# VinAIResearch/GeoFormer

Measured on AMD Instinct MI355X. Metric: scenes/sec forward (ScanNetV2 ~150k pts), higher is better.
Workload: dtype f32

## Files before the change

geoformer_amd/_build.py:

```python
from __future__ import annotations

import os
import shutil
import subprocess
import sys
from concurrent.futures import ThreadPoolExecutor

PKG_DIR = os.path.dirname(os.path.abspath(__file__))
REPO_DIR = os.path.dirname(PKG_DIR)
CSRC_DIR = os.path.join(PKG_DIR, "csrc")
LIB_DIR = os.path.join(PKG_DIR, "lib")
OBJ_DIR = os.path.join(LIB_DIR, "obj")
LIB_PATH = os.path.join(LIB_DIR, "libgeoformer_hip.so")
INCLUDE_DIR = os.path.join(REPO_DIR, "include")

ARCH = "gfx950"


def _hipcc() -> str:
    for cand in (os.environ.get("HIPCC"), shutil.which("hipcc"), "/opt/rocm/bin/hipcc"):
        if cand and os.path.exists(cand):
            return cand
    raise RuntimeError("hipcc not found (need ROCm toolchain to build libgeoformer_hip.so)")


def _sources():
    return sorted(
        os.path.join(CSRC_DIR, f) for f in os.listdir(CSRC_DIR) if f.endswith(".hip")
    )


def _headers():
    hs = [os.path.join(CSRC_DIR, f) for f in os.listdir(CSRC_DIR) if f.endswith((".h", ".hpp"))]
    hs += [os.path.join(INCLUDE_DIR, f) for f in os.listdir(INCLUDE_DIR) if f.endswith(".h")]
    return hs


def _stale(target: str, deps) -> bool:
    if not os.path.exists(target):
        return True
    t = os.path.getmtime(target)
    return any(os.path.getmtime(d) > t for d in deps)


def build_hip(force: bool = False, verbose: bool = False) -> str:
    os.makedirs(OBJ_DIR, exist_ok=True)
    hipcc = _hipcc()
    hdrs = _headers()
    srcs = _sources()
    flags = [
        f"--offload-arch={ARCH}",
        "-O3",
        "-fPIC",
        "-std=c++17",
        "-ffp-contract=off",
        "-fno-gpu-rdc",
        "-Wno-unused-result",
        f"-I{INCLUDE_DIR}",
        f"-I{CSRC_DIR}",
    ]
    extra = {}
    jobs = []
    objs = []
    for s in srcs:
        o = os.path.join(OBJ_DIR, os.path.basename(s)[:-4] + ".o")
        objs.append(o)
        if force or _stale(o, [s] + hdrs):
            jobs.append((s, o))

    def _cc(job):
        s, o = job
        cmd = [hipcc, *flags, *extra.get(os.path.basename(s), []), "-c", s, "-o", o]
        if verbose:
            print(" ".join(cmd), file=sys.stderr)
        r = subprocess.run(cmd, capture_output=True, text=True)
        if r.returncode != 0:
            raise RuntimeError(f"hipcc failed for {s}:\n{r.stdout}\n{r.stderr}")
        return o

    if jobs:
        with ThreadPoolExecutor(max_workers=min(6, len(jobs))) as ex:
            list(ex.map(_cc, jobs))
    if force or jobs or _stale(LIB_PATH, objs):
        cmd = [hipcc, f"--offload-arch={ARCH}", "-shared", "-fPIC", "-o", LIB_PATH, *objs]
        r = subprocess.run(cmd, capture_output=True, text=True)
        if r.returncode != 0:
            raise RuntimeError(f"link failed:\n{r.stdout}\n{r.stderr}")
    return LIB_PATH


if __name__ == "__main__":
    print(build_hip(force="--force" in sys.argv, verbose=True))
```

geoformer_amd/_lib.py:

```python
from __future__ import annotations

import ctypes
import os
from ctypes import c_char_p, c_float, c_int, c_longlong, c_size_t, c_uint, c_void_p

from ._build import LIB_PATH

LIB_PATH = os.environ.get("GF_LIB_PATH", LIB_PATH)

_lib = None


class GeoFormerHipError(RuntimeError):
    pass


def _declare(lib):
    P, I, F = c_void_p, c_int, c_float
    sig = {
        "gf_abi_version": (I, []),
        "gf_last_error": (c_char_p, []),
        "gf_index_words": (c_size_t, [I, I, I, I]),
        "gf_index_scratch_bytes": (c_size_t, [c_size_t]),
        "gf_index_build": (I, [P, I, P, I, I, I, I, P, P, P, P, P]),
        "gf_rules_subm3": (I, [P, I, P, I, I, I, P, P, P, P, I, P, P, P]),
        "gf_rules_steps_words": (c_size_t, [I]),
        "gf_rules_down2": (I, [P, I, P, I, I, I, I, P, P, P, P, P, P, I, P, P, P, I, P, P, P]),
        "gf_rules_down2_chain_plan": (I, [I, I, I, I, I, I, P, P, P, P, P]),
        "gf_rules_down2_chain": (I, [P, I, I, I, I, I, I, P, P, P]),
        "gf_conv_packed_floats": (c_size_t, [I, I, I]),
        "gf_conv_pack_weights": (I, [P, I, I, I, P, P]),
        "gf_conv_pack_weights_t": (I, [P, I, I, I, I, P, P]),
        "gf_conv_fwd": (I, [P, P, P, P, P, I, I, I, I, I, I, P, P, P, P, P, P, P]),
        "gf_feeder_create": (P, [I]),
        "gf_feeder_submit": (I, [P, P]),
        "gf_feeder_wait_issued": (I, [P, I]),
        "gf_feeder_wait_copied": (I, [P, I]),
        "gf_feeder_wait_head": (I, [P, I]),
        "gf_feeder_destroy": (I, [P]),
        "gf_conv_dual_supported": (I, [I, I, I, I, I]),
        "gf_rules_flat_words": (c_size_t, [I, I]),
        "gf_rules_flat_steps": (I, [P, P, I, I, I, I, P, P]),
        "gf_conv_fwd_flat": (I, [P, P, P, P, P, P, I, I, I, I, I, I, P, P, P, P, P, P, P, P]),
        "gf_conv_fwd_dual": (I, [P, P, P, P, P, I, I, I, I, I, I, P, P, P, P, P, P, P, P]),
        "gf_dev_conv_fwd_timed": (I, [P, P, P, P, P, I, I, I, I, I, I, P, P, P, P, P, P, P, P, P]),
        "gf_dev_conv_knobs_g16": (I, [I, I, I, I]),
        "gf_dev_conv_chunks": (I, [I]),
        "gf_dev_conv_g16p_wpb": (I, [I]),
        "gf_dev_conv_knobs": (I, [I, I, I, I, I]),
        "gf_dev_conv_knob_flat": (I, [I, I]),
        "gf_dev_conv_knob_lw": (I, [I, I]),
        "gf_dev_conv_plan": (I, [P, P, P, P, P, P, I, I, I, I, I, I, P, P, P, P, P, P, P, P]),
        "gf_resblock_fwd": (I, [P, P, P, P, P, P, P, I, I, I, I, I, P, P, P, P, P, P, P, P]),
        "gf_conv_wgrad": (I, [P, P, P, I, I, I, I, I, P, P]),
        "gf_conv_wgrad_masked": (I, [P, P, P, P, I, I, I, I, I, P, P]),
        "gf_conv_wgrad_masked_acc": (I, [P, P, P, P, I, I, I, I, I, P, P]),
        "gf_lsap": (I, [P, I, I, P, P, P, P, P, P]),
        "gf_pair_losses_sums_floats": (c_size_t, [I]),
        "gf_pair_losses_fwd": (I, [P, P, P, I, I, I, P, P, P, P]),
        "gf_pair_losses_bwd": (I, [P, P, P, P, I, I, I, P, P, P, P]),
        "gf_unet_ws_bytes": (c_size_t, [P, I, I, I, I, I]),
        "gf_dev_unet_probe": (I, [I]),
        "gf_dev_host_wait_ns": (ctypes.c_ulonglong, [I]),
        "gf_dev_unet_probe_read": (I, [I, P, P]),
        "gf_dev_unet_probe_read2": (I, [I, P, P, P]),
        "gf_dev_conv_kernel_events": (I, [P, P]),
        "gf_dev_conv_kernel_events_taken": (I, []),
        "gf_dev_op_kernel_events": (I, [I, P, P]),
        "gf_dev_op_kernel_events_taken": (I, [I]),
        "gf_dev_event_create": (P, []),
        "gf_dev_event_destroy": (I, [P]),
        "gf_dev_event_elapsed_us": (I, [P, P, P]),
        "gf_unet_fwd": (I, [P, P, P, I, I, I, I, I, P, c_size_t, P, P, P, P]),
        "gf_unet_fwd_phased": (I, [P, P, P, I, I, I, I, I, P, c_size_t, P, P, P, P, P, I, P, P]),
        "gf_unet_fwd_ahead": (I, [P, P, P, I, I, I, I, I, P, c_size_t, P, P, P, P, P, I]),
        "gf_voxelize_fp": (I, [P, P, I, I, I, I, P, P]),
        "gf_voxelize_bp": (I, [P, P, I, I, I, I, P, P]),
        "gf_gather_points": (I, [P, P, I, I, I, I, P, P]),
        "gf_gather_points_grad": (I, [P, P, I, I, I, I, P, P]),
        "gf_group_points": (I, [P, P, I, I, I, I, I, P, P]),
        "gf_group_points_grad": (I, [P, P, I, I, I, I, I, P, P]),
        "gf_ball_query": (I, [P, P, I, I, I, F, I, P, P]),
        "gf_fps_scratch_bytes": (c_size_t, [I]),
        "gf_furthest_point_sampling": (I, [P, I, I, I, P, P, P]),
        "gf_furthest_point_sampling_resume": (I, [P, I, I, I, I, P, P, P]),
        "gf_knn_scratch_bytes": (c_size_t, [I]),
        "gf_knn_radius": (I, [P, I, I, F, I, P, P, P, P, P]),
        "gf_knn_error_flag": (P, [P, I]),
        "gf_geodesic_bfs": (I, [P, P, P, I, I, P, I, F, I, P, P, P, P]),
        "gf_geodesic_bfs_cfg": (I, [P, P, P, I, I, P, I, F, I, P, P, P, c_size_t, I, P]),
        "gf_geodesic_bfs_queue_words": (c_size_t, [I]),
        "gf_dev_cross_attn_bf3": (I, [I]),
        "gf_dev_bfs_qcap_max": (I, [I]),
        "gf_mask_head": (I, [P, P, P, P, P, P, P, P, P, I, I, I, P, P]),
        "gf_mask_head_packed": (I, [P, P, P, P, P, P, P, P, P, I, I, I, I, P, P]),
        "gf_mask_head_episodes": (I, [P, P, P, P, P, P, P, P, P, I, I, I, I, I, P, P, P]),
        "gf_mask_head_split_bytes": (c_size_t, [I]),
        "gf_mask_head_bwd": (I, [P, P, P, P, P, P, P, P, P, I, I, I, I, P, P, P, P]),
        "gf_mask_head_bwd_episodes": (I, [P, P, P, P, P, P, P, P, P, I, I, I, I, I, P, P, P, P]),
        "gf_mask_head_bwd_scratch_floats": (c_size_t, [I, I]),
        "gf_softmax_dim1_fwd": (I, [P, I, I, I, F, P, P]),
        "gf_softmax_dim1_bwd": (I, [P, P, I, I, I, F, P, P]),
        "gf_pointwise_mlp": (I, [P, I, I, P, P, P, P, P, P, P]),
        "gf_pointwise_mlp_rows": (I, [P, P, I, I, P, P, P, P, P, P, P]),
        "gf_group_mlp_max": (I, [P, I, I, I, I, P, P, P, P, P, P, P]),
        "gf_ball_query_centres": (I, [P, P, I, I, I, F, I, P, P, P]),
        "gf_sa_group_mlp_max": (I, [P, P, P, I, I, I, I, F, I, I, I, I, P, P, P, P, P, P, P, P, P, I, P]),
        "gf_ball_query_grid": (I, [P, I, P, P, I, F, I, P, I, P, P, P]),
        "gf_point_grid_build": (I, [P, I, F, P, P]),
        "gf_decoder_token_state_bytes": (c_size_t, [I, I]),
        "gf_decoder_token_stage": (I, [P, P, P, I, I, I, I, I, P, P, P, P, P, P]),
        "gf_mask_intersections_scratch_bytes": (c_size_t, [I, I]),
        "gf_mask_intersections": (I, [P, I, I, P, P, P]),
        "gf_proposal_stats_batched": (I, [P, I, I, P, P, c_longlong, I, F, F, I, I, P, P, P, P, P]),
        "gf_proposal_select_batched": (I, [P, P, P, I, I, P, P, P, P, P]),
        "gf_proposal_scatter_batched": (I, [P, I, I, P, P, I, I, P, F, P, P]),
        "gf_mask_intersections_batched": (I, [P, I, c_longlong, c_longlong, P, P, P]),
        "gf_matrix_nms_batched": (I, [P, I, P, I, F, F, P, P, P]),
        "gf_label_map_batched": (I, [P, I, c_longlong, I, F, P, P, P, P, P, P, P, P, P]),
        "gf_instance_overlaps_scratch_bytes": (c_size_t, [I, I]),
        "gf_instance_overlaps": (I, [P, I, I, P, I, P, P, I, I, P, P, P, P, P, P]),
        "gf_voxelize_idx_scratch_bytes": (c_size_t, [I]),
        "gf_voxelize_idx_count": (I, [P, I, I, I, P, P, P, P]),
        "gf_voxelize_idx_fill": (I, [P, I, I, I, P, P, I, I, P, P, P]),
        "gf_host_legacy_choice": (I, [P, P, c_longlong, c_longlong, P]),
        "gf_host_legacy_prefetch": (I, [P, I, c_longlong]),
        "gf_host_draw_sample": (I, [P, P, c_longlong, c_longlong, P, c_longlong, P, P, P, P, I, P, P, P]),
        "gf_fg_scratch_bytes": (c_size_t, [I]),
        "gf_fg_select": (I, [P, I, I, I, I, P, P, P, P, I, P, P, P, P, P, P, P, P, P]),
        "gf_host_wait_word": (I, [P, I, c_longlong]),
        "gf_proposal_stats": (I, [P, P, P, I, I, I, F, F, I, I, P, P, P, P, P]),
        "gf_proposal_stats_fs": (I, [P, P, I, I, F, F, I, F, P, P, P, P]),
        "gf_proposal_scatter": (I, [P, P, I, I, P, F, I, P, P]),
        "gf_relpos_prepare": (I, [P, P, I, I, I, P, P, P]),
        "gf_proposal_select": (I, [P, P, P, I, P, P, P, P, P]),
        "gf_backbone_transformer_scratch_bytes": (c_size_t, [I]),
        "gf_backbone_transformer_num_params": (I, [I]),
        "gf_backbone_transformer": (I, [P, P, P, I, I, I, I, P, P, P, P]),
        "gf_decoder_pre_train_save_bytes": (c_size_t, [I, I]),
        "gf_decoder_pre_train_work_bytes": (c_size_t, [I, I]),
        "gf_decoder_pre_grad_floats": (c_longlong, []),
        "gf_decoder_pre_train_fwd": (I, [P, P, I, I, P, F, c_uint, I, P, P, P, P]),
        "gf_decoder_pre_train_bwd": (I, [P, P, P, P, P, I, I, P, F, c_uint, I, P, P, P, P, P, P]),
        "gf_decoder_post_train_save_bytes": (c_size_t, [I, I, I]),
        "gf_decoder_post_train_work_bytes": (c_size_t, [I, I, I]),
        "gf_decoder_post_grad_floats": (c_longlong, [I]),
        "gf_decoder_post_train_fwd": (I, [P, P, I, I, I, P, F, c_uint, I, P, P, P, P]),
        "gf_decoder_post_train_bwd": (I, [P, P, P, P, I, I, I, P, F, c_uint, I, P, P, P, P, P, P]),
        "gf_backbone_transformer_train_save_bytes": (c_size_t, [I, I]),
        "gf_backbone_transformer_train_work_bytes": (c_size_t, [I, I, I]),
        "gf_backbone_transformer_grad_floats": (c_longlong, [I, I]),
        "gf_backbone_transformer_train_fwd": (I, [P, P, I, I, I, I, P, F, c_uint, P, P, P]),
        "gf_backbone_transformer_train_bwd": (I, [P, P, I, I, I, I, P, F, c_uint, P, P, P, P, P]),
        "gf_decoder_wpack_floats": (c_size_t, []),
        "gf_decoder_pack_weights": (I, [P, P, P, P, P]),
        "gf_decoder_cross_attn": (I, [P, P, P, P, P, P, P, P, P, P, P, P, I, I, I, I, P, P, P, P]),
        "gf_decoder_cross_attn_cfg": (I, [P, P, P, P, P, P, P, P, P, P, P, P, I, I, I, I, P, P, P, I, P]),
        "gf_decoder_cross_attn_bwd_scratch_floats": (c_size_t, [I, I, I]),
        "gf_decoder_cross_attn_bwd": (I, [P] * 16 + [I, I, I, I] + [P] * 6),
        "gf_bn_train_scratch_floats": (c_size_t, [I, I]),
        "gf_bn_relu_train_fwd": (I, [P, I, I, P, P, F, F, I, P, P, P, P, P, P, P]),
        "gf_bn_relu_train_bwd": (I, [P, P, P, I, I, P, P, P, I, P, P, P, P, P]),
        "gf_bn_relu_train_bwd_add": (I, [P, P, P, I, I, P, P, P, I, P, P, P, P, P, P]),
        "gf_unet_train_scratch_floats": (c_size_t, [P, I, P]),
        "gf_unet_train_fwd": (I, [P, I, I, P, P, P, P, P, P]),
        "gf_unet_train_bwd": (I, [P, I, I, P, P, P, P, P, P, P, P]),
        "gf_bn_train_cl_scratch_floats": (c_size_t, [I, I, c_longlong]),
        "gf_bn_relu_train_cl_fwd": (I, [P, I, I, c_longlong, P, P, F, F, I, P, P, P, P, P, P, P]),
        "gf_bn_relu_train_cl_bwd": (I, [P, P, P, I, I, c_longlong, P, P, P, I, P, P, P, P, P]),
        "gf_sec_op": (I, [I, P, P, I, I, P, P]),
        "gf_roipool_fp": (I, [P, P, I, I, P, P, P]),
        "gf_roipool_bp": (I, [P, P, I, I, P, P]),
        "gf_get_iou": (I, [P, P, P, P, I, I, P, P]),
        "gf_ballquery_batch_p_scratch_bytes": (c_size_t, [I]),
        "gf_ballquery_batch_p": (I, [P, P, P, I, I, F, P, P, P, P, P]),
        "gf_bfs_cluster_host": (I, [P, P, P, I, I, P, P, P, P]),
        "gf_three_nn": (I, [P, P, I, I, I, P, P, P]),
        "gf_three_interpolate": (I, [P, P, P, I, I, I, I, P, P]),
        "gf_three_interpolate_grad": (I, [P, P, P, I, I, I, I, P, P]),
        "gf_aug_scan_blocks": (I, [I]),
        "gf_aug_draw": (I, [P, ctypes.c_ulonglong, c_longlong, I, P]),
        "gf_aug_transform": (I, [P, I, I, ctypes.c_double, I, P]),
        "gf_aug_elastic": (I, [P, I, I, I, I, ctypes.c_double, I, ctypes.c_ulonglong, c_longlong, I, c_longlong, P]),
        "gf_aug_crop": (I, [P, I, I, I, I, c_longlong, I, P]),
        "gf_aug_collate": (I, [P, P, I, I, I, I, P]),
        "gf_aug_collate_fs": (I, [P, I, I, I, P]),
        "gf_aug_support": (I, [P, P, ctypes.c_double, I, I, P]),
        "gf_aug_test_query": (I, [P, ctypes.c_double, I, I, P]),
        "gf_aug_support_block": (I, [P, P, P, ctypes.c_double, I, I, P]),
    }
    for name, (res, args) in sig.items():
        fn = getattr(lib, name)
        fn.restype = res
        fn.argtypes = args
    return sig


EXPORTS = None


def _check_hw_queues(torch):
    import warnings

    from . import HW_QUEUES_MIN, HW_QUEUES_WANTED, hw_queues_setting

    have = hw_queues_setting()
    if have is not None and have >= HW_QUEUES_MIN:
        return
    up = torch.cuda.is_initialized()
    warnings.warn(
        f"geoformer_amd: GPU_MAX_HW_QUEUES is {'unset (runtime default 4)' if have is None else have}"
        + (" and the HIP runtime is already initialised" if up else "")
        + f": the runtime picks its own number of hardware queues.  Export GPU_MAX_HW_QUEUES="
        f"{HW_QUEUES_WANTED} or call geoformer_amd.configure_runtime() before the process's first HIP call"
        + (" (e.g. before torch.cuda.set_device in train.py / test.py)." if up else "."),
        RuntimeWarning, stacklevel=3)


def load():
    global _lib, EXPORTS
    if _lib is not None:
        return _lib
    if not os.path.exists(LIB_PATH):
        raise GeoFormerHipError(
            f"{LIB_PATH} is missing: build it with `python -m geoformer_amd._build` "
            "(or __graft_entry__.build()).  There is no CPU fallback for the HIP operators."
        )
    import torch

    _check_hw_queues(torch)
    lib = ctypes.CDLL(LIB_PATH)
    EXPORTS = _declare(lib)
    if lib.gf_abi_version() != 7:
        raise GeoFormerHipError("libgeoformer_hip.so ABI version mismatch")
    _lib = lib
    return lib


def check(status: int, what: str = ""):
    if status != 0:
        msg = load().gf_last_error()
        raise GeoFormerHipError(f"{what} failed ({status}): {msg.decode() if msg else ''}")


FEEDER_MAX_COPIES = 16

# ... 49 lines not shown
```

geoformer_amd/csrc/common.h:

```cpp
#pragma once
#include <hip/hip_runtime.h>
#include <hip/hip_ext.h>
#include <stdint.h>
#include <stdio.h>

#include <type_traits>

#include "geoformer_hip.h"

#define GF_WAVE 64

typedef float f32x4 __attribute__((ext_vector_type(4)));

#define GF_STEP_BLKS 7
#define GF_STEP_PHA 3
#define GF_CONV_CHUNKS 3072
#define GF_CONV_CHUNKS_MAX 4096
int gf_conv_chunks();

void gf_set_error(const char* fmt, ...);

#define GF_CHECK_ARG(cond, ...)          \
    do {                                 \
        if (!(cond)) {                   \
            gf_set_error(__VA_ARGS__);   \
            return GF_ERR_INVALID_ARG;   \
        }                                \
    } while (0)

#define GF_TRY(call)                                                             \
    do {                                                                         \
        hipError_t e__ = (call);                                                 \
        if (e__ != hipSuccess) {                                                 \
            gf_set_error("%s failed: %s", #call, hipGetErrorString(e__));        \
            return GF_ERR_LAUNCH;                                                \
        }                                                                        \
    } while (0)

#define GF_CHECK_LAUNCH(name)                                                        \
    do {                                                                             \
        hipError_t e__ = hipGetLastError();                                          \
        if (e__ != hipSuccess) {                                                     \
            gf_set_error("%s: launch failed: %s", name, hipGetErrorString(e__));     \
            return GF_ERR_LAUNCH;                                                    \
        }                                                                            \
    } while (0)

int gf_rules_down2_chain_range(const int32_t* coords, int M0, int B, int X, int Y, int Z, int nlevels, int l_begin,
                               int l_end, int32_t* ws, int32_t* counts, hipStream_t st);

int gf_iscan_blocks(int n);
void gf_iscan(const int32_t* v, int n, int32_t* start, int32_t* cursor, int32_t* block_sums, int32_t* block_off,
              hipStream_t st);

int gf_rules_down2_chain_all(const int32_t* coords, int M0, int B, int X, int Y, int Z, int nlevels, int32_t* ws,
                             int32_t* counts, hipStream_t st);
bool gf_rules_level_parallel();

static inline int gf_div_up(long long a, long long b) { return (int)((a + b - 1) / b); }

template <class T, T... Vs, class F>
static inline void gf_with(T v, F&& f) {
    (void)((v == Vs && (f(std::integral_constant<T, Vs>{}), true)) || ...);
}

void gf_allow_lds(const void* kernel, int bytes);

template <int D>
__device__ __forceinline__ float gf_shfl_xor(float v) {
    static_assert(D == 32 || D == 16 || D == 8 || D == 4 || D == 2 || D == 1, "gf_shfl_xor: D = 1, 2, 4, 8, 16, 32");
    const unsigned x = __float_as_uint(v);
    if constexpr (D == 32) {
        const auto r = __builtin_amdgcn_permlane32_swap(x, x, false, false);
        return __uint_as_float((__lane_id() & 32) ? r[0] : r[1]);
    } else if constexpr (D == 16) {
        const auto r = __builtin_amdgcn_permlane16_swap(x, x, false, false);
        return __uint_as_float((__lane_id() & 16) ? r[0] : r[1]);
    } else if constexpr (D == 8) {
        return __uint_as_float((unsigned)__builtin_amdgcn_update_dpp((int)x, (int)x, 0x128, 0xF, 0xF, false));
    } else if constexpr (D == 4) {
        const int t = __builtin_amdgcn_update_dpp((int)x, (int)x, 0x104, 0xF, 0x5, false);
        return __uint_as_float((unsigned)__builtin_amdgcn_update_dpp(t, (int)x, 0x114, 0xF, 0xA, false));
    } else if constexpr (D == 2) {
        return __uint_as_float((unsigned)__builtin_amdgcn_update_dpp((int)x, (int)x, 0x4E, 0xF, 0xF, false));
    } else {
        return __uint_as_float((unsigned)__builtin_amdgcn_update_dpp((int)x, (int)x, 0xB1, 0xF, 0xF, false));
    }
}
template <int D>
__device__ __forceinline__ int gf_shfl_xor_i(int v) {
    return __float_as_int(gf_shfl_xor<D>(__int_as_float(v)));
}
__device__ __forceinline__ int gf_wave_sum_i(int s) {
    s += gf_shfl_xor_i<32>(s);
    s += gf_shfl_xor_i<16>(s);
    s += gf_shfl_xor_i<8>(s);
    s += gf_shfl_xor_i<4>(s);
    s += gf_shfl_xor_i<2>(s);
    s += gf_shfl_xor_i<1>(s);
    return s;
}
__device__ __forceinline__ float gf_wave_max(float m) {
    m = fmaxf(m, gf_shfl_xor<32>(m));
    m = fmaxf(m, gf_shfl_xor<16>(m));
    m = fmaxf(m, gf_shfl_xor<8>(m));
    m = fmaxf(m, gf_shfl_xor<4>(m));
    m = fmaxf(m, gf_shfl_xor<2>(m));
    m = fmaxf(m, gf_shfl_xor<1>(m));
    return m;
}
__device__ __forceinline__ float gf_wave_sum(float s) {
    s += gf_shfl_xor<32>(s);
    s += gf_shfl_xor<16>(s);
    s += gf_shfl_xor<8>(s);
    s += gf_shfl_xor<4>(s);
    s += gf_shfl_xor<2>(s);
    s += gf_shfl_xor<1>(s);
    return s;
}

#define GF_FLAT_HIST 8
#define GF_FLAT_BSTART 40
#define GF_FLAT_BCUR 72
#define GF_FLAT_GOFF 128
#define GF_FLAT_BINS 1024
#define GF_FLAT_PAD 32
#define GF_LW_WPB 12
__host__ __device__ static inline size_t gf_flat_ppos_at(int ngroups) { return GF_FLAT_GOFF + (size_t)ngroups + 1; }
__host__ __device__ static inline size_t gf_flat_desc_at(int ngroups) { return (GF_FLAT_GOFF + 2 * (size_t)ngroups + 1 + 63) / 64 * 64; }
__host__ __device__ static inline size_t gf_flat_steps_at(int ngroups, int nbins) {
    return gf_flat_desc_at(ngroups) + (size_t)((ngroups + nbins - 1) / nbins + 1) * nbins * 4;
}
int gf_conv_lw_supported(int K, int M_in, int M_out, int Cin, int Cout, bool aligned, int* forced);
int gf_conv_lw(const float* in, const float* Wp, const uint32_t* gmask, const int32_t* flat, int K, int M_in, int M_out, int Cin,
               int Cout, const float* in_scale, const float* in_shift, const float* residual, const float* out_scale,
               const float* out_shift, float* out, float* out2, hipStream_t st);

enum { GF_OP_BFS = 0, GF_OP_CROSS_ATTN = 1, GF_OP_MASK_HEAD = 2, GF_OP_FPS = 3, GF_OP_CROSS_ATTN_BWD = 4,
       GF_OP_MASK_HEAD_BWD_FEAT = 5, GF_OP_MASK_HEAD_BWD_PARAM = 6, GF_OP_WGRAD = 7, GF_OP_COUNT = 8 };
struct GfOpEvents {
    hipEvent_t start, stop;
    int taken;
};
GfOpEvents* gf_op_events(int op);
#define GF_LAUNCH_OP(op, kernel, grid, block, lds, st, ...)                                              \
    do {                                                                                                 \
        GfOpEvents* oe__ = gf_op_events(op);                                                             \
        if (oe__->start) {                                                                               \
            hipExtLaunchKernelGGL(kernel, grid, block, (uint32_t)(lds), st, oe__->start, oe__->stop, 0u, __VA_ARGS__); \
            oe__->start = oe__->stop = nullptr;                                                          \
            oe__->taken = 1;                                                                             \
        } else {                                                                                         \
            hipLaunchKernelGGL(kernel, grid, block, lds, st, __VA_ARGS__);                               \
        }                                                                                                \
    } while (0)

struct GfIndex {
    const uint32_t* bitmap;
    const int32_t* prefix;
    const int32_t* perm;
    int X, Y, Z;
};

__device__ __forceinline__ int gf_index_lookup(const GfIndex& ix, int b, int x, int y, int z) {
    if ((unsigned)x >= (unsigned)ix.X || (unsigned)y >= (unsigned)ix.Y || (unsigned)z >= (unsigned)ix.Z) return -1;
    unsigned long long lin = (((unsigned long long)b * ix.X + x) * ix.Y + y) * ix.Z + z;
    unsigned long long w = lin >> 5;
    unsigned bit = (unsigned)(lin & 31);
    uint32_t word = ix.bitmap[w];
    if (!((word >> bit) & 1u)) return -1;
    int rank = ix.prefix[w] + __popc(word & ((1u << bit) - 1u));
    return ix.perm ? ix.perm[rank] : rank;
}

#define SCAN_THREADS 256
__device__ __forceinline__ int wave_incl_scan(int v) {
    const int lane = threadIdx.x & 63;
#pragma unroll
    for (int d = 1; d < 64; d <<= 1) {
        int t = __shfl_up(v, d, 64);
        if (lane >= d) v += t;
    }
    return v;
}

__device__ __forceinline__ int block_excl_scan(int v, int* total) {
    __shared__ int wsum[SCAN_THREADS / 64];
    const int lane = threadIdx.x & 63, wid = threadIdx.x >> 6;
    int inc = wave_incl_scan(v);
    if (lane == 63) wsum[wid] = inc;
    __syncthreads();
    int off = 0, tot = 0;
#pragma unroll
    for (int w = 0; w < SCAN_THREADS / 64; w++) {
        int s = wsum[w];
        if (w < wid) off += s;
        tot += s;
    }
    __syncthreads();
    *total = tot;
    return off + inc - v;
}

int gf_backbone_transformer_tables(const int* scene_offsets, int n_scenes, int M, void* scratch, void* stream);
int gf_backbone_transformer_prepared(const float* feats, const int* coords, const int* scene_offsets, int n_scenes, int M, int c,
                                     int n_layers, const float* const* params, void* scratch, float* out, void* stream);
```

geoformer_amd/csrc/geodesic.hip:

```cpp
#include <cstdlib>
#include "common.h"

#ifndef BFS_KEY_SCOPE
#define BFS_KEY_SCOPE __HIP_MEMORY_SCOPE_AGENT
#endif
#include <type_traits>

__device__ __forceinline__ int3 cell_of(float x, float y, float z, float inv_cell) {
    return make_int3((int)floorf(x * inv_cell), (int)floorf(y * inv_cell), (int)floorf(z * inv_cell));
}
__device__ __forceinline__ unsigned bucket_of(int cx, int cy, int cz, unsigned tmask) {
    return (((unsigned)cx * 73856093u) ^ ((unsigned)cy * 19349663u) ^ ((unsigned)cz * 83492791u)) & tmask;
}

__global__ void k_grid_count(const float* __restrict__ xyz, int n, float inv_cell, unsigned tmask,
                             int32_t* __restrict__ counts) {
    int i = blockIdx.x * blockDim.x + threadIdx.x;
    if (i >= n) return;
    int3 c = cell_of(xyz[i * 3 + 0], xyz[i * 3 + 1], xyz[i * 3 + 2], inv_cell);
    atomicAdd(&counts[bucket_of(c.x, c.y, c.z, tmask)], 1);
}

#define ISCAN_IPT 4
#define ISCAN_IPB (SCAN_THREADS * ISCAN_IPT)
__global__ void k_iscan_block_sums(const int32_t* __restrict__ v, int n, int32_t* __restrict__ block_sums) {
    int base = blockIdx.x * ISCAN_IPB + threadIdx.x * ISCAN_IPT;
    int s = 0;
#pragma unroll
    for (int j = 0; j < ISCAN_IPT; j++)
        if (base + j < n) s += v[base + j];
    int tot;
    block_excl_scan(s, &tot);
    if (threadIdx.x == 0) block_sums[blockIdx.x] = tot;
}
__global__ void k_iscan_top(const int32_t* __restrict__ block_sums, int nblocks, int32_t* __restrict__ block_off) {
    __shared__ int carry_s;
    if (threadIdx.x == 0) carry_s = 0;
    __syncthreads();
    for (int base = 0; base < nblocks; base += SCAN_THREADS) {
        int i = base + threadIdx.x;
        int val = i < nblocks ? block_sums[i] : 0;
        int tot;
        int ex = block_excl_scan(val, &tot);
        int carry = carry_s;
        if (i < nblocks) block_off[i] = carry + ex;
        __syncthreads();
        if (threadIdx.x == 0) carry_s = carry + tot;
        __syncthreads();
    }
}
__global__ void k_iscan_apply(const int32_t* __restrict__ v, int n, const int32_t* __restrict__ block_off,
                              int32_t* __restrict__ start, int32_t* __restrict__ cursor) {
    int base = blockIdx.x * ISCAN_IPB + threadIdx.x * ISCAN_IPT;
    int c[ISCAN_IPT];
    int s = 0;
#pragma unroll
    for (int j = 0; j < ISCAN_IPT; j++) {
        c[j] = (base + j < n) ? v[base + j] : 0;
        s += c[j];
    }
    int tot;
    int ex = block_excl_scan(s, &tot) + block_off[blockIdx.x];
#pragma unroll
    for (int j = 0; j < ISCAN_IPT; j++) {
        if (base + j < n) {
            start[base + j] = ex;
            cursor[base + j] = ex;
        }
        ex += c[j];
        if (base + j == n - 1) start[n] = ex;
    }
}

__global__ void k_grid_fill(const float* __restrict__ xyz, int n, float inv_cell, unsigned tmask,
                            int32_t* __restrict__ cursor, float4* __restrict__ sorted) {
    int i = blockIdx.x * blockDim.x + threadIdx.x;
    if (i >= n) return;
    const float x = xyz[i * 3 + 0], y = xyz[i * 3 + 1], z = xyz[i * 3 + 2];
    int3 c = cell_of(x, y, z, inv_cell);
    int pos = atomicAdd(&cursor[bucket_of(c.x, c.y, c.z, tmask)], 1);
    sorted[pos] = make_float4(x, y, z, __int_as_float(i));
}

int gf_iscan_blocks(int n) { return (n + ISCAN_IPB - 1) / ISCAN_IPB; }
void gf_iscan(const int32_t* v, int n, int32_t* start, int32_t* cursor, int32_t* block_sums, int32_t* block_off,
              hipStream_t st) {
    const int nb = gf_iscan_blocks(n);
    hipLaunchKernelGGL(k_iscan_block_sums, dim3(nb), dim3(SCAN_THREADS), 0, st, v, n, block_sums);
    hipLaunchKernelGGL(k_iscan_top, dim3(1), dim3(SCAN_THREADS), 0, st, block_sums, nb, block_off);
    hipLaunchKernelGGL(k_iscan_apply, dim3(nb), dim3(SCAN_THREADS), 0, st, v, n, block_off, start, cursor);
}

#define KNN_WAVES 4
#define KNN_CAP 1024
__global__ __launch_bounds__(KNN_WAVES * 64) void k_knn_radius(const float* __restrict__ xyz, int n, int k,
                                                               float radius, float inv_cell, unsigned tmask,
                                                               const int32_t* __restrict__ start,
                                                               const float4* __restrict__ sorted, int sqrt_out,
                                                               float* __restrict__ D, int32_t* __restrict__ I,
                                                               int32_t* __restrict__ deg, int* __restrict__ err) {
    __shared__ unsigned long long s_keys[KNN_WAVES][KNN_CAP];
    __shared__ int s_off[KNN_WAVES][28];
    __shared__ int s_beg[KNN_WAVES][27];
    const int lane = threadIdx.x & 63, wid = threadIdx.x >> 6;
    const int i = blockIdx.x * KNN_WAVES + wid;
    if (i >= n) return;
    const float qx = xyz[i * 3 + 0], qy = xyz[i * 3 + 1], qz = xyz[i * 3 + 2];
    const int3 qc = cell_of(qx, qy, qz, inv_cell);
    int beg = 0, cnt = 0;
    int ncx = 0, ncy = 0, ncz = 0;
    if (lane < 27) {
        ncx = qc.x + lane / 9 - 1;
        ncy = qc.y + (lane / 3) % 3 - 1;
        ncz = qc.z + lane % 3 - 1;
        const unsigned h = bucket_of(ncx, ncy, ncz, tmask);
        beg = start[h];
        cnt = start[h + 1] - beg;
    }
    int inc = cnt;
#pragma unroll
    for (int d = 1; d < 32; d <<= 1) {
        int t = __shfl_up(inc, d, 64);
        if (lane >= d) inc += t;
    }
    if (lane < 27) {
        s_off[wid][lane + 1] = inc;
        s_beg[wid][lane] = beg;
    }
    if (lane == 0) s_off[wid][0] = 0;
    const int total = __shfl(inc, 26, 64);
    __builtin_amdgcn_wave_barrier();
    int nin = 0;
    for (int t0 = 0; t0 < total; t0 += 64) {
        const int t = t0 + lane;
        bool hit = false;
        unsigned long long key = 0;
        if (t < total) {
            int c = 0;
#pragma unroll
            for (int s = 1; s < 27; s++) c += (s_off[wid][s] <= t) ? 1 : 0;
            const float4 p = sorted[s_beg[wid][c] + (t - s_off[wid][c])];
            const int3 pc = cell_of(p.x, p.y, p.z, inv_cell);
            const int ex = qc.x + c / 9 - 1, ey = qc.y + (c / 3) % 3 - 1, ez = qc.z + c % 3 - 1;
            if (pc.x == ex && pc.y == ey && pc.z == ez) {
                const float dx = qx - p.x, dy = qy - p.y, dz = qz - p.z;
                const float d2 = fmaf(dz, dz, fmaf(dy, dy, dx * dx));
                if (sqrtf(d2) <= radius) {
                    hit = true;
                    key = ((unsigned long long)__float_as_uint(d2) << 32) | (unsigned)__float_as_int(p.w);
                }
            }
        }
        const unsigned long long bal = __ballot(hit);
// ... 70 lines not shown

extern "C" int gf_point_grid_build(const float* xyz, int n, float radius, void* scratch, void* stream) {
    GF_CHECK_ARG(xyz && scratch && n >= 1 && radius > 0.f, "gf_point_grid_build: bad arguments");
    PointGrid G;
    if (int rc = build_point_grid(xyz, n, radius, scratch, (hipStream_t)stream, &G)) return rc;
    GF_CHECK_LAUNCH("gf_point_grid_build");
    return GF_OK;
}

extern "C" int gf_knn_radius(const float* xyz, int n, int k, float radius, int sqrt_out, float* D, int32_t* I,
                             int32_t* deg, void* scratch, void* stream) {
    GF_CHECK_ARG(n >= 0 && k >= 1 && k <= 64 && radius > 0.f, "gf_knn_radius: bad arguments n=%d k=%d r=%g", n, k,
                 radius);
    if (n == 0) return GF_OK;
    hipStream_t st = (hipStream_t)stream;
    PointGrid G;
    if (int rc = build_point_grid(xyz, n, radius, scratch, st, &G)) return rc;
    hipLaunchKernelGGL(k_knn_radius, dim3(gf_div_up(n, KNN_WAVES)), dim3(KNN_WAVES * 64), 0, st, xyz, n, k, radius,
                       G.inv_cell, G.tmask, G.start, G.sorted, sqrt_out, D, I, deg, G.err);
    GF_CHECK_LAUNCH("gf_knn_radius");
    return GF_OK;
}

#define BQG_WAVES 4
#define BQG_CAP 1024
__global__ __launch_bounds__(BQG_WAVES * 64) void k_ball_query_grid(const float* __restrict__ xyz, int n,
                                                                    const int32_t* __restrict__ centre_idx,
                                                                    const float* __restrict__ centres, int m,
                                                                    float radius2, int nsample, PointGrid G,
                                                                    float* __restrict__ new_xyz_out,
                                                                    int32_t* __restrict__ idx) {
    __shared__ __attribute__((aligned(16))) unsigned s_hit[BQG_WAVES][BQG_CAP + 16];
    __shared__ int s_off[BQG_WAVES][28];
    __shared__ int s_beg[BQG_WAVES][27];
    const int lane = threadIdx.x & 63, wid = threadIdx.x >> 6;
    const int j = blockIdx.x * BQG_WAVES + wid;
    if (j >= m) return;
    const float* c = centre_idx ? xyz + (size_t)centre_idx[j] * 3 : centres + (size_t)j * 3;
    const float qx = c[0], qy = c[1], qz = c[2];
    if (new_xyz_out && lane < 3) new_xyz_out[(size_t)j * 3 + lane] = lane == 0 ? qx : lane == 1 ? qy : qz;
    const int3 qc = cell_of(qx, qy, qz, G.inv_cell);
    int beg = 0, cnt = 0;
    if (lane < 27) {
        const unsigned h = bucket_of(qc.x + lane / 9 - 1, qc.y + (lane / 3) % 3 - 1, qc.z + lane % 3 - 1, G.tmask);
        beg = G.start[h];
        cnt = G.start[h + 1] - beg;
    }
    int inc = cnt;
#pragma unroll
    for (int d = 1; d < 32; d <<= 1) {
        int t = __shfl_up(inc, d, 64);
        if (lane >= d) inc += t;
    }
    if (lane < 27) {
        s_off[wid][lane + 1] = inc;
        s_beg[wid][lane] = beg;
    }
    if (lane == 0) s_off[wid][0] = 0;
    const int total = __shfl(inc, 26, 64);
    __builtin_amdgcn_wave_barrier();
    int nin = 0;
    for (int t0 = 0; t0 < total; t0 += 64) {
        const int t = t0 + lane;
        bool hit = false;
        unsigned pid = 0;
        if (t < total) {
            int cc = 0;
#pragma unroll
            for (int s = 1; s < 27; s++) cc += (s_off[wid][s] <= t) ? 1 : 0;
            const float4 p = G.sorted[s_beg[wid][cc] + (t - s_off[wid][cc])];
            const int3 pc = cell_of(p.x, p.y, p.z, G.inv_cell);
            if (pc.x == qc.x + cc / 9 - 1 && pc.y == qc.y + (cc / 3) % 3 - 1 && pc.z == qc.z + cc % 3 - 1) {
                const float dx = qx - p.x, dy = qy - p.y, dz = qz - p.z;
                hit = fmaf(dz, dz, fmaf(dy, dy, dx * dx)) < radius2;
                pid = (unsigned)__float_as_int(p.w);
            }
        }
        const unsigned long long bal = __ballot(hit);
        const int pos = nin + __popcll(bal & ((1ull << lane) - 1ull));
        if (hit && pos < BQG_CAP) s_hit[wid][pos] = pid;
        nin += __popcll(bal);
    }
    int32_t* row = idx + (size_t)j * nsample;
    if (nin > BQG_CAP) {
        int got = 0, first = -1;
        for (int s = 0; s < n && got < nsample; s += 64) {
            const int p = s + lane;
            bool hit = false;
            if (p < n) {
                const float dx = qx - xyz[(size_t)p * 3 + 0], dy = qy - xyz[(size_t)p * 3 + 1],
                            dz = qz - xyz[(size_t)p * 3 + 2];
                hit = fmaf(dz, dz, fmaf(dy, dy, dx * dx)) < radius2;
            }
            const unsigned long long bal = __ballot(hit);
            if (bal) {
                if (first < 0) first = s + __builtin_ctzll(bal);
                const int pos = got + __popcll(bal & ((1ull << lane) - 1ull));
                if (hit && pos < nsample) row[pos] = p;
                got += __popcll(bal);
            }
        }
        for (int l = min(got, nsample) + lane; l < nsample; l += 64) row[l] = first < 0 ? 0 : first;
        return;
    }
    {
        const int padded = (nin + 15) & ~15;
        if (nin + lane < padded) s_hit[wid][nin + lane] = 0xffffffffu;
    }
    __builtin_amdgcn_wave_barrier();
    unsigned lowest = 0xffffffffu;
    typedef unsigned u32x4 __attribute__((ext_vector_type(4)));
    const u32x4* list = reinterpret_cast<const u32x4*>(s_hit[wid]);
    const int n16 = (nin + 15) >> 4;
    for (int t = lane; t < nin; t += 64) {
        const unsigned key = s_hit[wid][t];
        int rank = 0;
        for (int u = 0; u < n16; u++) {
            const u32x4 a = list[4 * u + 0], b = list[4 * u + 1], c2 = list[4 * u + 2], d = list[4 * u + 3];
            rank += (a[0] < key) + (a[1] < key) + (a[2] < key) + (a[3] < key) + (b[0] < key) + (b[1] < key) +
                    (b[2] < key) + (b[3] < key) + (c2[0] < key) + (c2[1] < key) + (c2[2] < key) + (c2[3] < key) +
                    (d[0] < key) + (d[1] < key) + (d[2] < key) + (d[3] < key);
        }
        if (rank < nsample) row[rank] = (int)key;
        lowest = min(lowest, key);
    }
#pragma unroll
    for (int d = 32; d >= 1; d >>= 1) lowest = min(lowest, (unsigned)__shfl_xor((int)lowest, d, 64));
    const int pad = nin > 0 ? (int)lowest : 0;
    for (int l = min(nin, nsample) + lane; l < nsample; l += 64) row[l] = pad;
}

extern "C" int gf_ball_query_grid(const float* xyz, int n, const int32_t* centre_idx, const float* centres, int m,
                                  float radius, int nsample, void* scratch, int grid_ready, float* new_xyz,
                                  int32_t* idx, void* stream) {
    GF_CHECK_ARG(xyz && scratch && idx && (centre_idx || centres), "gf_ball_query_grid: null argument");
    GF_CHECK_ARG(n >= 1 && m >= 0 && nsample >= 1 && radius > 0.f, "gf_ball_query_grid: bad sizes");
    if (m == 0) return GF_OK;
    hipStream_t st = (hipStream_t)stream;
    PointGrid G;
    if (int rc = build_point_grid(xyz, n, radius, scratch, st, &G, grid_ready != 0)) return rc;
    hipLaunchKernelGGL(k_ball_query_grid, dim3(gf_div_up(m, BQG_WAVES)), dim3(BQG_WAVES * 64), 0, st, xyz, n, centre_idx,
                       centres, m, radius * radius, nsample, G, new_xyz, idx);
    GF_CHECK_LAUNCH("gf_ball_query_grid");
    return GF_OK;
}

extern "C" const int32_t* gf_knn_error_flag(void* scratch, int n) {
    const unsigned T = knn_table_size(n);
    const int nb = (int)((T + ISCAN_IPB - 1) / ISCAN_IPB);
    return (const int32_t*)scratch + 3 * (size_t)T + 1 + 2 * (size_t)nb;
}

#define BFS_THREADS 1024
__global__ __launch_bounds__(BFS_THREADS) void k_geodesic_bfs(const float* __restrict__ D, const int32_t* __restrict__ I,
                                                              const int32_t* __restrict__ deg, int n, int K,
                                                              const int32_t* __restrict__ src, float radius,
                                                              int max_step, float* __restrict__ geo,
                                                              unsigned* __restrict__ keys,
                                                              int32_t* __restrict__ queues) {
    __shared__ int s_cnt;
    const int q = blockIdx.x;
    float* g = geo + (size_t)q * n;
    unsigned* key = keys + (size_t)q * n;
    int2* cur = reinterpret_cast<int2*>(queues + (size_t)q * 4 * n);
    int2* nxt = cur + n;
    const int tid = threadIdx.x;
    for (int t = tid; t < n; t += BFS_THREADS) {
        g[t] = -1.0f;
        key[t] = 0xffffffffu;
    }
    const int s = src[q];
    __syncthreads();
    if (tid == 0) {
        g[s] = 0.0f;
        cur[0] = make_int2(s, deg ? deg[s] : K - 1);
        s_cnt = 0;
    }
    __syncthreads();
    int ncur = 1;
    const bool vec = (K & 3) == 0;
    for (int step = 0; step < max_step && ncur > 0; step++) {
        for (int f = tid; f < ncur; f += BFS_THREADS) {
            const int2 e = cur[f];
            const int u = e.x, du = e.y;
            const int32_t* Iu = I + (size_t)u * K;
            const float* Du = D + (size_t)u * K;
            for (int r0 = 0; r0 <= du; r0 += 16) {
                int v[16];
                float d[16];
#pragma unroll
                for (int c = 0; c < 4; c++) {
                    const int rb = r0 + 4 * c;
                    if (rb <= du && vec) {
                        const int4 vi = *reinterpret_cast<const int4*>(Iu + rb);
                        const float4 di = *reinterpret_cast<const float4*>(Du + rb);
                        v[4 * c + 0] = vi.x; v[4 * c + 1] = vi.y; v[4 * c + 2] = vi.z; v[4 * c + 3] = vi.w;
                        d[4 * c + 0] = di.x; d[4 * c + 1] = di.y; d[4 * c + 2] = di.z; d[4 * c + 3] = di.w;
                    } else {
#pragma unroll
                        for (int j = 0; j < 4; j++) {
                            const int rr = rb + j;
                            const bool ok = rr <= du && rr < K;
                            v[4 * c + j] = ok ? Iu[rr] : -1;
                            d[4 * c + j] = ok ? Du[rr] : 0.f;
                        }
                    }
                }
                float gv[16];
#pragma unroll
                for (int j = 0; j < 16; j++) {
                    const int rr = r0 + j;
                    const bool ok = rr >= 1 && rr <= du && v[j] >= 0 && d[j] <= radius;
                    gv[j] = ok ? g[v[j]] : 0.0f;
                }
#pragma unroll
                for (int j = 0; j < 16; j++) {
                    if (gv[j] < 0.0f) {
                        const unsigned cand = (((unsigned)u << 6) | (unsigned)(r0 + j)) + 1u;
                        const unsigned old = __hip_atomic_fetch_min(&key[v[j]], cand, __ATOMIC_RELAXED, BFS_KEY_SCOPE);
                        if (old == 0xffffffffu) {
                            const int pos = atomicAdd(&s_cnt, 1);
                            nxt[pos].x = v[j];
                        }
                    }
                }
            }
        }
        __syncthreads();
        const int nn = s_cnt;
        __syncthreads();
        if (tid == 0) s_cnt = 0;
        for (int t = tid; t < nn; t += BFS_THREADS) {
            const int v = nxt[t].x;
            const unsigned kk = __hip_atomic_load(&key[v], __ATOMIC_RELAXED, BFS_KEY_SCOPE) - 1u;
            const int u = (int)(kk >> 6), r = (int)(kk & 63u);
            const int dv = deg ? deg[v] : K - 1;
            g[v] = D[(size_t)u * K + r] + g[u];
            nxt[t].y = dv;
        }
        __syncthreads();
        int2* tmp = cur;
        cur = nxt;
        nxt = tmp;
        ncur = nn;
    }
}

#define BFS_LDS_MAX_N (1 << 19)
#ifndef BFS_LDS_BYTES
#define BFS_LDS_BYTES (150 * 1024)
#endif
__device__ __forceinline__ void bfs_lds_barrier() {
    __builtin_amdgcn_fence(__ATOMIC_RELEASE, "workgroup", "local");
    __builtin_amdgcn_s_barrier();
    __builtin_amdgcn_fence(__ATOMIC_ACQUIRE, "workgroup", "local");
}
template <int THREADS>
__global__ __launch_bounds__(THREADS) void k_geodesic_bfs_lds(const float* __restrict__ D,
                                                                  const int32_t* __restrict__ I, int n, int K,
                                                                  const int32_t* __restrict__ src, float radius,
                                                                  int max_step, float* __restrict__ geo,
                                                                  unsigned long long* __restrict__ keys,
                                                                  int2* __restrict__ queues, int qcap) {
    extern __shared__ __attribute__((aligned(16))) unsigned char smem[];
    __shared__ int s_cnt[2];
    const int nw = (n + 31) >> 5;
    unsigned* visited = reinterpret_cast<unsigned*>(smem);
    unsigned* touched = visited + nw;
    int2* q0 = reinterpret_cast<int2*>(touched + nw + ((2 * nw) & 1));
    int2* q1 = q0 + qcap;
    const int q = blockIdx.x;
    float* g = geo + (size_t)q * n;
    unsigned long long* key = keys + (size_t)q * n;
    int2* gq0 = queues + (size_t)q * 2 * n;
    int2* gq1 = gq0 + n;
    const int tid = threadIdx.x;
    for (int t = tid; t < n; t += THREADS) {
        g[t] = -1.0f;
        key[t] = ~0ull;
    }
    for (int t = tid; t < nw; t += THREADS) {
        visited[t] = 0u;
        touched[t] = 0u;
    }
    const int s = src[q];
    __syncthreads();
    if (tid == 0) {
        g[s] = 0.0f;
        visited[s >> 5] = 1u << (s & 31);
        touched[s >> 5] = 1u << (s & 31);
        q0[0] = make_int2(s, __float_as_int(0.0f));
        s_cnt[0] = 0;
        s_cnt[1] = 0;
    }
    __syncthreads();
    int ncur = 1;
    int2 *cl = q0, *cg = gq0, *nl = q1, *ng = gq1;
    constexpr int BFS_B = 4;
    const int l16 = tid & 15;
    const int gsh = (tid & 48) | 15;
    int pv[BFS_B];
    float pd[BFS_B];
    bool have_pf = false;
#ifdef BFS_TRACE
    unsigned long long tr[12] = {0, 0, 0, 0, 0, 0, 0, 0, 0, 0, 0, 0};
#define BT() __builtin_amdgcn_s_memtime()
#endif
    for (int step = 0; step < max_step && ncur > 0; step++) {
#ifdef BFS_TRACE
        const unsigned long long t0_ = BT();
        tr[5]++; tr[6] += ncur; tr[7] = tr[7] > (unsigned long long)ncur ? tr[7] : (unsigned long long)ncur;
#endif
        int* cnt = &s_cnt[step & 1];
        auto bid = [&](int u, float gu, int r, int v, float d) {
            const unsigned bit = 1u << (v & 31);
            if (!(visited[v >> 5] & bit)) {
#ifdef BFS_TRACE
                if ((tid >> 4) == 0) tr[9]++;
#endif
                const unsigned cand = (((unsigned)u << 6) | (unsigned)r) + 1u;
                __hip_atomic_fetch_min(&key[v], ((unsigned long long)cand << 32) | (unsigned)__float_as_int(d + gu),
                                       __ATOMIC_RELAXED, BFS_KEY_SCOPE);
                const unsigned old = atomicOr(&touched[v >> 5], bit);
                if (!(old & bit)) {
                    const int pos = atomicAdd(cnt, 1);
                    if (pos < qcap) nl[pos].x = v;
                    else ng[pos - qcap].x = v;
                }
            }
        };
        const int kc = l16 < K ? l16 : K - 1;
        auto batch = [&](int base, auto spill, auto pf) {
            unsigned cand[BFS_B];
            int v[BFS_B];
            float d[BFS_B];
            {
                float gu[BFS_B];
#pragma unroll
                for (int k = 0; k < BFS_B; k++) {
                    const int f = (base + k * THREADS + tid) >> 4;
                    const int fc = f < ncur ? f : ncur - 1;
                    int2 e = cl[fc < qcap ? fc : 0];
                    if constexpr (decltype(spill)::value)
                        if (fc >= qcap) e = cg[fc - qcap];
                    cand[k] = (((unsigned)e.x << 6) | (unsigned)l16) + 1u;
                    gu[k] = __int_as_float(e.y);
                    if constexpr (decltype(pf)::value) {
                        v[k] = pv[k];
                        d[k] = pd[k];
                    } else {
                        v[k] = I[(size_t)e.x * K + kc];
                        d[k] = D[(size_t)e.x * K + kc];
                    }
                }
#ifdef BFS_TRACE
                if (tid == 0) tr[8]++;
#endif
#pragma unroll
                for (int k = 0; k < BFS_B; k++) asm volatile("" : "+v"(v[k]), "+v"(d[k]));
#ifdef BFS_TRACE
                asm volatile("s_waitcnt vmcnt(0) lgkmcnt(0)" ::: "memory");
                if (base == 0) tr[10] += BT() - t0_;
#endif
#pragma unroll
                for (int k = 0; k < BFS_B; k++) {
                    const int f = (base + k * THREADS + tid) >> 4;
                    if (!(f < ncur && l16 < K && d[k] <= radius)) v[k] = -1;
                    d[k] += gu[k];
                }
            }
#ifdef BFS_TRACE
            const unsigned long long tb0_ = BT();
#endif
            unsigned long long mm = 0ull;
            unsigned w[BFS_B];
#pragma unroll
            for (int k = 0; k < BFS_B; k++) {
                mm |= ((__ballot(v[k] >= 0) >> gsh) & 1ull) << k;
                w[k] = visited[v[k] >= 0 ? (v[k] >> 5) : 0];
            }
#pragma unroll
            for (int k = 0; k < BFS_B; k++) {
                const unsigned bit = 1u << (v[k] & 31);
                const bool bids = v[k] >= 0 && l16 >= 1 && !(w[k] & bit);
#ifdef BFS_TRACE
                if ((tid >> 4) == 0) tr[9] += bids ? 1 : 0;
#endif
                w[k] = 1u;
                if (bids) {
                    __hip_atomic_fetch_min(&key[v[k]], ((unsigned long long)cand[k] << 32) | (unsigned)__float_as_int(d[k]),
                                           __ATOMIC_RELAXED, BFS_KEY_SCOPE);
                    w[k] = atomicOr(&touched[v[k] >> 5], bit) & bit;
                }
            }
            unsigned long long fm[BFS_B];
            int nfirst = 0;
#pragma unroll
            for (int k = 0; k < BFS_B; k++) {
                fm[k] = __ballot(w[k] == 0u);
                nfirst += __popcll(fm[k]);
            }
            if (nfirst) {
                int pos = 0;
                if ((tid & 63) == 0) pos = atomicAdd(cnt, nfirst);
                pos = __builtin_amdgcn_readfirstlane(pos);
#pragma unroll
                for (int k = 0; k < BFS_B; k++) {
                    if (w[k] == 0u) {
                        const int p = pos + (int)__builtin_amdgcn_mbcnt_hi((unsigned)(fm[k] >> 32),
                                                                             __builtin_amdgcn_mbcnt_lo((unsigned)fm[k], 0u));
                        if (p < qcap) nl[p].x = v[k];
                        else ng[p - qcap].x = v[k];
                    }
                    pos += __popcll(fm[k]);
                }
            }
#ifdef BFS_TRACE
            if (base == 0) tr[11] += BT() - tb0_;
#endif
            if (mm) {
#pragma unroll
                for (int k = 0; k < BFS_B; k++) {
                    if ((mm >> k) & 1ull) {
                        const int f = (base + k * THREADS + tid) >> 4;
                        int2 e = cl[f < qcap ? f : 0];
                        if constexpr (decltype(spill)::value)
                            if (f >= qcap) e = cg[f - qcap];
                        for (int r0 = 16; r0 < K; r0 += 16) {
                            const int r = r0 + l16;
                            int vv = -1;
                            float dd = 0.f;
                            if (r < K) {
                                vv = I[(size_t)e.x * K + r];
                                dd = D[(size_t)e.x * K + r];
                            }
                            const bool in2 = vv >= 0 && dd <= radius;
                            if (in2) bid(e.x, __int_as_float(e.y), r, vv, dd);
                            if (!((__ballot(in2) >> gsh) & 1ull)) break;
                        }
                    }
                }
            }
        };
        auto expand = [&](auto spill) {
            int base = 0;
            if (have_pf) {
                batch(0, spill, std::true_type{});
                base = BFS_B * THREADS;
            }
            for (; (base >> 4) < ncur; base += BFS_B * THREADS) batch(base, spill, std::false_type{});
        };
        if (ncur > qcap) expand(std::true_type{});
        else expand(std::false_type{});
#ifdef BFS_TRACE
        const unsigned long long t1_ = BT();
#endif
        asm volatile("s_waitcnt vmcnt(0)" ::: "memory");
#ifdef BFS_TRACE
        const unsigned long long t2_ = BT();
#endif
        __syncthreads();
#ifdef BFS_TRACE
        const unsigned long long t3_ = BT();
#endif
        const int nn = *cnt;
        if (tid == 0) s_cnt[(step + 1) & 1] = 0;
        const bool pf_now = step + 1 < max_step;
        auto commit_batch = [&](int base, auto spill, auto pf) {
            int v[BFS_B];
            unsigned kk[BFS_B];
#pragma unroll
            for (int k = 0; k < BFS_B; k++) {
                const int t = (base + k * THREADS + tid) >> 4;
                const int tc = t < nn ? t : nn - 1;
                v[k] = nl[tc < qcap ? tc : 0].x;
                if constexpr (decltype(spill)::value)
                    if (tc >= qcap) v[k] = ng[tc - qcap].x;
                kk[k] = __hip_atomic_load(reinterpret_cast<const unsigned*>(&key[v[k]]), __ATOMIC_RELAXED, BFS_KEY_SCOPE);
            }
            if constexpr (decltype(pf)::value) {
#pragma unroll
                for (int k = 0; k < BFS_B; k++) {
                    pv[k] = I[(size_t)v[k] * K + kc];
                    pd[k] = D[(size_t)v[k] * K + kc];
                }
            }
#pragma unroll
            for (int k = 0; k < BFS_B; k++) {
                const int t = (base + k * THREADS + tid) >> 4;
                if (t < nn && l16 == 0) {
                    const int di = (int)kk[k];
                    g[v[k]] = __int_as_float(di);
                    if (!decltype(spill)::value || t < qcap) nl[t].y = di;
                    else ng[t - qcap].y = di;
                    atomicOr(&visited[v[k] >> 5], 1u << (v[k] & 31));
                }
            }
        };
        auto commit = [&](auto spill) {
            int base = 0;
            if (pf_now && nn > 0) {
                commit_batch(0, spill, std::true_type{});
                base = BFS_B * THREADS;
            }
            for (; (base >> 4) < nn; base += BFS_B * THREADS) commit_batch(base, spill, std::false_type{});
        };
        if (nn > qcap) commit(std::true_type{});
        else commit(std::false_type{});
        have_pf = pf_now;
#ifdef BFS_TRACE
        const unsigned long long t4_ = BT();
#endif
        if (nn > qcap) __syncthreads();
        else bfs_lds_barrier();
#ifdef BFS_TRACE
        const unsigned long long t5_ = BT();
        tr[0] += t1_ - t0_; tr[1] += t2_ - t1_; tr[2] += t3_ - t2_; tr[3] += t4_ - t3_; tr[4] += t5_ - t4_;
#endif
        int2* t1 = cl; cl = nl; nl = t1;
        int2* t2 = cg; cg = ng; ng = t2;
        ncur = nn;
    }
#ifdef BFS_TRACE
    if (tid == 0 && n >= 12)
        for (int i = 0; i < 12; i++) reinterpret_cast<unsigned long long*>(gq0)[i] = tr[i];
#endif
}

template <int THREADS>
static void launch_bfs_lds(int nq, size_t lds, hipStream_t st, const float* D, const int32_t* I, int n, int K,
                           const int32_t* src, float radius, int max_step, float* geo, void* keys_ws, void* queue_ws,
                           int qcap) {
    gf_allow_lds((const void*)k_geodesic_bfs_lds<THREADS>, BFS_LDS_BYTES);
    GF_LAUNCH_OP(GF_OP_BFS, k_geodesic_bfs_lds<THREADS>, dim3(nq), dim3(THREADS), lds, st, D, I, n, K, src, radius, max_step,
                 geo, (unsigned long long*)keys_ws, (int2*)queue_ws, qcap);
}
static int g_bfs_qcap_max = 0;
extern "C" int gf_dev_bfs_qcap_max(int qcap) {
    g_bfs_qcap_max = qcap > 0 ? qcap : 0;
    return GF_OK;
}
extern "C" size_t gf_geodesic_bfs_queue_words(int n) { return (size_t)4 * (size_t)(n > 0 ? n : 0); }

extern "C" int gf_geodesic_bfs_cfg(const float* D, const int32_t* I, const int32_t* deg, int n, int K,
                                   const int32_t* src, int nq, float radius, int max_step, float* geo, void* keys_ws,
                                   void* queue_ws, size_t queue_words, int wg_threads, void* stream) {
    GF_CHECK_ARG(n >= 1 && K >= 2 && K <= 64 && nq >= 0 && max_step >= 0, "gf_geodesic_bfs: bad arguments");
    GF_CHECK_ARG(n < (1 << 26), "gf_geodesic_bfs: n=%d exceeds the 26-bit parent field", n);
    GF_CHECK_ARG(wg_threads == 1024 || wg_threads == 512 || wg_threads == 256, "gf_geodesic_bfs: wg_threads=%d (256, 512 or 1024)",
                 wg_threads);
    if (nq == 0) return GF_OK;
    GF_CHECK_ARG(queue_words >= (size_t)4 * (size_t)n, "gf_geodesic_bfs: queue workspace of %zu words per query, %zu needed",
                 queue_words, (size_t)4 * (size_t)n);
    const int nw = (n + 31) / 32;
    const size_t bm = ((size_t)2 * nw + ((2 * nw) & 1)) * sizeof(unsigned);
    while (wg_threads < 1024 && bm + 256 * 2 * sizeof(int2) > (size_t)BFS_LDS_BYTES * wg_threads / 1024) wg_threads *= 2;
    const size_t budget = (size_t)BFS_LDS_BYTES * wg_threads / 1024;
    if (n <= BFS_LDS_MAX_N && (K & 3) == 0 && bm + 64 * 2 * sizeof(int2) <= budget) {
        int qcap = (int)((budget - bm) / (2 * sizeof(int2)));
        if (qcap > n) qcap = n;
        if (g_bfs_qcap_max > 0 && qcap > g_bfs_qcap_max) qcap = g_bfs_qcap_max < 64 ? 64 : g_bfs_qcap_max;
        const size_t lds = bm + (size_t)qcap * 2 * sizeof(int2);
        hipStream_t st = (hipStream_t)stream;
        if (wg_threads == 256)
            launch_bfs_lds<256>(nq, lds, st, D, I, n, K, src, radius, max_step, geo, keys_ws, queue_ws, qcap);
        else if (wg_threads == 512)
            launch_bfs_lds<512>(nq, lds, st, D, I, n, K, src, radius, max_step, geo, keys_ws, queue_ws, qcap);
        else
            launch_bfs_lds<1024>(nq, lds, st, D, I, n, K, src, radius, max_step, geo, keys_ws, queue_ws, qcap);
        GF_CHECK_LAUNCH("gf_geodesic_bfs");
        return GF_OK;
    }
    hipLaunchKernelGGL(k_geodesic_bfs, dim3(nq), dim3(BFS_THREADS), 0, (hipStream_t)stream, D, I, deg, n, K, src,
                       radius, max_step, geo, (unsigned*)keys_ws, (int32_t*)queue_ws);
    GF_CHECK_LAUNCH("gf_geodesic_bfs");
    return GF_OK;
}

extern "C" int gf_geodesic_bfs(const float* D, const int32_t* I, const int32_t* deg, int n, int K, const int32_t* src,
                               int nq, float radius, int max_step, float* geo, void* keys_ws, void* queue_ws,
                               void* stream) {
    return gf_geodesic_bfs_cfg(D, I, deg, n, K, src, nq, radius, max_step, geo, keys_ws, queue_ws, (size_t)4 * (size_t)(n > 0 ? n : 0),
                               1024, stream);
}

__global__ void k_bqb_count(const float* __restrict__ xyz, const int32_t* __restrict__ batch_idxs,
                            const int32_t* __restrict__ batch_offsets, int n, float radius2, int32_t* __restrict__ cnt) {
    int i = blockIdx.x * blockDim.x + threadIdx.x;
    if (i >= n) return;
    const float ox = xyz[i * 3 + 0], oy = xyz[i * 3 + 1], oz = xyz[i * 3 + 2];
    const int b = batch_idxs[i];
    int c = 0;
    for (int k = batch_offsets[b]; k < batch_offsets[b + 1]; k++) {
        const float dx = ox - xyz[k * 3 + 0], dy = oy - xyz[k * 3 + 1], dz = oz - xyz[k * 3 + 2];
        if (fmaf(dz, dz, fmaf(dy, dy, dx * dx)) < radius2) {
            if (c >= 1000) break;
            c++;
        }
    }
    cnt[i] = c;
}
__global__ void k_bqb_fill(const float* __restrict__ xyz, const int32_t* __restrict__ batch_idxs,
                           const int32_t* __restrict__ batch_offsets, int n, float radius2,
                           const int32_t* __restrict__ start, const int32_t* __restrict__ cnt, long long thre,
                           int32_t* __restrict__ idx, int32_t* __restrict__ start_len) {
    int i = blockIdx.x * blockDim.x + threadIdx.x;
    if (i >= n) return;
    const int s = start[i];
    int c = cnt[i];
    start_len[i * 2 + 0] = s;
    start_len[i * 2 + 1] = c;
    if (s >= thre) return;
    if ((long long)s + c >= thre) c = (int)(thre - s);
    const float ox = xyz[i * 3 + 0], oy = xyz[i * 3 + 1], oz = xyz[i * 3 + 2];
    const int b = batch_idxs[i];
    int w = 0;
    for (int k = batch_offsets[b]; k < batch_offsets[b + 1] && w < c; k++) {
        const float dx = ox - xyz[k * 3 + 0], dy = oy - xyz[k * 3 + 1], dz = oz - xyz[k * 3 + 2];
        if (fmaf(dz, dz, fmaf(dy, dy, dx * dx)) < radius2) idx[s + w++] = k;
    }
}
extern "C" size_t gf_ballquery_batch_p_scratch_bytes(int n) {
    const size_t nb = ((size_t)n + ISCAN_IPB - 1) / ISCAN_IPB;
    return (2 * (size_t)n + 4 + 2 * nb + 16) * sizeof(int32_t);
}
extern "C" int gf_ballquery_batch_p(const float* xyz, const int32_t* batch_idxs, const int32_t* batch_offsets, int n,
                                    int meanActive, float radius, int32_t* idx, int32_t* start_len, int32_t* d_cumsum,
                                    void* scratch, void* stream) {
    GF_CHECK_ARG(n >= 0 && meanActive >= 1, "gf_ballquery_batch_p: bad arguments");
    hipStream_t st = (hipStream_t)stream;
    if (n == 0) {
        GF_TRY(hipMemsetAsync(d_cumsum, 0, sizeof(int32_t), st));
        return GF_OK;
    }
    const int nb = (n + ISCAN_IPB - 1) / ISCAN_IPB;
    int32_t* cnt = (int32_t*)scratch;
    int32_t* start = cnt + n;
    int32_t* block_sums = start + n + 2;
    int32_t* block_off = block_sums + nb;
    const float r2 = radius * radius;
    hipLaunchKernelGGL(k_bqb_count, dim3(gf_div_up(n, 256)), dim3(256), 0, st, xyz, batch_idxs, batch_offsets, n, r2, cnt);
    hipLaunchKernelGGL(k_iscan_block_sums, dim3(nb), dim3(SCAN_THREADS), 0, st, cnt, n, block_sums);
    hipLaunchKernelGGL(k_iscan_top, dim3(1), dim3(SCAN_THREADS), 0, st, block_sums, nb, block_off);
    hipLaunchKernelGGL(k_iscan_apply, dim3(nb), dim3(SCAN_THREADS), 0, st, cnt, n, block_off, start, start_len);
    GF_TRY(hipMemcpyAsync(d_cumsum, start + n, sizeof(int32_t), hipMemcpyDeviceToDevice, st));
    hipLaunchKernelGGL(k_bqb_fill, dim3(gf_div_up(n, 256)), dim3(256), 0, st, xyz, batch_idxs, batch_offsets, n, r2,
                       start, cnt, (long long)n * meanActive, idx, start_len);
    GF_CHECK_LAUNCH("gf_ballquery_batch_p");
    return GF_OK;
}
```

geoformer_amd/csrc/pointops.hip:

```cpp
#include <stdlib.h>

#include <type_traits>

#include "common.h"

__global__ void k_voxelize_fp(const float* __restrict__ feats, const int32_t* __restrict__ rules, int M, int maxActive,
                              int C, int average, float* __restrict__ out) {
    long long t = (long long)blockIdx.x * blockDim.x + threadIdx.x;
    if (t >= (long long)M * C) return;
    const int row = (int)(t / C), c = (int)(t - (long long)row * C);
    const int32_t* r = rules + (size_t)row * (maxActive + 1);
    const int n = r[0];
    const float mult = (average && n > 0) ? __fdiv_rn(1.0f, (float)n) : 1.0f;
    float acc = 0.f;
    for (int i = 1; i <= n; i++) acc = __fadd_rn(acc, __fmul_rn(mult, feats[(size_t)r[i] * C + c]));
    out[t] = acc;
}

__global__ void k_voxelize_bp(const float* __restrict__ d_out, const int32_t* __restrict__ rules, int M, int maxActive,
                              int C, int average, float* __restrict__ d_feats) {
    long long t = (long long)blockIdx.x * blockDim.x + threadIdx.x;
    if (t >= (long long)M * C) return;
    const int row = (int)(t / C), c = (int)(t - (long long)row * C);
    const int32_t* r = rules + (size_t)row * (maxActive + 1);
    const int n = r[0];
    const float mult = (average && n > 0) ? __fdiv_rn(1.0f, (float)n) : 1.0f;
    const float g = __fmul_rn(mult, d_out[t]);
    for (int i = 1; i <= n; i++) atomicAdd(&d_feats[(size_t)r[i] * C + c], g);
}

extern "C" int gf_voxelize_fp(const float* feats, const int32_t* rules, int M, int maxActive, int C, int average,
                              float* out, void* stream) {
    GF_CHECK_ARG(M >= 0 && maxActive >= 0 && C >= 1, "gf_voxelize_fp: bad sizes");
    if (M == 0) return GF_OK;
    hipLaunchKernelGGL(k_voxelize_fp, dim3(gf_div_up((long long)M * C, 256)), dim3(256), 0, (hipStream_t)stream, feats,
                       rules, M, maxActive, C, average, out);
    GF_CHECK_LAUNCH("gf_voxelize_fp");
    return GF_OK;
}
extern "C" int gf_voxelize_bp(const float* d_out, const int32_t* rules, int M, int maxActive, int C, int average,
                              float* d_feats, void* stream) {
    GF_CHECK_ARG(M >= 0 && maxActive >= 0 && C >= 1, "gf_voxelize_bp: bad sizes");
    if (M == 0) return GF_OK;
    hipLaunchKernelGGL(k_voxelize_bp, dim3(gf_div_up((long long)M * C, 256)), dim3(256), 0, (hipStream_t)stream, d_out,
                       rules, M, maxActive, C, average, d_feats);
    GF_CHECK_LAUNCH("gf_voxelize_bp");
    return GF_OK;
}

__global__ void k_gather_points(const float* __restrict__ points, const int32_t* __restrict__ idx, int b, int c, int n,
                                int m, float* __restrict__ out) {
    long long t = (long long)blockIdx.x * blockDim.x + threadIdx.x;
    if (t >= (long long)b * c * m) return;
    const int j = (int)(t % m);
    const long long bc = t / m;
    const int bi = (int)(bc / c);
    out[t] = points[bc * n + idx[(size_t)bi * m + j]];
}
__global__ void k_gather_points_grad(const float* __restrict__ grad_out, const int32_t* __restrict__ idx, int b, int c,
                                     int n, int m, float* __restrict__ grad_points) {
    long long t = (long long)blockIdx.x * blockDim.x + threadIdx.x;
    if (t >= (long long)b * c * m) return;
    const int j = (int)(t % m);
    const long long bc = t / m;
    const int bi = (int)(bc / c);
    atomicAdd(&grad_points[bc * n + idx[(size_t)bi * m + j]], grad_out[t]);
}
__global__ void k_group_points(const float* __restrict__ points, const int32_t* __restrict__ idx, int b, int c, int n,
                               int np, int ns, float* __restrict__ out) {
    long long t = (long long)blockIdx.x * blockDim.x + threadIdx.x;
    const long long per = (long long)np * ns;
    if (t >= (long long)b * c * per) return;
    const long long js = t % per;
    const long long bc = t / per;
    const int bi = (int)(bc / c);
    out[t] = points[bc * n + idx[(size_t)bi * per + js]];
}
__global__ void k_group_points_grad(const float* __restrict__ grad_out, const int32_t* __restrict__ idx, int b, int c,
                                    int n, int np, int ns, float* __restrict__ grad_points) {
    long long t = (long long)blockIdx.x * blockDim.x + threadIdx.x;
    const long long per = (long long)np * ns;
    if (t >= (long long)b * c * per) return;
    const long long js = t % per;
    const long long bc = t / per;
    const int bi = (int)(bc / c);
    atomicAdd(&grad_points[bc * n + idx[(size_t)bi * per + js]], grad_out[t]);
}

#define GF_ELEMENTWISE(fn, kern, total, ...)                                                                    \
    do {                                                                                                        \
        long long tot__ = (total);                                                                              \
        if (tot__ > 0) {                                                                                        \
            hipLaunchKernelGGL(kern, dim3(gf_div_up(tot__, 256)), dim3(256), 0, (hipStream_t)stream, __VA_ARGS__); \
            GF_CHECK_LAUNCH(fn);                                                                                \
        }                                                                                                       \
        return GF_OK;                                                                                           \
    } while (0)

extern "C" int gf_gather_points(const float* points, const int32_t* idx, int b, int c, int n, int m, float* out,
                                void* stream) {
    GF_ELEMENTWISE("gf_gather_points", k_gather_points, (long long)b * c * m, points, idx, b, c, n, m, out);
}
extern "C" int gf_gather_points_grad(const float* grad_out, const int32_t* idx, int b, int c, int n, int m,
                                     float* grad_points, void* stream) {
    GF_ELEMENTWISE("gf_gather_points_grad", k_gather_points_grad, (long long)b * c * m, grad_out, idx, b, c, n, m,
                   grad_points);
}
extern "C" int gf_group_points(const float* points, const int32_t* idx, int b, int c, int n, int np, int ns, float* out,
                               void* stream) {
    GF_ELEMENTWISE("gf_group_points", k_group_points, (long long)b * c * np * ns, points, idx, b, c, n, np, ns, out);
}
extern "C" int gf_group_points_grad(const float* grad_out, const int32_t* idx, int b, int c, int n, int np, int ns,
                                    float* grad_points, void* stream) {
    GF_ELEMENTWISE("gf_group_points_grad", k_group_points_grad, (long long)b * c * np * ns, grad_out, idx, b, c, n, np,
                   ns, grad_points);
}

#ifndef BQ_WAVES
#define BQ_WAVES 8
#endif
#ifndef BQ_TILE
#define BQ_TILE 2048
#endif
#define BQ_PLANE (BQ_TILE + 12)
#define BQ_LD ((BQ_TILE * 3 + BQ_WAVES * 64 - 1) / (BQ_WAVES * 64))
__global__ __launch_bounds__(BQ_WAVES * 64) void k_ball_query(const float* __restrict__ new_xyz,
                                                               const float* __restrict__ xyz, int n, int m,
                                                               float radius2, int nsample, int32_t* __restrict__ idx,
                                                               const int32_t* __restrict__ centre_idx,
                                                               float* __restrict__ new_xyz_out) {
    __shared__ __attribute__((aligned(16))) float tile[2][3 * BQ_PLANE];
    __shared__ int s_done[2][BQ_WAVES];
    const int bi = blockIdx.y;
    xyz += (size_t)bi * n * 3;
    idx += (size_t)bi * m * nsample;
    const int lane = threadIdx.x & 63, wid = threadIdx.x >> 6;
    const int j = blockIdx.x * BQ_WAVES + wid;
    const bool valid = j < m;
    float nx = 0.f, ny = 0.f, nz = 0.f;
    if (valid) {
        const float* c = centre_idx ? xyz + (size_t)centre_idx[(size_t)bi * m + j] * 3 : new_xyz + ((size_t)bi * m + j) * 3;
        nx = c[0];
        ny = c[1];
        nz = c[2];
        if (centre_idx && lane < 3) new_xyz_out[((size_t)bi * m + j) * 3 + lane] = lane == 0 ? nx : lane == 1 ? ny : nz;
    }
    int cnt = valid ? 0 : nsample;
    int first = -1;
    int slot[BQ_LD];
#pragma unroll
    for (int i = 0; i < BQ_LD; i++) {
        const unsigned f = threadIdx.x + BQ_WAVES * 64 * i;
        const unsigned p = __umulhi(f, 0xAAAAAAABu) >> 1;
        slot[i] = f < BQ_TILE * 3 ? (int)((f - 3u * p) * BQ_PLANE + p) : -1;
    }
// ... 46 lines not shown
                    if (first < 0) {
                        const int l0 = __builtin_ctzll(any);
                        const int u0 = ((bal[0] >> l0) & 1) ? 0 : ((bal[1] >> l0) & 1) ? 1 : ((bal[2] >> l0) & 1) ? 2 : 3;
                        first = base + s + 4 * l0 + u0;
                    }
                    const unsigned long long below = (1ull << lane) - 1ull;
                    int pos = cnt + __popcll(bal[0] & below) + __popcll(bal[1] & below) + __popcll(bal[2] & below) +
                              __popcll(bal[3] & below);
#pragma unroll
                    for (int u = 0; u < 4; u++) {
                        if (hit[u]) {
                            if (pos < nsample) idx[(size_t)j * nsample + pos] = base + s + 4 * lane + u;
                            pos++;
                        }
                    }
                    cnt += __popcll(bal[0]) + __popcll(bal[1]) + __popcll(bal[2]) + __popcll(bal[3]);
                }
            }
        }
        if (t + 1 < ntiles) stage(buf ^ 1);
        if (lane == 0) s_done[buf ^ 1][wid] = cnt >= nsample;
        __syncthreads();
    }
    if (valid) {
        const int filled = min(cnt, nsample);
        const int pad = first < 0 ? 0 : first;
        for (int l = filled + lane; l < nsample; l += 64) idx[(size_t)j * nsample + l] = pad;
    }
}

extern "C" int gf_ball_query(const float* new_xyz, const float* xyz, int b, int n, int m, float radius, int nsample,
                             int32_t* idx, void* stream) {
    GF_CHECK_ARG(b >= 0 && n >= 0 && m >= 0 && nsample >= 1, "gf_ball_query: bad sizes");
    if (b == 0 || m == 0) return GF_OK;
    const float radius2 = radius * radius;
    hipLaunchKernelGGL(k_ball_query, dim3(gf_div_up(m, BQ_WAVES), b), dim3(BQ_WAVES * 64), 0, (hipStream_t)stream,
                       new_xyz, xyz, n, m, radius2, nsample, idx, nullptr, nullptr);
    GF_CHECK_LAUNCH("gf_ball_query");
    return GF_OK;
}

extern "C" int gf_ball_query_centres(const float* xyz, const int32_t* centre_idx, int b, int n, int m, float radius,
                                     int nsample, float* new_xyz, int32_t* idx, void* stream) {
    GF_CHECK_ARG(b >= 0 && n >= 0 && m >= 0 && nsample >= 1, "gf_ball_query_centres: bad sizes");
    GF_CHECK_ARG(centre_idx && new_xyz, "gf_ball_query_centres: null argument");
    if (b == 0 || m == 0) return GF_OK;
    const float radius2 = radius * radius;
    hipLaunchKernelGGL(k_ball_query, dim3(gf_div_up(m, BQ_WAVES), b), dim3(BQ_WAVES * 64), 0, (hipStream_t)stream,
                       nullptr, xyz, n, m, radius2, nsample, idx, centre_idx, new_xyz);
    GF_CHECK_LAUNCH("gf_ball_query_centres");
    return GF_OK;
}

#define FPS_KEY_NONE 0x7fffffffu
#define FPS_SPIN_LIMIT (1 << 22)

__device__ __forceinline__ unsigned dpp_max_step(unsigned v, unsigned o) { return o > v ? o : v; }

__device__ __forceinline__ unsigned wave_max_u32(unsigned v) {
    v = dpp_max_step(v, (unsigned)__builtin_amdgcn_update_dpp(0, (int)v, 0xB1, 0xF, 0xF, true));
    v = dpp_max_step(v, (unsigned)__builtin_amdgcn_update_dpp(0, (int)v, 0x4E, 0xF, 0xF, true));
    v = dpp_max_step(v, (unsigned)__builtin_amdgcn_update_dpp(0, (int)v, 0x141, 0xF, 0xF, true));
    v = dpp_max_step(v, (unsigned)__builtin_amdgcn_update_dpp(0, (int)v, 0x140, 0xF, 0xF, true));
    const unsigned r0 = __builtin_amdgcn_readlane((int)v, 0), r1 = __builtin_amdgcn_readlane((int)v, 16);
    const unsigned r2 = __builtin_amdgcn_readlane((int)v, 32), r3 = __builtin_amdgcn_readlane((int)v, 48);
    const unsigned a = r0 > r1 ? r0 : r1, b = r2 > r3 ? r2 : r3;
    return a > b ? a : b;
}

__device__ __forceinline__ void wave_best(unsigned& dbits, unsigned& key) {
    const unsigned md = wave_max_u32(dbits);
    const unsigned long long owners = __ballot(dbits == md);
    if (__popcll(owners) == 1) {
        key = (unsigned)__builtin_amdgcn_readlane((int)key, __builtin_ctzll(owners));
    } else {
        const unsigned cand = dbits == md ? (FPS_KEY_NONE - key) : 0u;
        key = FPS_KEY_NONE - wave_max_u32(cand);
    }
    dbits = md;
}

template <int I, int N, typename F>
__device__ __forceinline__ void fps_static_for(F&& f) {
    if constexpr (I < N) {
        f(std::integral_constant<int, I>{});
        fps_static_for<I + 1, N>(f);
    }
}

#ifndef FPS_WAVES
#define FPS_WAVES 16
#endif
#ifndef FPS_MAXG
#define FPS_MAXG 16
#endif
#ifndef FPS_KPUB
#define FPS_KPUB 4
#endif
#ifndef FPS_K
#define FPS_K 16
#endif
#define FPS_PW (FPS_WAVES - FPS_WAVES / 4)
#ifndef FPS_POLL_SLEEP
#define FPS_POLL_SLEEP 4
#endif
#define FPS_NG (FPS_MAXG * FPS_KPUB / 64)
#define FPS_TAG (1ull << 63)

__device__ __forceinline__ unsigned long long fps_code(unsigned dbits, unsigned key) {
    return ((unsigned long long)dbits << 32) | ((unsigned long long)(FPS_KEY_NONE - key) << 1);
}
__device__ __forceinline__ unsigned long long wave_max_u64(unsigned long long c) {
    const unsigned hi = (unsigned)(c >> 32), md = wave_max_u32(hi);
    const unsigned long long owners = __ballot(hi == md);
    unsigned ml;
    if (__popcll(owners) == 1) {
        ml = (unsigned)__builtin_amdgcn_readlane((int)(unsigned)c, __builtin_ctzll(owners));
    } else {
        ml = wave_max_u32(hi == md ? (unsigned)c : 0u);
    }
    return ((unsigned long long)md << 32) | ml;
}
__device__ __forceinline__ int fps_code_index(unsigned long long c) {
    return c ? (int)((FPS_KEY_NONE - (unsigned)((c >> 1) & 0x7fffffffull)) & 0x3fffffu) : 0;
}

#ifdef FPS_TRACE
__device__ unsigned long long* g_fps_trace = nullptr;
extern "C" int gf_dev_fps_trace(void* p) {
    GF_TRY(hipMemcpyToSymbol(HIP_SYMBOL(g_fps_trace), &p, sizeof(p)));
    return GF_OK;
}
#define FT() __builtin_amdgcn_s_memtime()
#define FTA(i, a, b) do { ftr[i] += (b) - (a); } while (0)
#else
#define FT() 0ull
#define FTA(i, a, b) do { } while (0)
#endif

#define FPS_LDS_ST(p, v) __hip_atomic_store((p), (v), __ATOMIC_RELAXED, __HIP_MEMORY_SCOPE_WORKGROUP)
#define FPS_LDS_LD(p) __hip_atomic_load((p), __ATOMIC_RELAXED, __HIP_MEMORY_SCOPE_WORKGROUP)
#define FPS_ORDER() asm volatile("" ::: "memory")
template <int P>
__device__ __forceinline__ void fps_absorb(const float (&px)[P], const float (&py)[P], const float (&pz)[P], float (&tmp)[P],
                                           float ax, float ay, float az) {
#pragma unroll
    for (int i = 0; i < P; i++) {
        const float dx = px[i] - ax, dy = py[i] - ay, dz = pz[i] - az;
        tmp[i] = fminf(fmaf(dz, dz, fmaf(dy, dy, dx * dx)), tmp[i]);
    }
}

template <int P>
__global__ __launch_bounds__(FPS_WAVES * 64) void k_fps(const float* __restrict__ xyz, int n, int m, int m0, int G,
                                                        int bs_log2, int batch0,
                                                        unsigned long long* __restrict__ slots,
                                                        int32_t* __restrict__ idxs, int* __restrict__ err) {
    static_assert(FPS_NG >= 1 && FPS_NG * 64 == FPS_MAXG * FPS_KPUB && FPS_KPUB <= FPS_K && FPS_WAVES * 2 <= 64,
                  "lane mappings of the exchange");
    __shared__ unsigned long long s_part[2][FPS_WAVES * 2];
    __shared__ float s_xyz[2][FPS_K * 3];
    __shared__ unsigned s_prog[2];
    const int bi = batch0 + blockIdx.y, wg = blockIdx.x;
    xyz += (size_t)bi * n * 3;
    idxs += (size_t)bi * m;
    slots += (size_t)bi * 2 * FPS_MAXG * FPS_KPUB;
    const int lane = threadIdx.x & 63, wid = threadIdx.x >> 6;
    const bool holder = (wid & 3) != 0;
    const int hid = wid - 1 - (wid >> 2);
    const int gtid = (wg * FPS_PW + hid) * 64 + lane;
    const int stride = G * FPS_PW * 64;
    if (threadIdx.x < 2) s_prog[threadIdx.x] = 0u;
    if (!holder && lane < 4) s_part[lane >> 1][wid * 2 + (lane & 1)] = 0ull;

    float px[P], py[P], pz[P], tmp[P];
    unsigned key[P];
    unsigned elig = 0;
    const unsigned bs_mask = (1u << bs_log2) - 1u;
#pragma unroll
    for (int i = 0; i < P; i++) {
        const int k = gtid + i * stride;
        px[i] = py[i] = pz[i] = 0.f;
        tmp[i] = 1e10f;
        key[i] = FPS_KEY_NONE;
        if (holder && k < n) {
            px[i] = xyz[(size_t)k * 3 + 0];
            py[i] = xyz[(size_t)k * 3 + 1];
            pz[i] = xyz[(size_t)k * 3 + 2];
            const float mag = fmaf(pz[i], pz[i], fmaf(py[i], py[i], px[i] * px[i]));
            if (!((double)mag <= 1e-3)) elig |= 1u << i;
            const unsigned rev = bs_log2 ? (__brev((unsigned)k & bs_mask) >> (32 - bs_log2)) : 0u;
            key[i] = (rev << 22) | (unsigned)k;
        }
    }
    if (m0 <= 0 && wg == 0 && threadIdx.x == 0) idxs[0] = 0;
    int nnew = 1;
    float nx[FPS_K], ny[FPS_K], nz[FPS_K];
    nx[0] = xyz[0]; ny[0] = xyz[1]; nz[0] = xyz[2];
#pragma unroll
    for (int a = 1; a < FPS_K; a++) nx[a] = ny[a] = nz[a] = 0.f;
    int done = 1;
    if (m0 > 1) {
        for (int base = 0; base < m0 - 1; base += FPS_K) {
            const int cntk = min(FPS_K, m0 - 1 - base);
#pragma unroll
            for (int a = 0; a < FPS_K; a++) {
                const int pi = a < cntk ? idxs[base + a] : 0;
                nx[a] = xyz[(size_t)pi * 3 + 0];
                ny[a] = xyz[(size_t)pi * 3 + 1];
                nz[a] = xyz[(size_t)pi * 3 + 2];
            }
#pragma unroll
            for (int i = 0; i < P; i++) {
                if (elig & (1u << i)) {
                    float d2 = tmp[i];
#pragma unroll
                    for (int a = 0; a < FPS_K; a++) {
                        if (a < cntk) {
                            const float dx = px[i] - nx[a], dy = py[i] - ny[a], dz = pz[i] - nz[a];
                            d2 = fminf(fmaf(dz, dz, fmaf(dy, dy, dx * dx)), d2);
                        }
                    }
                    tmp[i] = d2;
                }
            }
        }
        const int pl = idxs[m0 - 1];
        nx[0] = xyz[(size_t)pl * 3 + 0];
        ny[0] = xyz[(size_t)pl * 3 + 1];
        nz[0] = xyz[(size_t)pl * 3 + 2];
        done = m0;
    }
#ifdef FPS_TRACE
    unsigned long long ftr[10] = {0, 0, 0, 0, 0, 0, 0, 0, 0, 0};
#endif
    if (holder) {
#pragma unroll
        for (int i = 0; i < P; i++) {
            if (elig & (1u << i)) {
                const float dx = px[i] - nx[0], dy = py[i] - ny[0], dz = pz[i] - nz[0];
                tmp[i] = fminf(fmaf(dz, dz, fmaf(dy, dy, dx * dx)), tmp[i]);
            }
        }
    } else {
        __builtin_amdgcn_s_setprio(3);
    }
    __syncthreads();
    for (int round = 1; done < m; round++) {
        const int par = round & 1;
        const unsigned long long ft0 = FT();
        unsigned bd = 0u, bk = FPS_KEY_NONE;
#pragma unroll
        for (int i = 0; i < P; i++) {
            if (elig & (1u << i)) {
                float d2 = tmp[i];
                const unsigned db = __float_as_uint(d2);
                if (db > bd || (db == bd && key[i] < bk)) {
                    bd = db;
                    bk = key[i];
                }
            }
        }
        const unsigned long long ft1 = FT();
        FTA(0, ft0, ft1);
        if (holder) {
        unsigned d1 = bd, k1 = bk;
        wave_best(d1, k1);
        unsigned cd = bd, ck = bk;
        if (bk == k1 && k1 != FPS_KEY_NONE) {
            cd = 0u;
            ck = FPS_KEY_NONE;
#pragma unroll
            for (int i = 0; i < P; i++) {
                if ((elig & (1u << i)) && key[i] != k1) {
                    const unsigned db = __float_as_uint(tmp[i]);
                    if (db > cd || (db == cd && key[i] < ck)) {
                        cd = db;
                        ck = key[i];
                    }
                }
            }
        }
        unsigned d2w = cd, k2w = ck;
        wave_best(d2w, k2w);
        if (lane == 0) {
            unsigned long long c1 = fps_code(d1, k1), c2 = fps_code(d2w, k2w);
            if (c2 != 0ull) c2 |= 1ull;
            else if (c1 != 0ull) c1 |= 1ull;
            s_part[par][wid * 2 + 0] = c1;
            s_part[par][wid * 2 + 1] = c2;
        }
        }
        const unsigned long long ft2 = FT();
        FTA(1, ft1, ft2);
        __syncthreads();
        const unsigned long long ft3 = FT();
        FTA(2, ft2, ft3);
        if (wid == 0) {
            unsigned long long mine = lane < FPS_WAVES * 2 ? s_part[par][lane] : 0ull;
            unsigned long long wgc[FPS_KPUB];
            bool stop = false;
            int cnt = 0;
            fps_static_for<0, FPS_KPUB>([&](auto tc) {
                constexpr int t = decltype(tc)::value;
                const unsigned long long best = stop ? 0ull : wave_max_u64(mine);
                wgc[t] = best & ~1ull;
                if (best != 0ull) {
                    if (mine == best) mine = 0ull;
                    if (best & 1ull) stop = true;
                    cnt = t + 1;
// ... 33 lines not shown
#pragma unroll
                    for (int j = 0; j < FPS_NG; j++) {
                        if (!ok[j]) {
                            v[j] = __hip_atomic_load(rs + lane + 64 * j, __ATOMIC_RELAXED, __HIP_MEMORY_SCOPE_AGENT);
                            ok[j] = (v[j] & FPS_TAG) == tag;
                            all = all && ok[j];
                        }
                    }
                    if (++spins > FPS_SPIN_LIMIT) {
                        *err = 1;
                        break;
                    }
                }
#pragma unroll
                for (int j = 0; j < FPS_NG; j++) v[j] = (lane + 64 * j < G * FPS_KPUB) ? (v[j] & ~FPS_TAG) : 0ull;
            }
            const unsigned long long ft5 = FT();
            FTA(4, ft4, ft5);
            float vx[FPS_NG], vy[FPS_NG], vz[FPS_NG];
#pragma unroll
            for (int j = 0; j < FPS_NG; j++) {
                const int ci = fps_code_index(v[j]);
                vx[j] = xyz[(size_t)ci * 3 + 0];
                vy[j] = xyz[(size_t)ci * 3 + 1];
                vz[j] = xyz[(size_t)ci * 3 + 2];
            }
            static_assert(FPS_NG == 1, "one gathered candidate per lane");
#ifdef FPS_TRACE
            {
                float probe = vx[0];
                asm volatile("v_mov_b32 %0, %0" : "+v"(probe));
                vx[0] = probe;
            }
#endif
            const unsigned long long ft6 = FT();
            FTA(5, ft5, ft6);
            const unsigned long long mine0 = v[0];
            const unsigned long long Bcode = wave_max_u64((mine0 & 1ull) ? (mine0 & ~1ull) : 0ull);
            unsigned ckey = (unsigned)((mine0 >> 1) & 0x7fffffffull);
            float cdist = __uint_as_float((unsigned)(mine0 >> 32));
            bool alive = mine0 != 0ull;
            int nacc = 0;
            float kx = 0.f, ky = 0.f, kz = 0.f;
            int kidx = 0;
            bool direct = false;
            const unsigned clo = ckey << 1;
            const unsigned Bhi = (unsigned)(Bcode >> 32), Blo = (unsigned)Bcode;
            auto take = [&](int ol, unsigned best_lo, int t) {
                const float bx = __int_as_float(__builtin_amdgcn_readlane(__float_as_int(vx[0]), ol));
                const float by = __int_as_float(__builtin_amdgcn_readlane(__float_as_int(vy[0]), ol));
                const float bz = __int_as_float(__builtin_amdgcn_readlane(__float_as_int(vz[0]), ol));
                const bool keeper = lane == t;
                kx = keeper ? bx : kx;
                ky = keeper ? by : ky;
                kz = keeper ? bz : kz;
                kidx = keeper ? (int)((FPS_KEY_NONE - ((best_lo >> 1) & 0x7fffffffu)) & 0x3fffffu) : kidx;
                if (lane == ol) alive = false;
                if (lane == 0) {
                    FPS_LDS_ST(&s_xyz[par][t * 3 + 0], bx);
                    FPS_LDS_ST(&s_xyz[par][t * 3 + 1], by);
                    FPS_LDS_ST(&s_xyz[par][t * 3 + 2], bz);
                    FPS_ORDER();
                    FPS_LDS_ST(&s_prog[par], ((unsigned)round << 8) | (unsigned)(t + 1));
                }
                const float dx = vx[0] - bx, dy = vy[0] - by, dz = vz[0] - bz;
                cdist = fminf(cdist, fmaf(dz, dz, fmaf(dy, dy, dx * dx)));
            };
            {
                const unsigned long long my = alive ? (((unsigned long long)__float_as_uint(cdist) << 32) | clo) : 0ull;
                const unsigned long long best = wave_max_u64(my);
                if (best == 0ull) {
                    if (lane == 0) {
                        FPS_LDS_ST(&s_xyz[par][0], xyz[0]);
                        FPS_LDS_ST(&s_xyz[par][1], xyz[1]);
                        FPS_LDS_ST(&s_xyz[par][2], xyz[2]);
                        if (wg == 0) idxs[done] = 0;
                    }
                    direct = true;
                } else {
                    take(__builtin_ctzll(__ballot(alive && my == best)), (unsigned)best, 0);
                }
                nacc = 1;
            }
            if (!direct) {
#pragma unroll 1
                for (int t = 1; t < FPS_K && done + t < m; t++) {
                    const unsigned hi = alive ? __float_as_uint(cdist) : 0u;
                    const unsigned md = wave_max_u32(hi);
                    if (md == 0u) break;
                    const unsigned long long owners = __ballot(hi == md);
                    int ol;
                    unsigned blo;
                    if (__popcll(owners) == 1) {
                        ol = __builtin_ctzll(owners);
                        blo = (unsigned)__builtin_amdgcn_readlane((int)clo, ol);
                    } else {
                        blo = wave_max_u32(hi == md ? clo : 0u);
                        ol = __builtin_ctzll(__ballot(hi == md && clo == blo));
                    }
                    if (md < Bhi || (md == Bhi && blo < Blo)) break;
                    take(ol, blo, t);
                    nacc = t + 1;
                }
            }
            if (!direct && lane < nacc && wg == 0) idxs[done + lane] = kidx;
            FPS_ORDER();
            if (lane == 0) FPS_LDS_ST(&s_prog[par], ((unsigned)round << 8) | 0x80u | (unsigned)nacc);
            nnew = nacc;
            (void)kx; (void)ky; (void)kz;
            const unsigned long long ft7 = FT();
            FTA(6, ft6, ft7);
        }
        else if (holder) {
            const unsigned tag = (unsigned)round << 8;
            int seen = 0;
            for (;;) {
                const unsigned c = FPS_LDS_LD(&s_prog[par]);
                FPS_ORDER();
                const bool cur = (c & 0xffffff00u) == tag;
                const int cnt = cur ? (int)(c & 0x7fu) : 0;
                for (int a = seen; a < cnt; a++) {
                    const float ax = FPS_LDS_LD(&s_xyz[par][a * 3 + 0]), ay = FPS_LDS_LD(&s_xyz[par][a * 3 + 1]),
                                az = FPS_LDS_LD(&s_xyz[par][a * 3 + 2]);
                    fps_absorb<P>(px, py, pz, tmp, ax, ay, az);
                }
                seen = cnt;
                if (cur && (c & 0x80u)) break;
                __builtin_amdgcn_s_sleep(FPS_POLL_SLEEP);
            }
            nnew = seen;
        } else {
            const unsigned tag = (unsigned)round << 8;
            unsigned c;
            for (;;) {
                c = FPS_LDS_LD(&s_prog[par]);
                if ((c & 0xffffff80u) == (tag | 0x80u)) break;
                __builtin_amdgcn_s_sleep(32);
            }
            nnew = (int)(c & 0x7fu);
        }
        done += nnew;
#ifdef FPS_TRACE
        ftr[8] += 1;
        ftr[9] += nnew;
#endif
    }
#ifdef FPS_TRACE
    if (g_fps_trace && wg == 0 && threadIdx.x == 0)
        for (int i = 0; i < 10; i++) g_fps_trace[i] = ftr[i];
#endif
}

template <int P>
static void launch_fps(int G, int nb, hipStream_t st, const float* xyz, int n, int m, int m0, int bs_log2, int batch0,
                       unsigned long long* slots, int32_t* idxs, int* err) {
    GF_LAUNCH_OP(GF_OP_FPS, (k_fps<P>), dim3(G, nb), dim3(FPS_WAVES * 64), 0, st, xyz, n, m, m0, G, bs_log2, batch0, slots,
                 idxs, err);
}

extern "C" size_t gf_fps_scratch_bytes(int b) {
    return ((size_t)b * 2 * FPS_MAXG * FPS_KPUB + 8) * sizeof(unsigned long long);
}

extern "C" int gf_furthest_point_sampling_resume(const float* xyz, int b, int n, int m, int m_known, int32_t* idxs,
                                                 void* scratch, void* stream);

extern "C" int gf_furthest_point_sampling(const float* xyz, int b, int n, int m, int32_t* idxs, void* scratch,
                                          void* stream) {
    return gf_furthest_point_sampling_resume(xyz, b, n, m, 0, idxs, scratch, stream);
}

extern "C" int gf_furthest_point_sampling_resume(const float* xyz, int b, int n, int m, int m_known, int32_t* idxs,
                                                 void* scratch, void* stream) {
    GF_CHECK_ARG(b >= 0 && n >= 1 && m >= 0, "gf_furthest_point_sampling: bad sizes b=%d n=%d m=%d", b, n, m);
    GF_CHECK_ARG(m_known >= 0 && m_known <= m, "gf_furthest_point_sampling_resume: m_known=%d not in [0, m=%d]", m_known,
                 m);
    if (m_known == m && m > 0) return GF_OK;
    GF_CHECK_ARG(n < (1 << 22), "gf_furthest_point_sampling: n=%d exceeds the 22-bit index of the tie-break key", n);
    if (b == 0 || m == 0) return GF_OK;
    hipStream_t st = (hipStream_t)stream;
    int bs_log2 = 0;
    while ((2 << bs_log2) <= n && bs_log2 < 9) bs_log2++;
    const int per_wg = FPS_PW * 64;
    int G = (2 * n + per_wg * 5 - 1) / (per_wg * 5);
    if (G < 1) G = 1;
    if (G > FPS_MAXG) G = FPS_MAXG;
    const int P = (n + G * per_wg - 1) / (G * per_wg);
    GF_CHECK_ARG(P <= 22, "gf_furthest_point_sampling: n=%d too large (max %d)", n, FPS_MAXG * per_wg * 22);
    unsigned long long* slots = (unsigned long long*)scratch;
    int* err = (int*)(slots + (size_t)b * 2 * FPS_MAXG * FPS_KPUB);
    GF_TRY(hipMemsetAsync(scratch, 0, gf_fps_scratch_bytes(b), st));
    const int per_launch = 1024 / (G * FPS_WAVES) > 0 ? 1024 / (G * FPS_WAVES) : 1;
    for (int b0 = 0; b0 < b; b0 += per_launch) {
        const int nb = (b - b0) < per_launch ? (b - b0) : per_launch;
        if (P <= 1) launch_fps<1>(G, nb, st, xyz, n, m, m_known, bs_log2, b0, slots, idxs, err);
        else if (P <= 2) launch_fps<2>(G, nb, st, xyz, n, m, m_known, bs_log2, b0, slots, idxs, err);
        else if (P <= 3) launch_fps<3>(G, nb, st, xyz, n, m, m_known, bs_log2, b0, slots, idxs, err);
        else if (P <= 4) launch_fps<4>(G, nb, st, xyz, n, m, m_known, bs_log2, b0, slots, idxs, err);
        else if (P <= 5) launch_fps<5>(G, nb, st, xyz, n, m, m_known, bs_log2, b0, slots, idxs, err);
        else if (P <= 6) launch_fps<6>(G, nb, st, xyz, n, m, m_known, bs_log2, b0, slots, idxs, err);
        else if (P <= 8) launch_fps<8>(G, nb, st, xyz, n, m, m_known, bs_log2, b0, slots, idxs, err);
        else if (P <= 12) launch_fps<12>(G, nb, st, xyz, n, m, m_known, bs_log2, b0, slots, idxs, err);
        else if (P <= 16) launch_fps<16>(G, nb, st, xyz, n, m, m_known, bs_log2, b0, slots, idxs, err);
        else if (P <= 20) launch_fps<20>(G, nb, st, xyz, n, m, m_known, bs_log2, b0, slots, idxs, err);
        else launch_fps<22>(G, nb, st, xyz, n, m, m_known, bs_log2, b0, slots, idxs, err);
    }
    GF_CHECK_LAUNCH("gf_furthest_point_sampling");
    return GF_OK;
}
```

geoformer_amd/model/geoformer.py:

```python
from __future__ import annotations

import functools
import os

import numpy as np
import torch
import torch.nn as nn
from torch.nn import functional as F

from .. import _lib, pointops, spconv, unet_exec, unet_train
from . import config as _config
from .backbone import ResidualBlock, UBlock, conv1d_bn_relu, random_downsample
from .layers import (BatchNorm1d, BigLinear, GenericMLP, LazyRelPos, PointwiseConv1d, PositionEmbeddingCoordsSine, RelPosSpec,
                     TransformerDecoder,
                     TransformerDecoderLayer, scene_counts)
from .set_abstraction import PointnetSAModuleVotesSeparate


class _Voxelization(torch.autograd.Function):

    @staticmethod
    def forward(ctx, feats, map_rule, mode=4):
        ctx.rule, ctx.mode, ctx.N = map_rule, mode, feats.shape[0]
        return pointops.voxelize_fp(feats.contiguous(), map_rule, mode)

    @staticmethod
    def backward(ctx, d_out):
        d_feats = torch.zeros((ctx.N, d_out.shape[1]), dtype=torch.float32, device=d_out.device)
        pointops.voxelize_bp(d_out.contiguous(), ctx.rule, ctx.mode, d_feats)
        return d_feats, None, None


voxelization = _Voxelization.apply


import threading
import weakref


def _bfs_wg(nq, scenes=1):
    return 1024 if nq * scenes <= 224 else 512
_SIDE_STREAMS = {}
_OFFS_CACHE = threading.local()


def get_batch_offsets(batch_idxs, bs, host_only=False):
    if bs == 1:
        n = int(batch_idxs.shape[0])
        t = torch.tensor([0, n], dtype=torch.int32, device="cpu" if host_only else batch_idxs.device)
        _OFFS_CACHE.key, _OFFS_CACHE.val = t, [0, n]
        return t
    counts = scene_counts(batch_idxs, bs)
    return torch.cat([counts.new_zeros(1), counts.cumsum(0)]).int()



def _offsets_list(t):
    if getattr(_OFFS_CACHE, "key", None) is t:
        return _OFFS_CACHE.val
    lru = getattr(_OFFS_CACHE, "lru", None)
    if lru is None:
        lru = _OFFS_CACHE.lru = {}
    hit = lru.get(id(t))
    if hit is not None and hit[0]() is t and hit[1] == t._version:
        return hit[2]
    val = t.tolist()
    if len(lru) > 64:
        lru.clear()
    lru[id(t)] = (weakref.ref(t), t._version, val)
    return val


def _tensors_of(obj):
    if torch.is_tensor(obj):
        yield obj
    elif isinstance(obj, (tuple, list)):
        for o in obj:
            yield from _tensors_of(o)


@torch.no_grad()
def knn_graphs(locs_float_, batch_offsets_, batch_size, neighbor=64, radius=0.05):
    offs = _offsets_list(batch_offsets_)
    return [pointops.knn_radius(locs_float_[offs[b]:offs[b + 1]].contiguous(), neighbor, radius, sqrt_out=True,
                                return_flag=True)
            for b in range(batch_size)]


def knn_truncated(graphs):
    fl = [g[3] for g in (graphs or ()) if len(g) > 3]
    return torch.stack([f.reshape(()) for f in fl]).amax().reshape(1) if fl else None


@torch.no_grad()
def cal_geodesic(pre_enc_inds, locs_float_, batch_offsets_, max_step=128, neighbor=64, radius=0.05, n_queries=128,
                 graphs=None):
    if graphs is None:
        graphs = knn_graphs(locs_float_, batch_offsets_, pre_enc_inds.shape[0], neighbor, radius)
    out = []
    for b in range(pre_enc_inds.shape[0]):
        D, I, deg = graphs[b][:3]
        src = pre_enc_inds[b][:n_queries].int().contiguous()
        out.append(pointops.geodesic_bfs(D, I, deg, src, radius, max_step))
    return out


def _stream_key_of(device, stream):
    idx = torch.device(device).index
    return (torch.cuda.current_device() if idx is None else idx, stream.cuda_stream)


def _stream_key(device=None):
    raw = getattr(torch._C, "_cuda_getCurrentRawStream", None)
    if raw is not None:
        idx = torch.cuda.current_device() if device is None else torch.device(device).index
        if idx is None:
            idx = torch.cuda.current_device()
        return (idx, raw(idx))
    st = torch.cuda.current_stream(device)
    return (st.device.index, st.cuda_stream)


class PendingProposals:

    _pinned = []
    _lock = threading.Lock()

    def __init__(self, final, cls_pred, scores, logits, fg_idxs, logit_thresh, num_points, knn_flags=()):
        self.stream = torch.cuda.current_stream(logits.device)
        sel, cls, sc, cnt = pointops.proposal_select(final.contiguous(), cls_pred.contiguous(), scores.contiguous())
        self.args = (sel, cls, sc, logits, fg_idxs, logit_thresh, num_points)
        with PendingProposals._lock:
            buf = PendingProposals._pinned.pop() if PendingProposals._pinned else None
        if buf is None:
            buf = torch.zeros(2, dtype=torch.int32).pin_memory()
        buf[1] = 0
        buf[0:1].copy_(cnt, non_blocking=True)
        for f in knn_flags:
            buf[1:2].copy_(f, non_blocking=True)
        self.host = buf
        self.done = torch.cuda.Event()
        self.done.record(self.stream)
        self.value = None
        self.home = None

    def get(self):
        if self.value is None:
            sel, cls, sc, logits, fg_idxs, logit_thresh, num_points = self.args
            _lib.timed_wait(self.done)
            n, overflow = int(self.host[0]), int(self.host[1])
            with PendingProposals._lock:
                PendingProposals._pinned.append(self.host)
            self.host = None
            if overflow:
                from .._lib import GeoFormerHipError

                raise GeoFormerHipError("kNN graph: a point has more in-radius neighbours than the kernel's candidate list "
                                        "holds (1024); its row is not the 64 nearest and the geodesic distances "
                                        "would be wrong -- deduplicate the scene's points")
            if n == 0:
                self.value = ([], [], [])
            else:
                with torch.cuda.stream(self.stream):
                    proposals = pointops.proposal_scatter(logits, sel[:n], fg_idxs, logit_thresh, num_points)
                self.value = (cls[:n], sc[:n], proposals)
                if self.home is not None:
                    cur = torch.cuda.current_stream(logits.device)
                    if cur.cuda_stream != self.stream.cuda_stream:
                        ev = torch.cuda.Event()
                        ev.record(self.stream)
                        cur.wait_event(ev)
                        for t in self.value:
                            t.record_stream(cur)
            self.args = None
        return self.value


class PendingBatchProposals:

    def __init__(self, n_scenes, scene_ids=(), table=None, sel=None, cls=None, scores=None, counts=None, fg_idxs=None,
                 logit_thresh=0.5, num_points=(), max_N=0, knn_flags=(), value=None):
        self.value = value
        if value is not None:
            return
        self.n_scenes, self.scene_ids, self.num_points, self.max_N = n_scenes, list(scene_ids), list(num_points), max_N
        self.args = (table, sel, cls, scores, counts, fg_idxs, logit_thresh)
        S = len(self.scene_ids)
        self.stream = torch.cuda.current_stream(sel.device)
        self.host = torch.zeros(S + 1, dtype=torch.int32).pin_memory()
        self.host[:S].copy_(counts, non_blocking=True)
        for f in knn_flags:
            self.host[S:S + 1].copy_(f, non_blocking=True)
        self.done = torch.cuda.Event()
        self.done.record(self.stream)
# ... 209 lines not shown
        return self._preprocess(batch_input, batch_size)

    def _preprocess(self, batch_input, batch_size):
        feats = batch_input["feats"]
        if self.cfg.use_coords:
            feats = torch.cat((feats, batch_input["locs_float"]), 1).float()
        voxel_feats = voxelization(feats, batch_input["v2p_map"], self.cfg.mode)
        return spconv.SparseConvTensor(voxel_feats, batch_input["voxel_locs"].int().contiguous(), batch_input["spatial_shape"],
                                       batch_size)

    def _inputs_ahead(self, batch_input):
        evs = batch_input.get("inputs_event") if isinstance(batch_input, dict) else None
        locs = batch_input["voxel_locs"]
        if evs is None or not locs.is_cuda or torch.is_grad_enabled() or os.environ.get("GF_UNET_EXEC", "1") == "0":
            return None
        if unet_exec.phase_pending():
            return None
        main = torch.cuda.current_stream(locs.device)
        if main.query():
            return None
        return main, unet_exec.side_stream_for(locs.device, main), list(evs)

    def unet_features(self, x, batch_size):
        if os.environ.get("GF_UNET_EXEC", "1") != "0" and unet_exec.supported(self, x.features, x.spatial_shape):
            x.features = unet_exec.unet_forward(self, x.features.contiguous(), x._coords(), batch_size, x.spatial_shape)
            return x
        if unet_exec.take_coords_ready() is not None:
            torch.cuda.current_stream().wait_stream(unet_exec.side_stream_for(x.features.device))
        sig = unet_train.supported(self, x)
        if sig:
            feats = unet_train.unet_forward(self, x, batch_size, sig)
            if feats is not None:
                x.features = feats
                return x
        x.indice_dict["_prebuild"] = self.prebuild_rulebooks
        return self.output_layer(self.unet(self.input_conv(x)))

    def forward_backbone(self, batch_input, batch_size, want_preds=True):
        ctx = self._grad_ctx("unet")
        with ctx():
            x = self.unet_features(self.preprocess_input(batch_input, batch_size), batch_size)
            return self._semantic_head(x, batch_input, want_preds)

    def _semantic_head(self, x, batch_input, want_preds):
        p2v = batch_input["p2v_map"]
        if not want_preds and p2v.dtype == torch.int32 and p2v.is_contiguous():
            vox = x.features.contiguous()
            chain = self._pointwise_chain("semantic", [self.semantic, self.semantic_linear], vox)
            if chain is not None:
                return (vox, p2v), pointops.pointwise_mlp(vox, chain, rows=p2v), None
        output_feats = pointops.points_from_voxels(x.features, p2v, batch_input.get("v2p_map")).contiguous()
        chain = self._pointwise_chain("semantic", [self.semantic, self.semantic_linear], output_feats)
        if chain is not None:
            semantic_scores = pointops.pointwise_mlp(output_feats, chain)
        else:
            semantic_scores = self.semantic_linear(self.semantic(output_feats))
        semantic_preds = semantic_scores.max(1)[1] if want_preds else None
        return output_feats, semantic_scores, semantic_preds

    @staticmethod
    def prebuild_rulebooks(x, nlevels=6):
        from .. import sparse

        if not x.features.is_cuda or x.indices.shape[0] == 0:
            return
        coords = x._coords()
        chain = sparse.down_rules_chain(coords, x.batch_size, x.spatial_shape, nlevels)
        cur = coords
        for l, r in enumerate(chain):
            r.prebuilt_for = cur.data_ptr()
            x.indice_dict[f"spconv{l + 1}"] = r
            cur = r.out_coords

    def _mask_tower_rows(self, feats):
        if not (feats.is_cuda and torch.is_grad_enabled() and feats.dim() == 2 and feats.dtype == torch.float32
                and os.environ.get("GF_FUSED_BN", "1") != "0"):
            return None
        from .layers import _SplitKLinearFn

        mods = list(self.mask_tower)
        x = feats.contiguous()
        last = mods[-1]
        if not (isinstance(last, nn.Conv1d) and last.kernel_size == (1,)):
            return None
        for mod in mods[:-1]:
            if not (isinstance(mod, nn.Sequential) and len(mod) == 3 and isinstance(mod[0], nn.Conv1d)
                    and mod[0].kernel_size == (1,) and mod[0].bias is None and isinstance(mod[2], nn.ReLU)
                    and isinstance(mod[1], nn.BatchNorm1d) and mod[1].num_features == mod[0].out_channels
                    and pointops.bn_relu_train_supported(
                        mod[1], x if mod[0].out_channels == x.shape[1] else x.new_empty((x.shape[0], mod[0].out_channels)))):
                return None
        for mod in mods[:-1]:
            x = pointops.bn_relu_train(mod[1], _SplitKLinearFn.apply(x, mod[0].weight[:, :, 0], None))
        return _SplitKLinearFn.apply(x, last.weight[:, :, 0], last.bias).unsqueeze(2)

    def forward_aggregator(self, locs_float_, output_feats_, batch_offsets_, batch_size):
        ctx = self._grad_ctx("set_aggregator")
        offs = _offsets_list(batch_offsets_)
        with ctx():
            locs, gfeat, gxyz, inds = [], [], [], []
            for b in range(batch_size):
                n_b = offs[b + 1] - offs[b]
                if n_b == 0:
                    return None
                npoint = min(n_b, self.cfg.n_downsampling)
                draw = pointops.legacy_choice(n_b, npoint) if locs_float_.is_cuda else \
                    np.random.choice(n_b, npoint, replace=False)
                sampling_indices = torch.tensor(draw, dtype=torch.long, device=locs_float_.device)
                self.last_sampling_indices = sampling_indices
                xyz_b = locs_float_[offs[b]:offs[b + 1]][sampling_indices].unsqueeze(0)
                feat_b = output_feats_[offs[b]:offs[b + 1]][sampling_indices].unsqueeze(0)
                l, gf, gx, idx = self.set_aggregator.group_points(xyz_b.contiguous(),
                                                                  feat_b.transpose(1, 2).contiguous())
                locs.append(l); gfeat.append(gf); gxyz.append(gx); inds.append(idx)
            context_locs, pre_enc_inds = torch.cat(locs), torch.cat(inds)
            context_feats = self.set_aggregator.mlp(torch.cat(gfeat), torch.cat(gxyz)).transpose(1, 2)
            return context_locs, context_feats, pre_enc_inds

    def _sampling_split(self):
        nq = self.cfg.n_query_points
        npoint_sa = self.set_aggregator.npoint
        return nq, npoint_sa, os.environ.get("GF_OVERLAP", "1") != "2" and npoint_sa > nq

    def _first_picks(self, xyz_b, sb, first=None, xyz_ready=None):
        nq, npoint_sa, split = self._sampling_split()
        if xyz_ready is None:
            xyz_ready = torch.cuda.Event()
            xyz_ready.record(sb)
        if first is None:
            first = pointops.furthest_point_sampling(xyz_b, nq if split else npoint_sa)
        src = first[0, :nq].contiguous()
        first_ready = torch.cuda.Event()
        first_ready.record(sb)
        idx = pointops.furthest_point_sampling(xyz_b, npoint_sa, known=first) if split else first
        fps_done = torch.cuda.Event()
        fps_done.record(sb)
        return xyz_ready, first, src, first_ready, idx, fps_done

    def _sample_from_count(self, n, locs_rows, bufs):
        npoint = min(n, self.cfg.n_downsampling)
        drawn = pointops.draw_sample(n, npoint, locs_rows, bufs)
        if drawn is None:
            return None
        sampling_indices, xyz_b = drawn[:2]
        sb = torch.cuda.current_stream()
        if len(drawn) == 3:
            first_ready = torch.cuda.Event()
            first_ready.record(sb)
            return (sampling_indices, xyz_b) + self._first_picks(xyz_b, sb, first=drawn[2], xyz_ready=first_ready)
        return (sampling_indices, xyz_b) + self._first_picks(xyz_b, sb)

    def _aggregate_geodesic_overlapped(self, locs_float_, output_feats_, batch_offsets_, batch_size, graphs, max_step,
                                       pc_dims=None, sample=True, epilogue=True, early=None, presampled=None,
                                       presampled_before=None):
        offs = _offsets_list(batch_offsets_)
        grad_ctx = self._grad_ctx("set_aggregator")
        nq, npoint_sa, split = self._sampling_split()
        main = torch.cuda.current_stream()
        sides = _SIDE_STREAMS
        side = sides.get((locs_float_.device, main.cuda_stream))
        if side is None:
            side = torch.cuda.Stream(device=locs_float_.device)
            sides[(locs_float_.device, main.cuda_stream)] = side
        aux = sides.get((locs_float_.device, main.cuda_stream, "aux"))
        if aux is None:
            aux = sides[(locs_float_.device, main.cuda_stream, "aux")] = torch.cuda.Stream(device=locs_float_.device)
        geo_ready = [None] * batch_size
        staged, geo = [None] * batch_size, [None] * batch_size
        fps_done_evs = []
        multi = batch_size > 1 and early is None and not epilogue
        scene_streams = []
        def host_draw(b, n_b):
            npoint = min(n_b, self.cfg.n_downsampling)
            pins = getattr(_OFFS_CACHE, "draw_pins", None)
            if pins is None:
                pins = _OFFS_CACHE.draw_pins = {}
            pin = pins.get((main.cuda_stream, b))
            if pin is None or pin.numel() < npoint:
                pin = pins[(main.cuda_stream, b)] = torch.empty(max(npoint, 65536), dtype=torch.int64).pin_memory()
            drawn = pointops.legacy_choice(n_b, npoint, out=pin.numpy())
            if drawn.ctypes.data != pin.data_ptr():
                pin.numpy()[:npoint] = drawn
            return pin, npoint

        order = list(range(batch_size))
        draws = {}
        if multi:
            for b in order:
                if offs[b + 1] - offs[b] == 0:
                    return None, None
                if sample:
                    draws[b] = host_draw(b, offs[b + 1] - offs[b])
            order.sort(key=lambda b: -(offs[b + 1] - offs[b]))
        for b in order:
            n_b = offs[b + 1] - offs[b]
            if n_b == 0:
                return None, None
            if multi:
                sb = sides.get((locs_float_.device, main.cuda_stream, "scene", b))
                if sb is None:
                    sb = sides[(locs_float_.device, main.cuda_stream, "scene", b)] = torch.cuda.Stream(device=locs_float_.device)
                side_b = sides.get((locs_float_.device, main.cuda_stream, "bfs", b))
                if side_b is None:
                    side_b = sides[(locs_float_.device, main.cuda_stream, "bfs", b)] = torch.cuda.Stream(device=locs_float_.device)
                sb.wait_stream(main)
                scene_streams.append(sb)
            else:
                sb, side_b = main, side
            with torch.cuda.stream(sb):
                if presampled is not None and b == 0 and not multi and sample:
                    sampling_indices, xyz_b, xyz_ready, first, src, first_ready, idx, fps_done = presampled
                    self.last_sampling_indices = sampling_indices
                else:
                    if sample:
                        pin, npoint = draws[b] if b in draws else host_draw(b, n_b)
                        sampling_indices = pin[:npoint].to(locs_float_.device, non_blocking=True)
                        self.last_sampling_indices = sampling_indices
                        xyz_b = locs_float_[offs[b]:offs[b + 1]][sampling_indices].unsqueeze(0).contiguous()
                    else:
                        sampling_indices = None
                        xyz_b = locs_float_[offs[b]:offs[b + 1]].unsqueeze(0).contiguous()
                    xyz_ready, first, src, first_ready, idx, fps_done = self._first_picks(xyz_b, sb)
                fps_done_evs.append(fps_done)
                picks_ready = first_ready
            if early is not None and b == 0:
                aux.wait_event(presampled_before if presampled_before is not None else xyz_ready)
                with torch.cuda.stream(aux):
                    graphs = early(True)
                    for t in _tensors_of(graphs):
                        t.record_stream(main)
                        t.record_stream(side)
                    graphs_done = torch.cuda.Event()
                    graphs_done.record(aux)
                side.wait_event(graphs_done)
            side_b.wait_event(first_ready)
            with torch.cuda.stream(side_b):
                D, I, deg = graphs[b][:3]
                g = pointops.geodesic_bfs(D, I, deg, src, 0.05, max_step,
                                          wg_threads=_bfs_wg(int(src.shape[0]), batch_size) if split else 1024)
                g.record_stream(main)
                src.record_stream(side_b)
                geo[b] = g
                ev = torch.cuda.Event()
                ev.record(side_b)
                geo_ready[b] = ev
            if early is not None and b == 0:
                with torch.cuda.stream(aux):
                    early_out = tuple(early(False)) + (graphs,)
                    for t in _tensors_of(early_out[:2]):
                        t.record_stream(main)
                        t.record_stream(side)
                    early_done = torch.cuda.Event()
                    early_done.record(aux)
            grid = None
            if xyz_b.shape[1] >= 4096 and not torch.is_grad_enabled():
                aux.wait_event(xyz_ready)
                with torch.cuda.stream(aux):
                    xyz_b.record_stream(aux)
                    grid = pointops.point_grid_build(xyz_b, self.set_aggregator.radius)
                    grid.record_stream(main)
                    grid_done = torch.cuda.Event()
                    grid_done.record(aux)
                grid = (grid, grid_done)
            if multi:
                for t in (xyz_b, idx, first, sampling_indices):
                    if t is not None:
                        t.record_stream(main)
            if early is not None and b == 0:
                main.wait_event(early_done)
            staged[b] = [xyz_b, None, idx, grid, sampling_indices]
            if not epilogue:
                continue
            self._side_epilogue(b, batch_size, g, xyz_b, src, pc_dims, main, side, aux, picks_ready)
        for sb in scene_streams:
            main.wait_stream(sb)
        with grad_ctx():
            for b, st in enumerate(staged):
                feat_b = output_feats_[offs[b]:offs[b + 1]]
                if st[4] is not None:
                    feat_b = pointops.take_rows_unique(feat_b, st[4])
                st[1] = feat_b.unsqueeze(0).transpose(1, 2).contiguous()
        staged = [tuple(st[:4]) for st in staged]
        self.__dict__.setdefault("_gf_pending_side", {})[_stream_key(locs_float_.device)] = geo_ready
        self.__dict__.setdefault("_gf_stretch_events", {})[_stream_key(locs_float_.device)] = fps_done_evs + [
            ev for ev in geo_ready if ev is not None]
        cat = lambda ts: ts[0] if len(ts) == 1 else torch.cat(ts)
        with grad_ctx():
            fused = []
            for xyz_b, feat_b, idx, grid in staged:
                if grid is not None:
                    main.wait_event(grid[1])
                fused.append(self.set_aggregator.fused_forward(xyz_b, feat_b, idx, grid=None if grid is None else grid[0]))
            if all(f is not None for f in fused):
                context_locs, pre_enc_inds = cat([f[0] for f in fused]), cat([st[2] for st in staged])
                context_feats = cat([f[1] for f in fused]).transpose(1, 2)
                res = ((context_locs, context_feats, pre_enc_inds), geo)
                return res + (early_out,) if early is not None else res
            locs, gfeat, gxyz, inds = [], [], [], []
            for xyz_b, feat_b, idx, _ in staged:
                l, gf, gx, idx = self.set_aggregator.group_points(xyz_b, feat_b, inds=idx)
                locs.append(l); gfeat.append(gf); gxyz.append(gx); inds.append(idx)
            context_locs, pre_enc_inds = cat(locs), cat(inds)
            context_feats = self.set_aggregator.mlp(cat(gfeat), cat(gxyz)).transpose(1, 2)
        res = ((context_locs, context_feats, pre_enc_inds), geo)
        return res + (early_out,) if early is not None else res

    def _side_epilogue(self, b, batch_size, g, xyz_b, src, pc_dims, main, side, aux, first_ready):
        early = self._early()
        if b == 0:
            early.clear()
        with torch.cuda.stream(side):
            mx = torch.max(g, dim=1)[0]
            mx = torch.sqrt(torch.where(mx < 0, torch.max(mx), mx)).contiguous()
            mx.record_stream(main)
            ev = torch.cuda.Event()
            ev.record(side)
            early[("mx", b)] = (g, mx, ev)
        if batch_size == 1 and pc_dims is not None and self.cfg.dec_dim == 64:
            aux.wait_event(first_ready)
            with torch.cuda.stream(aux):
                qpr = self._pointwise_chain("qproj", [self.query_projection], xyz_b)
                if qpr is not None:
                    xyz_b.record_stream(aux)
                    q_locs = xyz_b[:, src.long()]
                    qpe = self.pos_embedding(q_locs, input_range=pc_dims).float()
                    qpos = pointops.pointwise_mlp(qpe[0].t().contiguous(), qpr)
                    qpos.record_stream(main)
                    src.record_stream(aux)
                    ev = torch.cuda.Event()
                    ev.record(aux)
                    early["qpos"] = (q_locs, qpos, ev)

    def _early(self):
        if not torch.cuda.is_available():
            return {}
        return self.__dict__.setdefault("_gf_early", {}).setdefault(_stream_key(), {})

    def _join_side_stream(self):
        pend = self.__dict__.get("_gf_pending_side")
        if pend and torch.cuda.is_available():
            for ev in pend.pop(_stream_key(), None) or ():
                torch.cuda.current_stream().wait_event(ev)

    def relative_position_embedding(self, context_locs, query_locs, pc_dims, geo_dists, pre_enc_inds):
        B = context_locs.shape[0]
        self._join_side_stream()
        if context_locs.is_cuda and self.cfg.dec_dim == 64 and (not torch.is_grad_enabled()
                                                                 or os.environ.get("GF_FUSED_BWD", "1") != "0"):
            if B == 1 and pre_enc_inds.dtype == torch.int32:
                g1, m1 = pointops.relpos_prepare(geo_dists[0].contiguous(), pre_enc_inds[0].contiguous())
                geo, max_geo = g1.unsqueeze(0), m1.unsqueeze(0)
            elif B > 1 and pre_enc_inds.stride(0) == 0 and all(g is geo_dists[0] for g in geo_dists):
                g1 = geo_dists[0][:, pre_enc_inds[0].long()]
                m1 = torch.max(g1, dim=1)[0]
                m1 = torch.where(m1 < 0, torch.max(m1), m1)
                geo, max_geo = g1.unsqueeze(0).expand(B, -1, -1).contiguous(), m1.unsqueeze(0).expand(B, -1).contiguous()
            else:
                geo = torch.stack([geo_dists[b][:, pre_enc_inds[b].long()] for b in range(B)], dim=0).contiguous()
                max_geo = torch.max(geo, dim=2)[0]
                max_geo = torch.where(max_geo < 0, torch.max(max_geo), max_geo).contiguous()
            return RelPosSpec(geo, max_geo, query_locs.contiguous(), context_locs.contiguous(),
                              pc_dims[0].float().contiguous(), pc_dims[1].float().contiguous(),
                              self.pos_embedding.gauss_B.contiguous())
        rel = torch.abs(query_locs[:, :, None, :] - context_locs[:, None, :, :])
        nq, nc = rel.shape[1], rel.shape[2]
        geo = torch.stack([geo_dists[b][:, pre_enc_inds[b].long()] for b in range(B)], dim=0)
        max_geo = torch.max(geo, dim=2)[0]
        max_all = torch.max(max_geo)
        max_geo = torch.where(max_geo < 0, max_all, max_geo)
        geo3 = geo[:, :, :, None].repeat(1, 1, 1, 3)
        geo3 = torch.where(geo3 < 0, max_geo[:, :, None, None] + rel, geo3)
        emb = self.pos_embedding(geo3.reshape(B, nq * nc, -1), input_range=pc_dims).reshape(B, -1, nq, nc)
        return emb.permute(2, 3, 0, 1)

    def forward_decoder(self, context_locs, context_feats, query_locs, pc_dims, geo_dists, pre_enc_inds):
        nq = self.cfg.n_query_points
        if context_locs.shape[0] == 1 and context_locs.is_cuda and not torch.is_grad_enabled():
            e2d = self._pointwise_chain("e2d", [self.encoder_to_decoder_projection], context_feats)
            qpr = self._pointwise_chain("qproj", [self.query_projection], context_feats)
            if e2d is not None and qpr is not None:
                ctx = pointops.pointwise_mlp(context_feats[0].contiguous(), e2d)
                rel = LazyRelPos(lambda: self.relative_position_embedding(context_locs, query_locs, pc_dims, geo_dists,
                                                                          pre_enc_inds))
                hit = self._early().pop("qpos", None)
                if hit is not None and hit[0].shape == query_locs.shape:
                    torch.cuda.current_stream().wait_event(hit[2])
                    qpos = hit[1]
                else:
                    qpe = self.pos_embedding(query_locs, input_range=pc_dims).float()
                    qpos = pointops.pointwise_mlp(qpe[0].t().contiguous(), qpr)
                memory = ctx.unsqueeze(1)
                return self.decoder(tgt=memory[:nq], memory=memory, pos=None, query_pos=qpos.unsqueeze(1),
                                    relative_pos=rel)
        context_embedding_pos = self.pos_embedding(context_locs, input_range=pc_dims)
        context_feats = self.encoder_to_decoder_projection(context_feats.permute(0, 2, 1))
        query_embedding_pos = self.query_projection(self.pos_embedding(query_locs, input_range=pc_dims).float())
        dec_inputs = context_feats[:, :, :nq].permute(2, 0, 1)
        relative_embedding_pos = self.relative_position_embedding(context_locs, query_locs, pc_dims, geo_dists,
                                                                  pre_enc_inds)
        return self.decoder(tgt=dec_inputs, memory=context_feats.permute(2, 0, 1),
                            pos=context_embedding_pos.permute(2, 0, 1), query_pos=query_embedding_pos.permute(2, 0, 1),
                            relative_pos=relative_embedding_pos)

    def parse_dynamic_params(self, params, out_channels):
        n = params.size(0)
        w1, w2, b1, b2 = torch.split_with_sizes(params, self.weight_nums + self.bias_nums, dim=1)
        return ([w1.reshape(n * out_channels, -1, 1), w2.reshape(n, -1, 1)],
                [b1.reshape(n * out_channels), b2.reshape(n)])

    def mask_heads_forward(self, geo_dist, mask_features, weights, biases, num_insts, coords_, fps_sampling_coords,
                           use_geo=True):
        n_mask = mask_features.size(0)
        if (mask_features.is_cuda and self.output_dim == 16 and not torch.is_grad_enabled()):
            mx = None
            if use_geo:
                early = self._early()
                hit = next((early.pop(k) for k in list(early) if k[0] == "mx" and early[k][0] is geo_dist), None)
                if hit is not None:
                    torch.cuda.current_stream().wait_event(hit[2])
                    mx = hit[1]
                else:
                    mx = torch.max(geo_dist, dim=1)[0]
                    mx = torch.sqrt(torch.where(mx < 0, torch.max(mx), mx)).contiguous()
            od = self.output_dim
            logits = pointops.mask_head(
                mask_features.reshape(n_mask, od).contiguous(), coords_.contiguous(),
                geo_dist.contiguous() if use_geo else None, fps_sampling_coords.reshape(-1, 3).contiguous(), mx,
                weights[0].reshape(num_insts, od, od + 3).contiguous(), biases[0].reshape(num_insts, od).contiguous(),
                weights[1].reshape(num_insts, od).contiguous(), biases[1].reshape(num_insts).contiguous())
            return logits.reshape(1, num_insts, n_mask)
        rel = fps_sampling_coords.reshape(-1, 1, 3) - coords_.reshape(1, -1, 3)
        if use_geo:
            mx = torch.max(geo_dist, dim=1)[0]
            mx = torch.sqrt(torch.where(mx < 0, torch.max(mx), mx))
            rel = torch.where((geo_dist < 0).unsqueeze(-1), rel + mx[:, None, None] * torch.sign(rel), rel)
        w1, w2 = weights[0].reshape(num_insts, self.output_dim, -1), weights[1].reshape(num_insts, 1, -1)
        b1, b2 = biases[0].reshape(num_insts, self.output_dim, 1), biases[1].reshape(num_insts, 1, 1)
        feat = mask_features.reshape(n_mask, -1)
        h = torch.matmul(w1[:, :, :3], rel.permute(0, 2, 1)) + torch.matmul(w1[:, :, 3:], feat.t().unsqueeze(0)) + b1
        x = torch.matmul(w2, F.relu(h)) + b2
        return x.reshape(1, num_insts, n_mask)

    def _mask_head_packed(self, geo_dist, mask_features, params, num_insts, coords_, fps_sampling_coords):
        n_mask = mask_features.size(0)
        early = self._early()
        hit = next((early.pop(k) for k in list(early) if k[0] == "mx" and early[k][0] is geo_dist), None)
        if hit is not None:
            torch.cuda.current_stream().wait_event(hit[2])
            mx = hit[1]
        else:
            mx = torch.max(geo_dist, dim=1)[0]
            mx = torch.sqrt(torch.where(mx < 0, torch.max(mx), mx)).contiguous()
        logits = pointops.mask_head_packed(mask_features.reshape(n_mask, self.output_dim).contiguous(),
                                           coords_.contiguous(), geo_dist.contiguous(),
                                           fps_sampling_coords.reshape(-1, 3).contiguous(), mx, params.contiguous())
        return logits.reshape(1, num_insts, n_mask)

    def get_mask_prediction(self, geo_dists, param_kernels, mask_features, locs_float_, fps_sampling_locs,
                            batch_offsets_):
        num_layers, n_queries, batch = param_kernels.shape[:3]
        offs = _offsets_list(batch_offsets_)
        outputs = []
        fused_train = (mask_features.is_cuda and torch.is_grad_enabled() and self.output_dim == 16 and self.use_coords
                       and os.environ.get("GF_FUSED_BWD", "1") != "0")
        per_scene, train_ctrl = {}, {}
        if fused_train:
# ... 112 lines not shown
        cls_scores = torch.gather(cls_prob, 1, cls_pred.unsqueeze(-1)).squeeze(-1)
        sem_scores = torch.matmul(mask_bool.float(), sem_b) / (npts[:, None] + 1e-6)
        sem_scores = torch.gather(sem_scores, 1, cls_pred.unsqueeze(-1)).squeeze(-1)
        scores = mask_scores * torch.pow(cls_scores, 0.5) * sem_scores
        final = (cls_pred >= 4) & (npts >= npoint_thresh) & (mask_scores >= score_thresh)
        if torch.count_nonzero(final) == 0:
            return [], [], []
        masks_final = mask_bool[final]
        proposals = torch.zeros((masks_final.shape[0], num_points), dtype=torch.int, device=mask_prob.device)
        inst, pts = torch.nonzero(masks_final, as_tuple=True)
        proposals[inst, fg_idxs[pts]] = 1
        return cls_pred[final], scores[final], proposals

    def generate_proposals_batched(self, mask_logits, cls_logits, fg_idxs, batch_offsets, fg_offsets, scene_ids,
                                   n_scenes, sem_prob, logit_thresh=0.5, score_thresh=0.5, npoint_thresh=100,
                                   defer=False, knn_flags=()):
        from .. import postprocess

        offs = _offsets_list(batch_offsets)
        logits = [ml.contiguous() for ml in mask_logits]
        nq = logits[0].shape[0]
        starts = [offs[b] for b in scene_ids]
        npts = [offs[b + 1] - offs[b] for b in scene_ids]
        sem_t = sem_prob[1] if isinstance(sem_prob, tuple) else sem_prob.t().contiguous()
        table = postprocess.proposal_scene_table([t.data_ptr() for t in logits], fg_offsets, starts, npts)
        table_d = pointops._table_dev(table, fg_idxs.device)
        cls_pred, _, scores, final = pointops.proposal_stats_batched(table_d, nq, cls_logits.contiguous(), sem_t,
                                                                     logit_thresh, score_thresh, npoint_thresh,
                                                                     min_class=4)
        sel, cls, sc, counts = pointops.proposal_select_batched(final, cls_pred, scores)
        pending = PendingBatchProposals(n_scenes, scene_ids, table_d, sel, cls, sc, counts, fg_idxs.contiguous(),
                                        logit_thresh, npts, int(table[:, 1].max()), knn_flags)
        pending.keep = logits
        return pending if defer else pending.get()

    def forward(self, batch_input, epoch, training=True, defer_proposals=False, all_scenes=False):
        if all_scenes and (training or not batch_input["locs_float"].is_cuda):
            raise ValueError("forward(all_scenes=True) is the batched eval forward on the GPU (training=False)")
        steps = self._forward_steps(batch_input, epoch, training, defer_proposals, False, all_scenes)
        try:
            while True:
                next(steps)
        except StopIteration as done:
            return done.value

    def forward_split(self, batch_input, epoch, training=True, defer_proposals=False):
        return SplitForward(self._forward_steps(batch_input, epoch, training, defer_proposals, True))

    def _forward_steps(self, batch_input, epoch, training, defer_proposals, split, all_scenes=False):
        cfg = self.cfg
        outputs = {}
        batch_idxs = batch_input["locs"][:, 0].int()
        locs_float = batch_input["locs_float"]
        batch_offsets = batch_input["offsets"]
        batch_size = len(batch_offsets) - 1
        assert batch_size > 0
        pc_dims = [batch_input["pc_maxs"], batch_input["pc_mins"]]

        fused_fg = (locs_float.is_cuda and not torch.is_grad_enabled() and epoch > self.prepare_epochs
                    and locs_float.dtype == torch.float32)
        output_feats, semantic_scores, semantic_preds = self.forward_backbone(batch_input, batch_size,
                                                                              want_preds=not fused_fg)
        outputs["semantic_scores"] = semantic_scores
        if epoch <= self.prepare_epochs:
            return outputs
        same_fold = cfg.train_fold == cfg.cvfold
        fg_pending = None
        if fused_fg:
            feats_src, feat_rows = output_feats if isinstance(output_feats, tuple) else (output_feats.contiguous(), None)
            fg_pending = pointops.select_foreground(
                semantic_scores.contiguous(), 4 if same_fold else 3, not same_fold, locs_float.contiguous(),
                batch_idxs.contiguous(), feats_src, feat_rows, deferred=True)
        if split:
            backbone_done = torch.cuda.Event() if locs_float.is_cuda else None
            if backbone_done is not None:
                backbone_done.record()
            yield backbone_done
        if fused_fg:
            presampled = None
            from_count = (batch_size == 1 and not training and cfg.n_downsampling
                          and os.environ.get("GF_OVERLAP", "1") != "0")
            if batch_size == 1 and locs_float.is_cuda and cfg.n_downsampling and epoch > self.prepare_epochs:
                pointops.legacy_prefetch(int(1.4 * locs_float.shape[0]) + 4096)
                if from_count:
                    nq_, npoint_sa_, split_ = self._sampling_split()
                    draw_bufs = pointops.draw_sample_buffers(int(cfg.n_downsampling), int(locs_float.shape[0]),
                                                             locs_float.device, fps_m=nq_ if split_ else npoint_sa_)
                    draw_bufs["before"] = fg_pending.done
            n_fg = fg_pending.wait()
            if from_count and n_fg > 0:
                presampled = self._sample_from_count(n_fg, fg_pending.bufs[1], draw_bufs)
            fg_idxs, locs_float_, batch_idxs_, output_feats_, semantic_scores_ = fg_pending.views()
        else:
            fg = semantic_preds >= 4 if same_fold else semantic_preds == 3
            fg_idxs = torch.nonzero(fg).view(-1)
        agree = self.rank_agreement if (training and torch.is_grad_enabled()) else None
        if len(fg_idxs) == 0:
            if agree is not None:
                agree(False, locs_float.device)
            outputs["mask_predictions"] = None
            if all_scenes:
                empty = [([], [], []) for _ in range(batch_size)]
                outputs["proposal_scores_per_scene"] = PendingBatchProposals(batch_size, value=empty) \
                    if defer_proposals else empty
            return outputs
        if not fused_fg:
            batch_idxs_ = batch_idxs[fg_idxs]
            locs_float_ = locs_float[fg_idxs]
            output_feats_ = pointops.take_rows_unique(output_feats, fg_idxs)
            semantic_scores_ = semantic_scores[fg_idxs]
        batch_offsets_ = get_batch_offsets(batch_idxs_, batch_size, host_only=fused_fg and not training)
        offs_ = _offsets_list(batch_offsets_)
        nonempty = min(offs_[b + 1] - offs_[b] for b in range(batch_size)) > 0
        n_scenes, scene_ids = batch_size, list(range(batch_size))
        if all_scenes and not nonempty:
            scene_ids = [b for b in range(batch_size) if offs_[b + 1] > offs_[b]]
            offs_ = [offs_[b] for b in scene_ids] + [offs_[-1]]
            batch_offsets_ = torch.tensor(offs_, dtype=torch.int32, device=batch_offsets_.device)
            pc_dims = [pc_dims[0][scene_ids], pc_dims[1][scene_ids]]
            batch_size, nonempty = len(scene_ids), True
        if agree is not None and not agree(nonempty, locs_float.device):
            outputs["mask_predictions"] = None
            return outputs

        def sampling_independent(graphs_only=None):
            if graphs_only is True:
                return knn_graphs(locs_float_, batch_offsets_, batch_size, neighbor=64, radius=0.05)
            chain = self._pointwise_chain("mask_tower", [self.mask_tower], output_feats_)
            if chain is not None:
                mf = pointops.pointwise_mlp(output_feats_.contiguous(), chain).unsqueeze(2)
            else:
                mf = self._mask_tower_rows(output_feats_)
                if mf is None:
                    mf = self.mask_tower(output_feats_.unsqueeze(2).permute(2, 1, 0)).permute(2, 1, 0)
            sp = None
            if not training:
                sp = F.softmax(semantic_scores_, dim=1)
                if sp.is_cuda:
                    sp = (sp, sp.t().contiguous())
            if graphs_only is False:
                return mf, sp
            gr = None
            if locs_float_.is_cuda and nonempty:
                gr = knn_graphs(locs_float_, batch_offsets_, batch_size, neighbor=64, radius=0.05)
            return mf, sp, gr

        max_step = 128 if self.training else 256
        geo_dists = None
        overlap = locs_float_.is_cuda and nonempty and os.environ.get("GF_OVERLAP", "1") != "0"
        if overlap and fused_fg and not training:
            contexts, geo_dists, (mask_features_, sem_prob, graphs) = self._aggregate_geodesic_overlapped(
                locs_float_, output_feats_, batch_offsets_, batch_size, None, max_step, pc_dims, epilogue=True,
                early=sampling_independent, presampled=presampled if fused_fg else None,
                presampled_before=draw_bufs["before"] if (fused_fg and presampled is not None) else None)
        else:
            mask_features_, sem_prob, graphs = sampling_independent()
            if graphs is not None and overlap:
                contexts, geo_dists = self._aggregate_geodesic_overlapped(locs_float_, output_feats_, batch_offsets_,
                                                                          batch_size, graphs, max_step, pc_dims,
                                                                          epilogue=not torch.is_grad_enabled())
            else:
                contexts = self.forward_aggregator(locs_float_, output_feats_, batch_offsets_, batch_size)
        if contexts is None:
            outputs["mask_predictions"] = None
            return outputs
        context_locs, context_feats, pre_enc_inds = contexts
        query_locs = context_locs[:, :cfg.n_query_points, :]

        if geo_dists is None:
            geo_dists = cal_geodesic(pre_enc_inds, locs_float_, batch_offsets_, max_step=max_step, neighbor=64,
                                     radius=0.05, n_queries=cfg.n_query_points, graphs=graphs)
        if split:
            stretch = []
            if locs_float.is_cuda:
                stretch = list(self.__dict__.get("_gf_stretch_events", {}).pop(_stream_key(locs_float.device), ()))
                if not stretch:
                    ev = torch.cuda.Event()
                    ev.record()
                    stretch = [ev]
            yield stretch
        dec_outputs = self.forward_decoder(context_locs, context_feats, query_locs, pc_dims, geo_dists, pre_enc_inds)
        self._join_side_stream()

        if training:
            idxs_sub, idxs_sub_raw = random_downsample(batch_offsets_, batch_size, n_subsample=30000,
                                                         host_offsets=_offsets_list(batch_offsets_))
            geo_sub = [geo_dists[b][:, idxs_sub_raw[b]] for b in range(batch_size)]
            del geo_dists
            batch_idxs_sub = batch_idxs_[idxs_sub]
            offsets_sub = get_batch_offsets(batch_idxs_sub, batch_size)
            outputs["fg_idxs"] = fg_idxs[idxs_sub]
            outputs["num_insts"] = cfg.n_query_points * batch_size
            outputs["batch_idxs"] = batch_idxs_sub
            outputs["n_fg_total"] = int(offs_[-1])
            trunc = knn_truncated(graphs)
            if trunc is not None:
                outputs["knn_truncated"] = trunc
            outputs["mask_predictions"] = self.get_mask_prediction(geo_sub, dec_outputs,
                                                                   pointops.take_rows_unique(mask_features_, idxs_sub),
                                                                   locs_float_[idxs_sub], query_locs, offsets_sub)
        else:
            dec_outputs = dec_outputs[-1:, ...]
            outputs["fg_idxs"] = fg_idxs
            outputs["num_insts"] = cfg.n_query_points * batch_size
            outputs["batch_idxs"] = batch_idxs_
            preds = self.get_mask_prediction(geo_dists, dec_outputs, mask_features_, locs_float_, query_locs,
                                             batch_offsets_)
            outputs["mask_predictions"] = preds
            if all_scenes:
                outputs["proposal_scores_per_scene"] = self.generate_proposals_batched(
                    preds[-1]["mask_logits"], preds[-1]["cls_logits"], fg_idxs, batch_offsets, offs_, scene_ids,
                    n_scenes, sem_prob, logit_thresh=0.5, score_thresh=cfg.TEST_SCORE_THRESH,
                    npoint_thresh=cfg.TEST_NPOINT_THRESH, defer=defer_proposals,
                    knn_flags=[f for f in (knn_truncated(graphs),) if f is not None])
            else:
                outputs["proposal_scores"] = self.generate_proposal(
                    preds[-1]["mask_logits"], preds[-1]["cls_logits"], fg_idxs, batch_offsets, batch_offsets_,
                    semantic_scores_=semantic_scores_, logit_thresh=0.5, score_thresh=cfg.TEST_SCORE_THRESH,
                    npoint_thresh=cfg.TEST_NPOINT_THRESH, sem_prob=sem_prob, defer=defer_proposals,
                    knn_flags=[f for f in (knn_truncated(graphs),) if f is not None])
        if locs_float.is_cuda:
            self._early().clear()
        return outputs
```

geoformer_amd/pointops.py:

```python
from __future__ import annotations

import contextlib
import os
import threading

import numpy as np
import torch

from . import _lib
from ._lib import check, ptr, stream_ptr


def _f32c(t, name):
    if not (t.is_cuda and t.dtype == torch.float32 and t.is_contiguous()):
        raise RuntimeError(f"{name}: expected a contiguous float32 tensor on the GPU")
    return t


def _i32c(t, name):
    if not (t.is_cuda and t.dtype == torch.int32 and t.is_contiguous()):
        raise RuntimeError(f"{name}: expected a contiguous int32 tensor on the GPU")
    return t


# ... 194 lines not shown

    bg = np.random.mtrand._rand._bit_generator
    hit = _LEGACY_STATE.get(id(bg))
    if hit is None or hit[0] is not bg:
        addr = None
        if type(bg).__name__ == "MT19937":
            try:
                a = int(bg.ctypes.state_address)
                st = np.random.get_state()
                key = np.ctypeslib.as_array((ctypes.c_uint32 * 624).from_address(a))
                if st[0] == "MT19937" and int(ctypes.c_int.from_address(a + 2496).value) == int(st[2]) and \
                        bool((key == np.asarray(st[1], dtype=np.uint32)).all()):
                    addr = a
            except Exception:
                addr = None
        _LEGACY_STATE.clear()
        hit = _LEGACY_STATE[id(bg)] = (bg, addr)
    return None if hit[1] is None else (hit[1], bg.lock)


def legacy_prefetch(nwords):
    import ctypes

    import numpy as np

    direct = _legacy_state()
    if direct is not None:
        addr, lock = direct
        with lock:
            check(_lib.load().gf_host_legacy_prefetch(addr, int(ctypes.c_int.from_address(addr + 2496).value), int(nwords)),
                  "gf_host_legacy_prefetch")
        return
    st = np.random.get_state()
    if st[0] != "MT19937":
        return
    key = np.ascontiguousarray(st[1], dtype=np.uint32)
    check(_lib.load().gf_host_legacy_prefetch(key.ctypes.data, int(st[2]), int(nwords)), "gf_host_legacy_prefetch")


_DRAW_PINS = {}


def draw_sample_buffers(kmax, n_cap, device, fps_m=0):
    key = (device.index, stream_ptr())
    pin = _DRAW_PINS.get(key)
    if pin is None or pin.numel() < max(n_cap, kmax):
        pin = _DRAW_PINS[key] = torch.empty(max(n_cap + n_cap // 4, kmax, 65536), dtype=torch.int32).pin_memory()
    bufs = {"pin": pin, "idx32": torch.empty(kmax, dtype=torch.int32, device=device),
            "idx64": torch.empty(kmax, dtype=torch.int64, device=device),
            "xyz": torch.empty((1, kmax, 3), dtype=torch.float32, device=device), "kmax": kmax, "fps_m": 0}
    if fps_m > 0:
        bufs["fps_m"] = int(fps_m)
        bufs["fps_idx"] = torch.empty((1, int(fps_m)), dtype=torch.int32, device=device)
        bufs["fps_scratch"] = torch.empty(_lib.load().gf_fps_scratch_bytes(1) // 8 + 1, dtype=torch.int64, device=device)
    return bufs


def draw_sample(n, k, xyz_src, bufs):
    n, k = int(n), int(k)
    direct = _legacy_state() if 1 <= k <= n <= 0x7fffffff and k <= bufs["kmax"] else None
    if direct is None:
        return None
    _f32c(xyz_src, "xyz_src")
    addr, lock = direct
    pin = bufs["pin"]
    fps_m = bufs["fps_m"] if 0 < bufs["fps_m"] <= k else 0
    with lock:
        check(_lib.load().gf_host_draw_sample(addr, addr + 2496, n, k, pin.data_ptr(), pin.numel(), ptr(bufs["idx32"]),
                                              ptr(bufs["idx64"]), ptr(xyz_src), ptr(bufs["xyz"]), fps_m,
                                              ptr(bufs["fps_idx"]) if fps_m else None,
                                              ptr(bufs["fps_scratch"]) if fps_m else None, stream_ptr()),
              "gf_host_draw_sample")
    if fps_m:
        return bufs["idx64"][:k], bufs["xyz"][:, :k], bufs["fps_idx"]
    return bufs["idx64"][:k], bufs["xyz"][:, :k]


def legacy_choice(n, k, out=None):
    import ctypes

    import numpy as np

    n, k = int(n), int(k)
    direct = _legacy_state() if 1 <= k <= n <= 0x7fffffff else None
    if direct is not None:
        addr, lock = direct
        if out is None or out.dtype != np.int64 or out.size < k or not out.flags.c_contiguous:
            out = np.empty(k, dtype=np.int64)
        with lock:
            check(_lib.load().gf_host_legacy_choice(addr, addr + 2496, n, k, out.ctypes.data), "gf_host_legacy_choice")
        return out[:k]
    st = np.random.get_state()
    if st[0] != "MT19937" or not (1 <= k <= n <= 0x7fffffff):
        return np.random.choice(n, k, replace=False)
    key = np.ascontiguousarray(st[1], dtype=np.uint32).copy()
    pos = ctypes.c_int32(int(st[2]))
    if out is None or out.dtype != np.int64 or out.size < k or not out.flags.c_contiguous:
        out = np.empty(k, dtype=np.int64)
    check(_lib.load().gf_host_legacy_choice(key.ctypes.data, ctypes.addressof(pos), n, k, out.ctypes.data),
          "gf_host_legacy_choice")
    np.random.set_state((st[0], key, int(pos.value), st[3], st[4]))
    return out[:k]


def knn_radius(xyz, k, radius, sqrt_out=True, check_overflow=False, return_flag=False):
    _f32c(xyz, "xyz")
    n = xyz.shape[0]
    lib = _lib.load()
    dev = xyz.device
    D = torch.empty((n, k), dtype=torch.float32, device=dev)
    I = torch.empty((n, k), dtype=torch.int32, device=dev)
    deg = torch.empty(n, dtype=torch.int32, device=dev)
    scratch = torch.empty(lib.gf_knn_scratch_bytes(n) // 4 + 16, dtype=torch.int32, device=dev)
    check(lib.gf_knn_radius(ptr(xyz), n, k, float(radius), int(sqrt_out), ptr(D), ptr(I), ptr(deg), ptr(scratch),
                            stream_ptr()), "gf_knn_radius")
    if check_overflow:
        off = (lib.gf_knn_error_flag(ptr(scratch), n) - scratch.data_ptr()) // 4
        if int(scratch[off].item()) != 0:
            raise _lib.GeoFormerHipError("gf_knn_radius: a point has more in-radius neighbours than the kernel's "
                                         "candidate list holds (rows truncated)")
    if return_flag:
        off = (lib.gf_knn_error_flag(ptr(scratch), n) - scratch.data_ptr()) // 4
        return D, I, deg, scratch[off:off + 1]
    return D, I, deg


_SCRATCH = {}


def scratch(name, numel, dtype, device):
    dev = torch.device(device)
    key = (dev.index if dev.index is not None else torch.cuda.current_device(), torch.cuda.current_stream(dev).cuda_stream,
           name, dtype)
    t = _SCRATCH.get(key)
    if t is None or t.numel() < numel:
        _SCRATCH[key] = None
        t = _SCRATCH[key] = torch.empty(int(numel * 1.25) + 64, dtype=dtype, device=dev)
    return t[:numel]


def release_scratch(device=None):
    if device is not None:
        dev = torch.device(device)
        idx = dev.index if dev.index is not None else torch.cuda.current_device()
    for key in list(_SCRATCH):
        if device is None or key[0] == idx:
            del _SCRATCH[key]


def scratch_bytes():
    return sum(t.numel() * t.element_size() for t in _SCRATCH.values() if t is not None)


def geodesic_bfs(D, I, deg, src, radius, max_step, wg_threads=1024):
    _f32c(D, "D"); _i32c(I, "I"); _i32c(src, "src")
    n, K = D.shape
    nq = src.shape[0]
    dev = D.device
    geo = torch.empty((nq, n), dtype=torch.float32, device=dev)
    lib = _lib.load()
    keys = scratch("bfs_keys", nq * n, torch.int64, dev)
    qwords = int(lib.gf_geodesic_bfs_queue_words(n))
    queues = scratch("bfs_queues", nq * qwords, torch.int32, dev)
    check(lib.gf_geodesic_bfs_cfg(ptr(D), ptr(I), ptr(deg), n, K, ptr(src), nq, float(radius), int(max_step),
                                          ptr(geo), ptr(keys), ptr(queues), qwords, int(wg_threads), stream_ptr()),
          "gf_geodesic_bfs")
    return geo


def _mask_head_split_ws(N, device, split):
    if not split:
        return None
    return scratch("mask_head_split", _lib.load().gf_mask_head_split_bytes(N) // 8 + 1, torch.int64, device)


def mask_head(feat, coords, geo, qxyz, sqrt_max_geo, w1, b1, w2, b2, split=True):
    for t, name in ((feat, "feat"), (coords, "coords"), (qxyz, "qxyz"), (w1, "w1"), (b1, "b1"), (w2, "w2"), (b2, "b2")):
        _f32c(t, name)
    N, C = feat.shape
    nq = qxyz.shape[0]
    out = torch.empty((nq, N), dtype=torch.float32, device=feat.device)
    check(_lib.load().gf_mask_head_episodes(ptr(feat), ptr(coords), ptr(geo), ptr(qxyz), ptr(sqrt_max_geo), ptr(w1), ptr(b1),
                                            ptr(w2), ptr(b2), 0, N, nq, 1, C, ptr(_mask_head_split_ws(N, feat.device, split)),
                                            ptr(out), stream_ptr()), "gf_mask_head")
    return out


def mask_head_packed(feat, coords, geo, qxyz, sqrt_max_geo, params, split=True):
    return mask_head_episodes(feat, coords, geo, qxyz, sqrt_max_geo, params.unsqueeze(0), split=split)[0]


def mask_head_episodes(feat, coords, geo, qxyz, sqrt_max_geo, params, split=True):
    for t, name in ((feat, "feat"), (coords, "coords"), (qxyz, "qxyz"), (params, "params")):
        _f32c(t, name)
    N, C = feat.shape
    E, nq, ld = params.shape
    if ld != C * (C + 3) + C + C + 1 or qxyz.shape[0] != nq:
        raise RuntimeError(f"mask_head_episodes: params {tuple(params.shape)} for {qxyz.shape[0]} queries, C={C}")
    base = params.data_ptr()
    o_w2, o_b1, o_b2 = C * (C + 3), C * (C + 3) + C, C * (C + 3) + 2 * C
    out = torch.empty((E, nq, N), dtype=torch.float32, device=feat.device)
    check(_lib.load().gf_mask_head_episodes(ptr(feat), ptr(coords), ptr(geo), ptr(qxyz), ptr(sqrt_max_geo), base,
                                            base + 4 * o_b1, base + 4 * o_w2, base + 4 * o_b2, ld, N, nq, E, C,
                                            ptr(_mask_head_split_ws(N, feat.device, split)), ptr(out), stream_ptr()),
          "gf_mask_head_episodes")
    return out


class _MaskHeadFn(torch.autograd.Function):

    @staticmethod
    def forward(ctx, feat, params, coords, geo, qxyz, sqrt_max_geo):
        ctx.save_for_backward(feat, params, coords, geo, qxyz, sqrt_max_geo)
        return mask_head_packed(feat, coords, geo, qxyz, sqrt_max_geo, params)

    @staticmethod
    def backward(ctx, gout):
        feat, params, coords, geo, qxyz, mx = ctx.saved_tensors
        N, C = feat.shape
        nq, ld = params.shape
        lib = _lib.load()
        dparams = torch.empty_like(params)
        dfeat = torch.zeros_like(feat)
        scratch = torch.empty(lib.gf_mask_head_bwd_scratch_floats(N, nq), dtype=torch.float32, device=feat.device)
        base = params.data_ptr()
        o_w2, o_b1 = C * (C + 3), C * (C + 3) + C
        check(lib.gf_mask_head_bwd(ptr(feat), ptr(coords), ptr(geo), ptr(qxyz), ptr(mx), base, base + 4 * o_b1,
                                   base + 4 * o_w2, ptr(gout.contiguous()), ld, N, nq, C, ptr(dparams), ptr(dfeat),
                                   ptr(scratch), stream_ptr()), "gf_mask_head_bwd")
        return dfeat, dparams, None, None, None, None


class _MaskHeadEpisodesFn(torch.autograd.Function):

    @staticmethod
    def forward(ctx, feat, params, coords, geo, qxyz, sqrt_max_geo):
        ctx.save_for_backward(feat, params, coords, geo, qxyz, sqrt_max_geo)
        return mask_head_episodes(feat, coords, geo, qxyz, sqrt_max_geo, params)

    @staticmethod
    def backward(ctx, gout):
        feat, params, coords, geo, qxyz, mx = ctx.saved_tensors
        N, C = feat.shape
        E, nq, ld = params.shape
        lib = _lib.load()
        dparams = torch.empty_like(params)
        dfeat = torch.zeros_like(feat)
        scratch = torch.empty(lib.gf_mask_head_bwd_scratch_floats(N, E * nq), dtype=torch.float32, device=feat.device)
        base = params.data_ptr()
        o_w2, o_b1 = C * (C + 3), C * (C + 3) + C
        check(lib.gf_mask_head_bwd_episodes(ptr(feat), ptr(coords), ptr(geo), ptr(qxyz), ptr(mx), base, base + 4 * o_b1,
                                            base + 4 * o_w2, ptr(gout.contiguous()), ld, N, nq, E, C, ptr(dparams),
                                            ptr(dfeat), ptr(scratch), stream_ptr()), "gf_mask_head_bwd_episodes")
        return dfeat, dparams, None, None, None, None


def mask_head_train_episodes(feat, params, coords, geo, qxyz, sqrt_max_geo):
    for t, name in ((feat, "feat"), (coords, "coords"), (qxyz, "qxyz"), (params, "params")):
        _f32c(t, name)
    return _MaskHeadEpisodesFn.apply(feat, params, coords, geo, qxyz, sqrt_max_geo)


def mask_head_train(feat, params, coords, geo, qxyz, sqrt_max_geo):
    for t, name in ((feat, "feat"), (coords, "coords"), (qxyz, "qxyz"), (params, "params")):
        _f32c(t, name)
    return _MaskHeadFn.apply(feat, params, coords, geo, qxyz, sqrt_max_geo)


class PointwiseChain:

    def __init__(self, modules):
        import ctypes

        layers = []
        for m in modules:
            name = type(m).__name__
            if isinstance(m, (torch.nn.Linear, torch.nn.Conv1d, torch.nn.Conv2d)):
                W = m.weight.detach()
                W = W.reshape(W.shape[0], W.shape[1]).float().contiguous()
                bias = m.bias.detach().float() if m.bias is not None else torch.zeros(W.shape[0], device=W.device)
                layers.append([W, torch.ones_like(bias), bias.clone(), 0])
            elif isinstance(m, torch.nn.modules.batchnorm._BatchNorm):
                if m.training:
                    raise RuntimeError("PointwiseChain folds eval-mode BatchNorm only")
                s = (m.weight / torch.sqrt(m.running_var + m.eps)).detach().float()
                layers[-1][2] = (layers[-1][2] - m.running_mean.detach()) * s + m.bias.detach()
                layers[-1][1] = layers[-1][1] * s
            elif isinstance(m, torch.nn.ReLU):
                layers[-1][3] = 1
            elif isinstance(m, (torch.nn.Identity, torch.nn.Dropout)):
                continue
            else:
                raise RuntimeError(f"PointwiseChain: unsupported module {name}")
        self.tensors = [[l[0], l[1].contiguous(), l[2].contiguous()] for l in layers]
        n = len(layers)
        self.n = n
        self.channels = [layers[0][0].shape[1]] + [l[0].shape[0] for l in layers]
        mk = lambda k: (ctypes.c_void_p * n)(*[t[k].data_ptr() for t in self.tensors])
        self.W, self.scale, self.shift = mk(0), mk(1), mk(2)
        self.ch = (ctypes.c_int * (n + 1))(*self.channels)
        self.relu = (ctypes.c_int * n)(*[l[3] for l in layers])

    @staticmethod
    def supported(modules):
        ch = []
        for m in modules:
            if isinstance(m, (torch.nn.Linear, torch.nn.Conv1d)):
                if isinstance(m, torch.nn.Conv1d) and (m.kernel_size != (1,) or m.groups != 1 or m.stride != (1,)):
                    return False
                ch.append((m.weight.shape[1], m.weight.shape[0]))
        if not 1 <= len(ch) <= 4:
            return False
        ok = all(ci % 16 == 0 and 16 <= ci <= 64 for ci, _ in ch) and all(co % 16 == 0 and co <= 64 for _, co in ch[:-1])
        return ok and 1 <= ch[-1][1] <= 64


def pointwise_mlp(x, chain, rows=None):
    _f32c(x, "x")
    N = x.shape[0]
    if rows is not None:
# ... 767 lines not shown
```

include/geoformer_hip.h:

```cpp
#ifndef GEOFORMER_HIP_H
#define GEOFORMER_HIP_H

#include <stddef.h>
#include <stdint.h>

#ifdef __cplusplus
extern "C" {
#endif

#define GF_ABI_VERSION 7

typedef enum {
    GF_OK = 0,
    GF_ERR_INVALID_ARG = -1,
    GF_ERR_LAUNCH = -2,
    GF_ERR_UNSUPPORTED = -3,
    GF_ERR_CALLBACK = -4,
} gf_status;

int gf_abi_version(void);
const char* gf_last_error(void);

size_t gf_fg_scratch_bytes(int N);
int gf_fg_select(const float* scores, int N, int C, int cls, int mode, const float* locs, const int32_t* batch_idxs,
// ... 60 lines not shown
                  float* dW, void* stream);
int gf_conv_wgrad_masked(const float* in, const float* dout, const int32_t* nbr, const uint32_t* gmask, int K, int M_out,
                         int ld, int Cin, int Cout, float* dW, void* stream);
int gf_conv_wgrad_masked_acc(const float* in, const float* dout, const int32_t* nbr, const uint32_t* gmask, int K,
                             int M_out, int ld, int Cin, int Cout, float* dW, void* stream);

typedef struct GfTrainOp {
    int kind, level, table, src, dst, aux, Cin, Cout, no_dgrad, pad_;
    const float* w;
    const float *gamma, *beta;
    float *running_mean, *running_var;
    float eps, momentum;
    long long wp_off;
    long long pgrad_off;
    long long stats_off;
} GfTrainOp;
typedef struct GfTrainLevel {
    int M, ld;
    const int32_t* nbr; const uint32_t* gmask; const int32_t* steps;
    int M_coarse, ld_down;
    const int32_t* child; const uint32_t* gmask_down;
    int ld_up, pad_; const int32_t* up; const uint32_t* gmask_up;
    const int32_t* flat;
} GfTrainLevel;
size_t gf_unet_train_scratch_floats(const GfTrainOp* ops, int nops, const GfTrainLevel* levels);
int gf_unet_train_fwd(const GfTrainOp* ops, int op_begin, int op_end, const GfTrainLevel* levels, float* const* act,
                      float* wp, float* stats, float* scratch, void* stream);
int gf_unet_train_bwd(const GfTrainOp* ops, int op_begin, int op_end, const GfTrainLevel* levels, float* const* act,
                      float** grad, unsigned char* ghas, const float* stats, float* pgrad, float* scratch, void* stream);

#define GF_UNET_MAX_LEVELS 8
typedef struct GfResBlockParams {
    const float *wp0, *wp1, *wpi;
    const float *s0, *t0, *s1, *t1;
} GfResBlockParams;
typedef struct GfUnetLevelParams {
    int C;
    int tr_layers;
    GfResBlockParams blocks[2];
    GfResBlockParams tail[2];
    const float *down_wp, *down_s, *down_t;
    const float *up_wp, *up_s, *up_t;
    const float* const* tr_params;
} GfUnetLevelParams;
typedef struct GfUnetParams {
    int nlevels;
    int cin;
    const float* input_wp;
    const float *out_s, *out_t;
    GfUnetLevelParams level[GF_UNET_MAX_LEVELS];
} GfUnetParams;
size_t gf_unet_ws_bytes(const GfUnetParams* P, int M0, int B, int X, int Y, int Z);
int gf_unet_fwd(const GfUnetParams* P, const float* feats, const int32_t* coords, int M0, int B, int X, int Y, int Z,
                void* ws, size_t ws_bytes, int32_t* host_counts, float* out, void* stream, void* side_stream);
typedef int (*GfUnetBetween)(void* user, void** events_out, int max_events);
int gf_unet_fwd_phased(const GfUnetParams* P, const float* feats, const int32_t* coords, int M0, int B, int X, int Y, int Z,
                       void* ws, size_t ws_bytes, int32_t* host_counts, float* out, void* stream, void* side_stream,
                       void* const* gate_events, int n_gate, GfUnetBetween between, void* user);

int gf_unet_fwd_ahead(const GfUnetParams* P, const float* feats, const int32_t* coords, int M0, int B, int X, int Y, int Z,
                      void* ws, size_t ws_bytes, int32_t* host_counts, float* out, void* stream, void* side_stream,
                      void* const* input_events, int n_input);


int gf_lsap(const float* cost, int nq, int K, const int32_t* present, int32_t* match_q, int32_t* match_of_q,
            int32_t* n_match, int32_t* status, void* stream);

size_t gf_pair_losses_sums_floats(int K);
int gf_pair_losses_fwd(const float* mask_logits, const float* inst_masks, const int32_t* match_q, int nq, int K, int n,
                       const int32_t* n_match, float* sums, float* out, void* stream);
int gf_pair_losses_bwd(const float* mask_logits, const float* inst_masks, const int32_t* match_of_q, const float* sums,
                       int nq, int K, int n, const int32_t* n_match, const float* grad_out, float* d_logits, void* stream);

size_t gf_bn_train_scratch_floats(int M, int C);
int gf_bn_relu_train_fwd(const float* x, int M, int C, const float* gamma, const float* beta, float eps, float momentum,
                         int relu, float* running_mean, float* running_var, float* y, float* save_mean,
                         float* save_invstd, float* scratch, void* stream);
int gf_bn_relu_train_bwd(const float* x, const float* y, const float* dy, int M, int C, const float* gamma,
                         const float* save_mean, const float* save_invstd, int relu, float* dx, float* dgamma,
                         float* dbeta, float* scratch, void* stream);
int gf_bn_relu_train_bwd_add(const float* x, const float* y, const float* dy, int M, int C, const float* gamma,
                             const float* save_mean, const float* save_invstd, int relu, const float* addend, float* dx,
                             float* dgamma, float* dbeta, float* scratch, void* stream);

size_t gf_bn_train_cl_scratch_floats(int B, int C, long long L);
int gf_bn_relu_train_cl_fwd(const float* x, int B, int C, long long L, const float* gamma, const float* beta, float eps,
                            float momentum, int relu, float* running_mean, float* running_var, float* y,
                            float* save_mean, float* save_invstd, float* scratch, void* stream);
int gf_bn_relu_train_cl_bwd(const float* x, const float* y, const float* dy, int B, int C, long long L,
                            const float* gamma, const float* save_mean, const float* save_invstd, int relu, float* dx,
                            float* dgamma, float* dbeta, float* scratch, void* stream);


size_t gf_voxelize_idx_scratch_bytes(int N);
int gf_voxelize_idx_count(const long long* coords, int N, int ncol, int mode, void* scratch, int32_t* input_map,
                          int32_t* d_M_maxActive, void* stream);
int gf_voxelize_idx_fill(const long long* coords, int N, int ncol, int mode, void* scratch, const int32_t* input_map,
                         int M, int maxActive, long long* out_coords, int32_t* out_map, void* stream);

#define GF_FEEDER_MAX_COPIES 16
typedef struct {
    int slot, n_copies;
    const void* src[GF_FEEDER_MAX_COPIES];
    void* pinned[GF_FEEDER_MAX_COPIES];
    void* dev[GF_FEEDER_MAX_COPIES];
    size_t bytes[GF_FEEDER_MAX_COPIES];
    const long long* coords_dev;
    int N, ncol, mode, pad_;
    void* scratch;
    int32_t* input_map;
    int32_t* head_dev;
    int32_t* head_host;
    void* stream;
} GfFeederJob;
void* gf_feeder_create(int device);
int gf_feeder_submit(void* feeder, const GfFeederJob* job);
int gf_feeder_wait_issued(void* feeder, int slot);
int gf_feeder_wait_copied(void* feeder, int slot);
int gf_feeder_wait_head(void* feeder, int slot);
int gf_feeder_destroy(void* feeder);

int gf_voxelize_fp(const float* feats, const int32_t* rules, int M, int maxActive, int C, int average, float* out,
                   void* stream);
int gf_voxelize_bp(const float* d_out, const int32_t* rules, int M, int maxActive, int C, int average, float* d_feats,
                   void* stream);


int gf_gather_points(const float* points, const int32_t* idx, int b, int c, int n, int m, float* out, void* stream);
int gf_gather_points_grad(const float* grad_out, const int32_t* idx, int b, int c, int n, int m, float* grad_points,
                          void* stream);
int gf_group_points(const float* points, const int32_t* idx, int b, int c, int n, int npoints, int nsample, float* out,
                    void* stream);
int gf_group_points_grad(const float* grad_out, const int32_t* idx, int b, int c, int n, int npoints, int nsample,
                         float* grad_points, void* stream);
int gf_ball_query(const float* new_xyz, const float* xyz, int b, int n, int m, float radius, int nsample, int32_t* idx,
                  void* stream);
size_t gf_fps_scratch_bytes(int b);
int gf_furthest_point_sampling(const float* xyz, int b, int n, int m, int32_t* idxs, void* scratch, void* stream);
int gf_furthest_point_sampling_resume(const float* xyz, int b, int n, int m, int m_known, int32_t* idxs,
                                      void* scratch, void* stream);


size_t gf_knn_scratch_bytes(int n);
int gf_knn_radius(const float* xyz, int n, int k, float radius, int sqrt_out, float* D, int32_t* I, int32_t* deg,
                  void* scratch, void* stream);
const int32_t* gf_knn_error_flag(void* scratch, int n);

size_t gf_geodesic_bfs_queue_words(int n);
int gf_geodesic_bfs(const float* D, const int32_t* I, const int32_t* deg, int n, int K, const int32_t* src, int nq,
                    float radius, int max_step, float* geo, void* keys_ws, void* queue_ws, void* stream);
int gf_geodesic_bfs_cfg(const float* D, const int32_t* I, const int32_t* deg, int n, int K, const int32_t* src, int nq,
                        float radius, int max_step, float* geo, void* keys_ws, void* queue_ws, size_t queue_words,
                        int wg_threads, void* stream);

int gf_mask_head(const float* feat, const float* coords, const float* geo, const float* qxyz,
                 const float* sqrt_max_geo, const float* w1, const float* b1, const float* w2, const float* b2, int N,
                 int nq, int C, float* out, void* stream);
int gf_mask_head_packed(const float* feat, const float* coords, const float* geo, const float* qxyz,
                        const float* sqrt_max_geo, const float* w1, const float* b1, const float* w2, const float* b2,
                        int ldp, int N, int nq, int C, float* out, void* stream);
size_t gf_mask_head_split_bytes(int N);
int gf_mask_head_episodes(const float* feat, const float* coords, const float* geo, const float* qxyz,
                          const float* sqrt_max_geo, const float* w1, const float* b1, const float* w2, const float* b2,
                          int ldp, int N, int nq, int E, int C, void* split_ws, float* out, void* stream);

size_t gf_mask_head_bwd_scratch_floats(int N, int nq);
int gf_mask_head_bwd(const float* feat, const float* coords, const float* geo, const float* qxyz,
                     const float* sqrt_max_geo, const float* w1, const float* b1, const float* w2, const float* gout,
                     int ldp, int N, int nq, int C, float* dparams, float* dfeat, float* scratch, void* stream);
int gf_mask_head_bwd_episodes(const float* feat, const float* coords, const float* geo, const float* qxyz,
                              const float* sqrt_max_geo, const float* w1, const float* b1, const float* w2,
                              const float* gout, int ldp, int N, int nq, int E, int C, float* dparams, float* dfeat,
                              float* scratch, void* stream);


int gf_pointwise_mlp(const float* x, int N, int n_layers, const float* const* W, const float* const* scale,
                     const float* const* shift, const int* channels, const int* relu, float* out, void* stream);
int gf_pointwise_mlp_rows(const float* x, const int32_t* rows, int N, int n_layers, const float* const* W,
                          const float* const* scale, const float* const* shift, const int* channels, const int* relu,
                          float* out, void* stream);

int gf_group_mlp_max(const float* grouped, int B, int npoint, int nsample, int n_layers, const float* const* W,
                     const float* const* scale, const float* const* shift, const int* channels, const int* relu,
                     float* out, void* stream);

int gf_ball_query_centres(const float* xyz, const int32_t* centre_idx, int b, int n, int m, float radius, int nsample,
                          float* new_xyz, int32_t* idx, void* stream);
int gf_point_grid_build(const float* xyz, int n, float radius, void* scratch, void* stream);
int gf_ball_query_grid(const float* xyz, int n, const int32_t* centre_idx, const float* centres, int m, float radius,
                       int nsample, void* scratch, int grid_ready, float* new_xyz, int32_t* idx, void* stream);
int gf_sa_group_mlp_max(const float* xyz, const float* feats, const int32_t* inds, int B, int n, int C, int npoint,
                        float radius, int nsample, int use_xyz, int normalize_xyz, int n_layers,
                        const float* const* W, const float* const* scale, const float* const* shift,
                        const int* channels, const int* relu, float* new_xyz, int32_t* idx, float* out, void* scratch,
                        int grid_ready, void* stream);

int gf_softmax_dim1_fwd(const float* x, int n0, int n1, int inner, float scale, float* y, void* stream);
int gf_softmax_dim1_bwd(const float* y, const float* gy, int n0, int n1, int inner, float scale, float* gx,
                        void* stream);


size_t gf_decoder_token_state_bytes(int nq, int B);
int gf_decoder_token_stage(const float* attn_out, const float* tgt_in, const float* query_pos, int nq, int B, int d,
                           int nhead, int ff, const float* const* post_params, const float* const* pre_params,
                           void* state, float* inter_out, float* q1_out, void* stream);

size_t gf_decoder_pre_train_save_bytes(int T, int B);
size_t gf_decoder_pre_train_work_bytes(int T, int B);
long long gf_decoder_pre_grad_floats(void);
int gf_decoder_pre_train_fwd(const float* x, const float* qpos, int T, int B, const float* const* params, float p,
                             unsigned seed, int layer, void* save, float* t2n, float* q1, void* stream);
int gf_decoder_pre_train_bwd(const float* x, const float* qpos, const float* t2n, const float* d_t2n, const float* d_q1,
                             int T, int B, const float* const* params, float p, unsigned seed, int layer, void* save,
                             void* work, float* dx, float* dqpos, float* grads, void* stream);
size_t gf_decoder_post_train_save_bytes(int T, int B, int ff);
size_t gf_decoder_post_train_work_bytes(int T, int B, int ff);
long long gf_decoder_post_grad_floats(int ff);
int gf_decoder_post_train_fwd(const float* ca, const float* t2n, int T, int B, int ff, const float* const* params,
                              float p, unsigned seed, int layer, void* save, float* x3, float* inter, void* stream);
int gf_decoder_post_train_bwd(const float* ca, const float* x3, const float* d_x3, const float* d_inter, int T, int B,
                              int ff, const float* const* params, float p, unsigned seed, int layer, void* save,
                              void* work, float* d_ca, float* d_t2n, float* grads, void* stream);


int gf_proposal_stats(const float* mask_logits, const float* cls_logits, const float* sem_prob, int nq, int N,
                      int ncls, float logit_thresh, float score_thresh, int npoint_thresh, int min_class,
                      int* cls_pred, int* npoints, float* scores, int* final_mask, void* stream);

int gf_proposal_stats_fs(const float* mask_logits, const float* sim, int nq, int N, float logit_thresh,
                         float score_thresh, int npoint_thresh, float sim_thresh, int* npoints, float* scores,
                         int* final_mask, void* stream);

int gf_proposal_scatter(const float* mask_logits, const int* sel, int n_sel, int N, const long long* fg_idxs,
                        float logit_thresh, int num_points, int* proposals, void* stream);

int gf_relpos_prepare(const float* geo, const int32_t* inds, int nq, int n, int nc, float* geo_ctx, float* max_geo,
                      void* stream);

int gf_proposal_select(const int32_t* final_, const int32_t* cls_pred, const float* scores, int nq, int32_t* sel,
                       long long* cls_out, float* scores_out, int32_t* d_count, void* stream);

size_t gf_mask_intersections_scratch_bytes(int n, int N);
int gf_mask_intersections(const int32_t* masks, int n, int N, void* scratch, int32_t* inter, void* stream);

#define GF_PROP_SCENE_FIELDS 6
int gf_proposal_stats_batched(const long long* table, int S, int nq, const float* cls_logits, const float* sem_prob,
                              long long sem_stride, int ncls, float logit_thresh, float score_thresh, int npoint_thresh,
                              int min_class, int* cls_pred, int* npoints, float* scores, int* final_mask, void* stream);
int gf_proposal_select_batched(const int32_t* final_, const int32_t* cls_pred, const float* scores, int S, int nq,
                               int32_t* sel, long long* cls_out, float* scores_out, int32_t* counts, void* stream);
int gf_proposal_scatter_batched(const long long* table, int S, int nq, const int32_t* sel, const int32_t* counts,
                                int total_rows, int max_N, const long long* fg_idxs, float logit_thresh, int* packed,
                                void* stream);

#define GF_NMS_SCENE_FIELDS 8
#define GF_NMS_MAX_N 1024
int gf_mask_intersections_batched(const long long* table, int S, long long max_waves, long long max_pairs, void* bits,
                                  int32_t* inter, void* stream);
int gf_matrix_nms_batched(const long long* table, int S, const int32_t* inter, int kernel, float sigma,
                          float final_score_thresh, int32_t* picks, int32_t* pick_counts, void* stream);

#define GF_LBL_SCENE_FIELDS 12
#define GF_LBL_CHUNK 4096
#define GF_LBL_OWN_SPLIT 4
#define GF_LBL_TABLE_INTS 5
#define GF_LBL_TABLE_FLOATS 10
int gf_label_map_batched(const long long* table, int S, long long max_points, int max_picks, float min_score,
                         void* bits, float* part_f, int32_t* part_cnt, int32_t* own_part, int32_t* owner, int32_t* ids,
                         int32_t* tab_i, float* tab_f, void* stream);

size_t gf_instance_overlaps_scratch_bytes(int N, int C);
int gf_instance_overlaps(const int32_t* masks, int n_rows, int N, const int32_t* rows, int n, const long long* gt_ids,
                         const int32_t* class_ids, int C, int max_gt, void* scratch, int32_t* d_G, long long* gt_id,
                         int32_t* gt_count, int32_t* inter, void* stream);


size_t gf_backbone_transformer_scratch_bytes(int M);
int gf_backbone_transformer_num_params(int n_layers);
int gf_backbone_transformer(const float* feats, const int* coords, const int* scene_offsets, int n_scenes, int M,
                            int c, int n_layers, const float* const* params, void* scratch, float* out,
                            void* stream);

size_t gf_backbone_transformer_train_save_bytes(int M, int n_layers);
size_t gf_backbone_transformer_train_work_bytes(int M, int n_layers, int n_scenes);
long long gf_backbone_transformer_grad_floats(int c, int n_layers);
int gf_backbone_transformer_train_fwd(const float* feats, const int* coords, int n_scenes, int M, int c, int n_layers,
                                      const float* const* params, float p, unsigned seed, void* save, float* out,
                                      void* stream);
int gf_backbone_transformer_train_bwd(const float* feats, const float* dout, int n_scenes, int M, int c, int n_layers,
                                      const float* const* params, float p, unsigned seed, void* save, void* work,
                                      float* dfeats, float* grads, void* stream);


size_t gf_decoder_wpack_floats(void);
int gf_decoder_pack_weights(const float* W1, const float* W2, const float* Wv, float* Wpack, void* stream);

int gf_decoder_cross_attn(const float* geo_ctx, const float* max_geo, const float* qloc, const float* cloc,
                          const float* lo, const float* hi, const float* gaussB, const float* Q1, const float* K1,
                          const float* Kv, const float* Wpack, const float* b2, int B, int nq, int nc, int d, float* out,
                          float* stat_m, float* stat_l, void* stream);
int gf_decoder_cross_attn_cfg(const float* geo_ctx, const float* max_geo, const float* qloc, const float* cloc,
                              const float* lo, const float* hi, const float* gaussB, const float* Q1, const float* K1,
                              const float* Kv, const float* Wpack, const float* b2, int B, int nq, int nc, int d,
                              float* out, float* stat_m, float* stat_l, int wg_waves, void* stream);

size_t gf_decoder_cross_attn_bwd_scratch_floats(int B, int nq, int nc);
// ... 98 lines not shown
```

include/geoformer_hip_dev.h:

```cpp
#ifndef GEOFORMER_HIP_DEV_H
#define GEOFORMER_HIP_DEV_H

#include "geoformer_hip.h"

#ifdef __cplusplus
extern "C" {
#endif

int gf_dev_conv_fwd_timed(const float* in, const float* Wp, const int32_t* nbr, const uint32_t* gmask,
                          const int32_t* steps, int K, int M_in, int M_out, int ld, int Cin, int Cout, const float* in_scale, const float* in_shift,
                          const float* residual, const float* out_scale, const float* out_shift, float* out, void* ev_start,
                          void* ev_stop, void* stream);

int gf_dev_conv_knobs(int split, int wide, int pair, int ldsw, int block);

int gf_dev_conv_knobs_g16(int use, int ldsw, int gpw, int pipe);

int gf_dev_conv_knob_flat(int use, int max_items);

int gf_dev_conv_knob_lw(int use, int min_groups);

int gf_dev_conv_plan(const float* in, const float* Wp, const int32_t* nbr, const uint32_t* gmask, const int32_t* steps,
                     const int32_t* flat, int K, int M_in, int M_out, int ld, int Cin, int Cout, const float* in_scale,
                     const float* in_shift, const float* residual, const float* out_scale, const float* out_shift, float* out,
                     float* out_act, int* desc);

int gf_dev_conv_chunks(int n);
int gf_dev_conv_g16p_wpb(int wpb);

int gf_dev_unet_probe(int mode);
unsigned long long gf_dev_host_wait_ns(int reset);
int gf_dev_unet_probe_read(int max_records, int* meta, float* us);
int gf_dev_unet_probe_read2(int max_records, int* meta, float* us, float* us_kernel);
int gf_dev_conv_kernel_events(void* start, void* stop);
int gf_dev_conv_kernel_events_taken(void);

int gf_dev_op_kernel_events(int op, void* start, void* stop);
int gf_dev_op_kernel_events_taken(int op);
void* gf_dev_event_create(void);
int gf_dev_event_destroy(void* event);
int gf_dev_event_elapsed_us(void* start, void* stop, float* us);

int gf_dev_cross_attn_bf3(int on);

int gf_dev_bfs_qcap_max(int qcap);

#ifdef __cplusplus
}
#endif
#endif
```

Measured before the change: 225.6.

## Fuse per-query geodesic max into BFS kernel and add co-residency launch planner

The geodesic BFS kernels now track the per-query maximum distance and write it out in a wave-shuffle plus atomicMax epilogue. The side epilogue uses that value, so it no longer runs a separate torch.max/where reduction over the full geo matrix. A planner can cap BFS LDS and pick the block size so BFS blocks fit on a CU beside the FPS kernel, but this is gated behind a dev flag that is off by default. The LDS kernel also gains a waves_per_eu(7) attribute, which may raise register pressure, and the build now emits kernel resource usage remarks.

```diff
diff --git a/geoformer_amd/_build.py b/geoformer_amd/_build.py
--- a/geoformer_amd/_build.py
+++ b/geoformer_amd/_build.py
@@ -15,6 +15,11 @@
 INCLUDE_DIR = os.path.join(REPO_DIR, "include")
 
 ARCH = "gfx950"
+USAGE_FLAG = "-Rpass-analysis=kernel-resource-usage"
+
+
+def _usage_path(obj: str) -> str:
+    return obj[:-2] + ".usage.txt"
 
 
 def _hipcc() -> str:
@@ -56,6 +61,7 @@
         "-ffp-contract=off",
         "-fno-gpu-rdc",
         "-Wno-unused-result",
+        USAGE_FLAG,
         f"-I{INCLUDE_DIR}",
         f"-I{CSRC_DIR}",
     ]
@@ -65,7 +71,7 @@
     for s in srcs:
         o = os.path.join(OBJ_DIR, os.path.basename(s)[:-4] + ".o")
         objs.append(o)
-        if force or _stale(o, [s] + hdrs):
+        if force or _stale(o, [s] + hdrs) or not os.path.exists(_usage_path(o)):
             jobs.append((s, o))
 
     def _cc(job):
@@ -76,6 +82,8 @@
         r = subprocess.run(cmd, capture_output=True, text=True)
         if r.returncode != 0:
             raise RuntimeError(f"hipcc failed for {s}:\n{r.stdout}\n{r.stderr}")
+        with open(_usage_path(o), "w") as f:
+            f.write(r.stderr)
         return o
 
     if jobs:
@@ -89,5 +97,28 @@
     return LIB_PATH
 
 
+_USAGE_FIELDS = {"VGPRs": "vgprs", "AGPRs": "agprs", "ScratchSize [bytes/lane]": "scratch", "LDS Size [bytes/block]": "lds",
+                 "Occupancy [waves/SIMD]": "occupancy"}
+
+
+def kernel_resource_usage(source: str) -> dict:
+    path = _usage_path(os.path.join(OBJ_DIR, source + ".o"))
+    if not os.path.exists(path):
+        build_hip()
+    out, cur = {}, None
+    with open(path) as f:
+        for line in f:
+            if "remark:" not in line:
+                continue
+            text = line.split("remark:", 1)[1].replace("[-Rpass-analysis=kernel-resource-usage]", "").strip()
+            key, _, val = text.rpartition(":")
+            key, val = key.strip(), val.strip()
+            if key == "Function Name":
+                cur = out.setdefault(val, {})
+            elif cur is not None and key in _USAGE_FIELDS:
+                cur[_USAGE_FIELDS[key]] = int(val)
+    return out
+
+
 if __name__ == "__main__":
     print(build_hip(force="--force" in sys.argv, verbose=True))
diff --git a/geoformer_amd/_lib.py b/geoformer_amd/_lib.py
--- a/geoformer_amd/_lib.py
+++ b/geoformer_amd/_lib.py
@@ -90,8 +90,11 @@
         "gf_geodesic_bfs": (I, [P, P, P, I, I, P, I, F, I, P, P, P, P]),
         "gf_geodesic_bfs_cfg": (I, [P, P, P, I, I, P, I, F, I, P, P, P, c_size_t, I, P]),
         "gf_geodesic_bfs_queue_words": (c_size_t, [I]),
+        "gf_geodesic_bfs_plan": (I, [I, I, I, P, P, P]),
+        "gf_geodesic_bfs_ex": (I, [P, P, P, I, I, P, I, F, I, P, P, P, P, c_size_t, I, I, I, I, P, P]),
         "gf_dev_cross_attn_bf3": (I, [I]),
         "gf_dev_bfs_qcap_max": (I, [I]),
+        "gf_dev_bfs_plan_coresident": (I, [I]),
         "gf_mask_head": (I, [P, P, P, P, P, P, P, P, P, I, I, I, P, P]),
         "gf_mask_head_packed": (I, [P, P, P, P, P, P, P, P, P, I, I, I, I, P, P]),
         "gf_mask_head_episodes": (I, [P, P, P, P, P, P, P, P, P, I, I, I, I, I, P, P, P]),
diff --git a/geoformer_amd/csrc/common.h b/geoformer_amd/csrc/common.h
--- a/geoformer_amd/csrc/common.h
+++ b/geoformer_amd/csrc/common.h
@@ -65,6 +65,8 @@
 }
 
 void gf_allow_lds(const void* kernel, int bytes);
+
+int gf_fps_footprint(int n, int* G, int* P, int* vgprs, int* static_lds, int* threads);
 
 template <int D>
 __device__ __forceinline__ float gf_shfl_xor(float v) {
diff --git a/geoformer_amd/csrc/geodesic.hip b/geoformer_amd/csrc/geodesic.hip
--- a/geoformer_amd/csrc/geodesic.hip
+++ b/geoformer_amd/csrc/geodesic.hip
@@ -1,4 +1,6 @@
 #include <cstdlib>
+#include <map>
+#include <mutex>
 #include "common.h"
 
 #ifndef BFS_KEY_SCOPE
@@ -375,13 +377,22 @@
 }
 
 #define BFS_THREADS 1024
+__device__ __forceinline__ void bfs_store_max(int lmax, int* s_max, float* out) {
+#pragma unroll
+    for (int d = 32; d >= 1; d >>= 1) lmax = max(lmax, __shfl_xor(lmax, d, 64));
+    if ((threadIdx.x & 63) == 0) atomicMax(s_max, lmax);
+    __syncthreads();
+    if (threadIdx.x == 0) *out = __int_as_float(*s_max);
+}
 __global__ __launch_bounds__(BFS_THREADS) void k_geodesic_bfs(const float* __restrict__ D, const int32_t* __restrict__ I,
                                                               const int32_t* __restrict__ deg, int n, int K,
                                                               const int32_t* __restrict__ src, float radius,
                                                               int max_step, float* __restrict__ geo,
+                                                              float* __restrict__ geo_max,
                                                               unsigned* __restrict__ keys,
                                                               int32_t* __restrict__ queues) {
     __shared__ int s_cnt;
+    __shared__ int s_max;
     const int q = blockIdx.x;
     float* g = geo + (size_t)q * n;
     unsigned* key = keys + (size_t)q * n;
@@ -398,9 +409,11 @@
         g[s] = 0.0f;
         cur[0] = make_int2(s, deg ? deg[s] : K - 1);
         s_cnt = 0;
+        s_max = 0;
     }
     __syncthreads();
     int ncur = 1;
+    int lmax = 0;
     const bool vec = (K & 3) == 0;
     for (int step = 0; step < max_step && ncur > 0; step++) {
         for (int f = tid; f < ncur; f += BFS_THREADS) {
@@ -458,7 +471,9 @@
             const unsigned kk = __hip_atomic_load(&key[v], __ATOMIC_RELAXED, BFS_KEY_SCOPE) - 1u;
             const int u = (int)(kk >> 6), r = (int)(kk & 63u);
             const int dv = deg ? deg[v] : K - 1;
-            g[v] = D[(size_t)u * K + r] + g[u];
+            const float gvn = D[(size_t)u * K + r] + g[u];
+            g[v] = gvn;
+            lmax = max(lmax, __float_as_int(gvn));
             nxt[t].y = dv;
         }
         __syncthreads();
@@ -467,6 +482,7 @@
         nxt = tmp;
         ncur = nn;
     }
+    if (geo_max) bfs_store_max(lmax, &s_max, geo_max + q);
 }
 
 #define BFS_LDS_MAX_N (1 << 19)
@@ -479,14 +495,16 @@
     __builtin_amdgcn_fence(__ATOMIC_ACQUIRE, "workgroup", "local");
 }
 template <int THREADS>
-__global__ __launch_bounds__(THREADS) void k_geodesic_bfs_lds(const float* __restrict__ D,
+__global__ __launch_bounds__(THREADS) __attribute__((amdgpu_waves_per_eu(7))) void k_geodesic_bfs_lds(const float* __restrict__ D,
                                                                   const int32_t* __restrict__ I, int n, int K,
                                                                   const int32_t* __restrict__ src, float radius,
                                                                   int max_step, float* __restrict__ geo,
+                                                                  float* __restrict__ geo_max,
                                                                   unsigned long long* __restrict__ keys,
                                                                   int2* __restrict__ queues, int qcap) {
     extern __shared__ __attribute__((aligned(16))) unsigned char smem[];
     __shared__ int s_cnt[2];
+    __shared__ int s_max;
     const int nw = (n + 31) >> 5;
     unsigned* visited = reinterpret_cast<unsigned*>(smem);
     unsigned* touched = visited + nw;
@@ -515,9 +533,11 @@
         q0[0] = make_int2(s, __float_as_int(0.0f));
         s_cnt[0] = 0;
         s_cnt[1] = 0;
+        s_max = 0;
     }
     __syncthreads();
     int ncur = 1;
+    int lmax = 0;
     int2 *cl = q0, *cg = gq0, *nl = q1, *ng = gq1;
     constexpr int BFS_B = 4;
     const int l16 = tid & 15;
@@ -714,6 +734,7 @@
                 if (t < nn && l16 == 0) {
                     const int di = (int)kk[k];
                     g[v[k]] = __int_as_float(di);
+                    lmax = max(lmax, di);
                     if (!decltype(spill)::value || t < qcap) nl[t].y = di;
                     else ng[t - qcap].y = di;
                     atomicOr(&visited[v[k] >> 5], 1u << (v[k] & 31));
@@ -748,15 +769,16 @@
     if (tid == 0 && n >= 12)
         for (int i = 0; i < 12; i++) reinterpret_cast<unsigned long long*>(gq0)[i] = tr[i];
 #endif
+    if (geo_max) bfs_store_max(lmax, &s_max, geo_max + q);
 }
 
 template <int THREADS>
 static void launch_bfs_lds(int nq, size_t lds, hipStream_t st, const float* D, const int32_t* I, int n, int K,
-                           const int32_t* src, float radius, int max_step, float* geo, void* keys_ws, void* queue_ws,
-                           int qcap) {
+                           const int32_t* src, float radius, int max_step, float* geo, float* geo_max, void* keys_ws,
+                           void* queue_ws, int qcap) {
     gf_allow_lds((const void*)k_geodesic_bfs_lds<THREADS>, BFS_LDS_BYTES);
     GF_LAUNCH_OP(GF_OP_BFS, k_geodesic_bfs_lds<THREADS>, dim3(nq), dim3(THREADS), lds, st, D, I, n, K, src, radius, max_step,
-                 geo, (unsigned long long*)keys_ws, (int2*)queue_ws, qcap);
+                 geo, geo_max, (unsigned long long*)keys_ws, (int2*)queue_ws, qcap);
 }
 static int g_bfs_qcap_max = 0;
 extern "C" int gf_dev_bfs_qcap_max(int qcap) {
@@ -765,20 +787,84 @@
 }
 extern "C" size_t gf_geodesic_bfs_queue_words(int n) { return (size_t)4 * (size_t)(n > 0 ? n : 0); }
 
-extern "C" int gf_geodesic_bfs_cfg(const float* D, const int32_t* I, const int32_t* deg, int n, int K,
-                                   const int32_t* src, int nq, float radius, int max_step, float* geo, void* keys_ws,
-                                   void* queue_ws, size_t queue_words, int wg_threads, void* stream) {
+#define BFS_COLDS_BYTES (BFS_LDS_BYTES / 2)
+#define BFS_CU_LDS_BYTES (160 * 1024)
+struct BfsFootprint {
+    int cus, bfs_vgprs, bfs_static_lds;
+};
+static int bfs_footprint(BfsFootprint* out) {
+    static std::mutex mu;
+    static std::map<int, BfsFootprint> cache;
+    int dev = 0;
+    GF_TRY(hipGetDevice(&dev));
+    std::lock_guard<std::mutex> lock(mu);
+    auto it = cache.find(dev);
+    if (it == cache.end()) {
+        BfsFootprint f;
+        hipFuncAttributes fa;
+        GF_TRY(hipDeviceGetAttribute(&f.cus, hipDeviceAttributeMultiprocessorCount, dev));
+        GF_TRY(hipFuncGetAttributes(&fa, (const void*)k_geodesic_bfs_lds<1024>));
+        f.bfs_vgprs = fa.numRegs;
+        f.bfs_static_lds = (int)fa.sharedSizeBytes;
+        it = cache.emplace(dev, f).first;
+    }
+    *out = it->second;
+    return GF_OK;
+}
+static int g_bfs_plan_coresident = 0;
+extern "C" int gf_dev_bfs_plan_coresident(int on) {
+    const int was = g_bfs_plan_coresident;
+    g_bfs_plan_coresident = on ? 1 : 0;
+    return was;
+}
+static bool bfs_fits_beside(int bfs_vgprs, int bfs_lds, int other_vgprs, int other_lds, int other_threads) {
+    const int bw = 1024 / 64 / 4, ow = (other_threads / 64 + 3) / 4;
+    const int regs = ((bfs_vgprs + 7) & ~7) * bw + ((other_vgprs + 7) & ~7) * ow;
+    return regs <= 512 && bw + ow <= 8 && bfs_lds + other_lds <= BFS_CU_LDS_BYTES;
+}
+extern "C" int gf_geodesic_bfs_plan(int nq, int scenes, int fps_n, const int* inject, int* wg_threads, int* lds_cap) {
+    GF_CHECK_ARG(nq >= 0 && scenes >= 1 && wg_threads && lds_cap, "gf_geodesic_bfs_plan: bad arguments");
+    *wg_threads = (long long)nq * scenes <= 224 ? 1024 : 512;
+    *lds_cap = 0;
+    if (scenes != 1 || fps_n <= 0 || !g_bfs_plan_coresident) return GF_OK;
+    int v[6];
+    bool all = inject != nullptr;
+    for (int i = 0; i < 6; i++) {
+        v[i] = inject ? inject[i] : -1;
+        all = all && v[i] >= 0;
+    }
+    if (!all) {
+        BfsFootprint f;
+        if (int rc = bfs_footprint(&f)) return rc;
+        int fv = 0, fl = 0, ft = 0;
+        if (int rc = gf_fps_footprint(fps_n, nullptr, nullptr, &fv, &fl, &ft)) return rc;
+        const int real[6] = {f.cus, f.bfs_vgprs, f.bfs_static_lds, fv, fl, ft};
+        for (int i = 0; i < 6; i++)
+            if (v[i] < 0) v[i] = real[i];
+    }
+    if (nq <= v[0] && bfs_fits_beside(v[1], v[2] + BFS_COLDS_BYTES, v[3], v[4], v[5])) {
+        *wg_threads = 1024;
+        *lds_cap = BFS_COLDS_BYTES;
+    }
+    return GF_OK;
+}
+
+static int bfs_launch(const float* D, const int32_t* I, const int32_t* deg, int n, int K, const int32_t* src, int nq,
+                      float radius, int max_step, float* geo, float* geo_max, void* keys_ws, void* queue_ws,
+                      size_t queue_words, int wg_threads, int lds_cap, void* stream) {
     GF_CHECK_ARG(n >= 1 && K >= 2 && K <= 64 && nq >= 0 && max_step >= 0, "gf_geodesic_bfs: bad arguments");
     GF_CHECK_ARG(n < (1 << 26), "gf_geodesic_bfs: n=%d exceeds the 26-bit parent field", n);
     GF_CHECK_ARG(wg_threads == 1024 || wg_threads == 512 || wg_threads == 256, "gf_geodesic_bfs: wg_threads=%d (256, 512 or 1024)",
                  wg_threads);
+    GF_CHECK_ARG(lds_cap >= 0, "gf_geodesic_bfs: lds_cap=%d", lds_cap);
     if (nq == 0) return GF_OK;
     GF_CHECK_ARG(queue_words >= (size_t)4 * (size_t)n, "gf_geodesic_bfs: queue workspace of %zu words per query, %zu needed",
                  queue_words, (size_t)4 * (size_t)n);
     const int nw = (n + 31) / 32;
     const size_t bm = ((size_t)2 * nw + ((2 * nw) & 1)) * sizeof(unsigned);
     while (wg_threads < 1024 && bm + 256 * 2 * sizeof(int2) > (size_t)BFS_LDS_BYTES * wg_threads / 1024) wg_threads *= 2;
-    const size_t budget = (size_t)BFS_LDS_BYTES * wg_threads / 1024;
+    size_t budget = (size_t)BFS_LDS_BYTES * wg_threads / 1024;
+    if (lds_cap > 0 && (size_t)lds_cap < budget && bm + 256 * 2 * sizeof(int2) <= (size_t)lds_cap) budget = (size_t)lds_cap;
     if (n <= BFS_LDS_MAX_N && (K & 3) == 0 && bm + 64 * 2 * sizeof(int2) <= budget) {
         int qcap = (int)((budget - bm) / (2 * sizeof(int2)));
         if (qcap > n) qcap = n;
@@ -786,18 +872,41 @@
         const size_t lds = bm + (size_t)qcap * 2 * sizeof(int2);
         hipStream_t st = (hipStream_t)stream;
         if (wg_threads == 256)
-            launch_bfs_lds<256>(nq, lds, st, D, I, n, K, src, radius, max_step, geo, keys_ws, queue_ws, qcap);
+            launch_bfs_lds<256>(nq, lds, st, D, I, n, K, src, radius, max_step, geo, geo_max, keys_ws, queue_ws, qcap);
         else if (wg_threads == 512)
-            launch_bfs_lds<512>(nq, lds, st, D, I, n, K, src, radius, max_step, geo, keys_ws, queue_ws, qcap);
+            launch_bfs_lds<512>(nq, lds, st, D, I, n, K, src, radius, max_step, geo, geo_max, keys_ws, queue_ws, qcap);
         else
-            launch_bfs_lds<1024>(nq, lds, st, D, I, n, K, src, radius, max_step, geo, keys_ws, queue_ws, qcap);
+            launch_bfs_lds<1024>(nq, lds, st, D, I, n, K, src, radius, max_step, geo, geo_max, keys_ws, queue_ws, qcap);
         GF_CHECK_LAUNCH("gf_geodesic_bfs");
         return GF_OK;
     }
     hipLaunchKernelGGL(k_geodesic_bfs, dim3(nq), dim3(BFS_THREADS), 0, (hipStream_t)stream, D, I, deg, n, K, src,
-                       radius, max_step, geo, (unsigned*)keys_ws, (int32_t*)queue_ws);
+                       radius, max_step, geo, geo_max, (unsigned*)keys_ws, (int32_t*)queue_ws);
     GF_CHECK_LAUNCH("gf_geodesic_bfs");
     return GF_OK;
+}
+
+extern "C" int gf_geodesic_bfs_cfg(const float* D, const int32_t* I, const int32_t* deg, int n, int K,
+                                   const int32_t* src, int nq, float radius, int max_step, float* geo, void* keys_ws,
+                                   void* queue_ws, size_t queue_words, int wg_threads, void* stream) {
+    return bfs_launch(D, I, deg, n, K, src, nq, radius, max_step, geo, nullptr, keys_ws, queue_ws, queue_words, wg_threads, 0,
+                      stream);
+}
+
+extern "C" int gf_geodesic_bfs_ex(const float* D, const int32_t* I, const int32_t* deg, int n, int K, const int32_t* src,
+                                  int nq, float radius, int max_step, float* geo, float* geo_max, void* keys_ws,
+                                  void* queue_ws, size_t queue_words, int wg_threads, int lds_cap, int scenes, int fps_n,
+                                  int* chosen, void* stream) {
+    if (wg_threads == 0) {
+        GF_CHECK_ARG(scenes >= 1, "gf_geodesic_bfs_ex: scenes=%d", scenes);
+        if (int rc = gf_geodesic_bfs_plan(nq, scenes, fps_n, nullptr, &wg_threads, &lds_cap)) return rc;
+    }
+    if (chosen) {
+        chosen[0] = wg_threads;
+        chosen[1] = lds_cap;
+    }
+    return bfs_launch(D, I, deg, n, K, src, nq, radius, max_step, geo, geo_max, keys_ws, queue_ws, queue_words, wg_threads,
+                      lds_cap, stream);
 }
 
 extern "C" int gf_geodesic_bfs(const float* D, const int32_t* I, const int32_t* deg, int n, int K, const int32_t* src,
diff --git a/geoformer_amd/csrc/pointops.hip b/geoformer_amd/csrc/pointops.hip
--- a/geoformer_amd/csrc/pointops.hip
+++ b/geoformer_amd/csrc/pointops.hip
@@ -1,6 +1,9 @@
 #include <stdlib.h>
 
+#include <map>
+#include <mutex>
 #include <type_traits>
+#include <utility>
 
 #include "common.h"
 
@@ -353,10 +356,9 @@
 }
 
 template <int P>
-__global__ __launch_bounds__(FPS_WAVES * 64) void k_fps(const float* __restrict__ xyz, int n, int m, int m0, int G,
-                                                        int bs_log2, int batch0,
-                                                        unsigned long long* __restrict__ slots,
-                                                        int32_t* __restrict__ idxs, int* __restrict__ err) {
+__device__ __forceinline__ void fps_body(const float* __restrict__ xyz, int n, int m, int m0, int G, int bs_log2, int batch0,
+                                         unsigned long long* __restrict__ slots, int32_t* __restrict__ idxs,
+                                         int* __restrict__ err) {
     static_assert(FPS_NG >= 1 && FPS_NG * 64 == FPS_MAXG * FPS_KPUB && FPS_KPUB <= FPS_K && FPS_WAVES * 2 <= 64,
                   "lane mappings of the exchange");
     __shared__ unsigned long long s_part[2][FPS_WAVES * 2];
@@ -696,10 +698,69 @@
 }
 
 template <int P>
+__global__ __launch_bounds__(FPS_WAVES * 64) void k_fps(const float* __restrict__ xyz, int n, int m, int m0, int G,
+                                                        int bs_log2, int batch0,
+                                                        unsigned long long* __restrict__ slots,
+                                                        int32_t* __restrict__ idxs, int* __restrict__ err) {
+    fps_body<P>(xyz, n, m, m0, G, bs_log2, batch0, slots, idxs, err);
+}
+#define FPS_PINNED_INSTANCE(P)                                                                                            \
+    template <>                                                                                                           \
+    __global__ __launch_bounds__(FPS_WAVES * 64) __attribute__((amdgpu_num_vgpr(56))) void k_fps<P>(                      \
+        const float* __restrict__ xyz, int n, int m, int m0, int G, int bs_log2, int batch0,                              \
+        unsigned long long* __restrict__ slots, int32_t* __restrict__ idxs, int* __restrict__ err) {                      \
+        fps_body<P>(xyz, n, m, m0, G, bs_log2, batch0, slots, idxs, err);                                                 \
+    }
+FPS_PINNED_INSTANCE(1)
+FPS_PINNED_INSTANCE(2)
+FPS_PINNED_INSTANCE(3)
+FPS_PINNED_INSTANCE(4)
+FPS_PINNED_INSTANCE(5)
+#undef FPS_PINNED_INSTANCE
+
+template <int P>
 static void launch_fps(int G, int nb, hipStream_t st, const float* xyz, int n, int m, int m0, int bs_log2, int batch0,
                        unsigned long long* slots, int32_t* idxs, int* err) {
     GF_LAUNCH_OP(GF_OP_FPS, (k_fps<P>), dim3(G, nb), dim3(FPS_WAVES * 64), 0, st, xyz, n, m, m0, G, bs_log2, batch0, slots,
                  idxs, err);
+}
+
+static void fps_geometry(int n, int* G_out, int* P_out) {
+    const int per_wg = FPS_PW * 64;
+    int G = (2 * n + per_wg * 5 - 1) / (per_wg * 5);
+    if (G < 1) G = 1;
+    if (G > FPS_MAXG) G = FPS_MAXG;
+    *G_out = G;
+    *P_out = (n + G * per_wg - 1) / (G * per_wg);
+}
+template <class F>
+static void fps_with_instance(int P, F&& f) {
+    const int inst = P <= 6 ? (P < 1 ? 1 : P) : P <= 8 ? 8 : P <= 12 ? 12 : P <= 16 ? 16 : P <= 20 ? 20 : 22;
+    gf_with<int, 1, 2, 3, 4, 5, 6, 8, 12, 16, 20, 22>(inst, f);
+}
+int gf_fps_footprint(int n, int* G_out, int* P_out, int* vgprs, int* static_lds, int* threads) {
+    int G, P;
+    fps_geometry(n > 0 ? n : 1, &G, &P);
+    if (G_out) *G_out = G;
+    if (P_out) *P_out = P;
+    if (threads) *threads = FPS_WAVES * 64;
+    if (!vgprs && !static_lds) return GF_OK;
+    static std::mutex mu;
+    static std::map<std::pair<int, int>, std::pair<int, int>> cache;
+    int dev = 0;
+    GF_TRY(hipGetDevice(&dev));
+    std::lock_guard<std::mutex> lock(mu);
+    auto it = cache.find({dev, P});
+    if (it == cache.end()) {
+        hipFuncAttributes fa;
+        hipError_t e = hipSuccess;
+        fps_with_instance(P, [&](auto pc) { e = hipFuncGetAttributes(&fa, (const void*)k_fps<decltype(pc)::value>); });
+        GF_TRY(e);
+        it = cache.emplace(std::make_pair(dev, P), std::make_pair((int)fa.numRegs, (int)fa.sharedSizeBytes)).first;
+    }
+    if (vgprs) *vgprs = it->second.first;
+    if (static_lds) *static_lds = it->second.second;
+    return GF_OK;
 }
 
 extern "C" size_t gf_fps_scratch_bytes(int b) {
@@ -726,10 +787,8 @@
     int bs_log2 = 0;
     while ((2 << bs_log2) <= n && bs_log2 < 9) bs_log2++;
     const int per_wg = FPS_PW * 64;
-    int G = (2 * n + per_wg * 5 - 1) / (per_wg * 5);
-    if (G < 1) G = 1;
-    if (G > FPS_MAXG) G = FPS_MAXG;
-    const int P = (n + G * per_wg - 1) / (G * per_wg);
+    int G, P;
+    fps_geometry(n, &G, &P);
     GF_CHECK_ARG(P <= 22, "gf_furthest_point_sampling: n=%d too large (max %d)", n, FPS_MAXG * per_wg * 22);
     unsigned long long* slots = (unsigned long long*)scratch;
     int* err = (int*)(slots + (size_t)b * 2 * FPS_MAXG * FPS_KPUB);
@@ -737,17 +796,9 @@
     const int per_launch = 1024 / (G * FPS_WAVES) > 0 ? 1024 / (G * FPS_WAVES) : 1;
     for (int b0 = 0; b0 < b; b0 += per_launch) {
         const int nb = (b - b0) < per_launch ? (b - b0) : per_launch;
-        if (P <= 1) launch_fps<1>(G, nb, st, xyz, n, m, m_known, bs_log2, b0, slots, idxs, err);
-        else if (P <= 2) launch_fps<2>(G, nb, st, xyz, n, m, m_known, bs_log2, b0, slots, idxs, err);
-        else if (P <= 3) launch_fps<3>(G, nb, st, xyz, n, m, m_known, bs_log2, b0, slots, idxs, err);
-        else if (P <= 4) launch_fps<4>(G, nb, st, xyz, n, m, m_known, bs_log2, b0, slots, idxs, err);
-        else if (P <= 5) launch_fps<5>(G, nb, st, xyz, n, m, m_known, bs_log2, b0, slots, idxs, err);
-        else if (P <= 6) launch_fps<6>(G, nb, st, xyz, n, m, m_known, bs_log2, b0, slots, idxs, err);
-        else if (P <= 8) launch_fps<8>(G, nb, st, xyz, n, m, m_known, bs_log2, b0, slots, idxs, err);
-        else if (P <= 12) launch_fps<12>(G, nb, st, xyz, n, m, m_known, bs_log2, b0, slots, idxs, err);
-        else if (P <= 16) launch_fps<16>(G, nb, st, xyz, n, m, m_known, bs_log2, b0, slots, idxs, err);
-        else if (P <= 20) launch_fps<20>(G, nb, st, xyz, n, m, m_known, bs_log2, b0, slots, idxs, err);
-        else launch_fps<22>(G, nb, st, xyz, n, m, m_known, bs_log2, b0, slots, idxs, err);
+        fps_with_instance(P, [&](auto pc) {
+            launch_fps<decltype(pc)::value>(G, nb, st, xyz, n, m, m_known, bs_log2, b0, slots, idxs, err);
+        });
     }
     GF_CHECK_LAUNCH("gf_furthest_point_sampling");
     return GF_OK;
diff --git a/geoformer_amd/model/geoformer.py b/geoformer_amd/model/geoformer.py
--- a/geoformer_amd/model/geoformer.py
+++ b/geoformer_amd/model/geoformer.py
@@ -38,8 +38,10 @@
 import weakref
 
 
-def _bfs_wg(nq, scenes=1):
-    return 1024 if nq * scenes <= 224 else 512
+def _bfs_wg(nq, scenes=1, serving=False):
+    if serving:
+        return 1024 if nq * scenes <= 224 else 512
+    return 0
 _SIDE_STREAMS = {}
 _OFFS_CACHE = threading.local()
 
@@ -555,7 +557,7 @@
 
     def _aggregate_geodesic_overlapped(self, locs_float_, output_feats_, batch_offsets_, batch_size, graphs, max_step,
                                        pc_dims=None, sample=True, epilogue=True, early=None, presampled=None,
-                                       presampled_before=None):
+                                       presampled_before=None, serving=False):
         offs = _offsets_list(batch_offsets_)
         grad_ctx = self._grad_ctx("set_aggregator")
         nq, npoint_sa, split = self._sampling_split()
@@ -640,7 +642,11 @@
             with torch.cuda.stream(side_b):
                 D, I, deg = graphs[b][:3]
                 g = pointops.geodesic_bfs(D, I, deg, src, 0.05, max_step,
-                                          wg_threads=_bfs_wg(int(src.shape[0]), batch_size) if split else 1024)
+                                          wg_threads=_bfs_wg(int(src.shape[0]), batch_size, serving) if split else 1024,
+                                          scenes=batch_size, fps_n=int(xyz_b.shape[1]), return_max=epilogue)
+                gmax = None
+                if epilogue:
+                    g, gmax = g
                 g.record_stream(main)
                 src.record_stream(side_b)
                 geo[b] = g
@@ -674,7 +680,7 @@
             staged[b] = [xyz_b, None, idx, grid, sampling_indices]
             if not epilogue:
                 continue
-            self._side_epilogue(b, batch_size, g, xyz_b, src, pc_dims, main, side, aux, picks_ready)
+            self._side_epilogue(b, batch_size, g, xyz_b, src, pc_dims, main, side, aux, picks_ready, gmax)
         for sb in scene_streams:
             main.wait_stream(sb)
         with grad_ctx():
@@ -708,13 +714,16 @@
         res = ((context_locs, context_feats, pre_enc_inds), geo)
         return res + (early_out,) if early is not None else res
 
-    def _side_epilogue(self, b, batch_size, g, xyz_b, src, pc_dims, main, side, aux, first_ready):
+    def _side_epilogue(self, b, batch_size, g, xyz_b, src, pc_dims, main, side, aux, first_ready, gmax=None):
         early = self._early()
         if b == 0:
             early.clear()
         with torch.cuda.stream(side):
-            mx = torch.max(g, dim=1)[0]
-            mx = torch.sqrt(torch.where(mx < 0, torch.max(mx), mx)).contiguous()
+            if gmax is not None:
+                mx = torch.sqrt(gmax)
+            else:
+                mx = torch.max(g, dim=1)[0]
+                mx = torch.sqrt(torch.where(mx < 0, torch.max(mx), mx)).contiguous()
             mx.record_stream(main)
             ev = torch.cuda.Event()
             ev.record(side)
@@ -1133,13 +1142,15 @@
             contexts, geo_dists, (mask_features_, sem_prob, graphs) = self._aggregate_geodesic_overlapped(
                 locs_float_, output_feats_, batch_offsets_, batch_size, None, max_step, pc_dims, epilogue=True,
                 early=sampling_independent, presampled=presampled if fused_fg else None,
-                presampled_before=draw_bufs["before"] if (fused_fg and presampled is not None) else None)
+                presampled_before=draw_bufs["before"] if (fused_fg and presampled is not None) else None,
+                serving=split)
         else:
             mask_features_, sem_prob, graphs = sampling_independent()
             if graphs is not None and overlap:
                 contexts, geo_dists = self._aggregate_geodesic_overlapped(locs_float_, output_feats_, batch_offsets_,
                                                                           batch_size, graphs, max_step, pc_dims,
-                                                                          epilogue=not torch.is_grad_enabled())
+                                                                          epilogue=not torch.is_grad_enabled(),
+                                                                          serving=split)
             else:
                 contexts = self.forward_aggregator(locs_float_, output_feats_, batch_offsets_, batch_size)
         if contexts is None:
diff --git a/geoformer_amd/pointops.py b/geoformer_amd/pointops.py
--- a/geoformer_amd/pointops.py
+++ b/geoformer_amd/pointops.py
@@ -370,20 +370,31 @@
     return sum(t.numel() * t.element_size() for t in _SCRATCH.values() if t is not None)
 
 
-def geodesic_bfs(D, I, deg, src, radius, max_step, wg_threads=1024):
+def geodesic_bfs_plan(nq, scenes=1, fps_n=0, inject=None):
+    import ctypes
+    wg, cap = ctypes.c_int(0), ctypes.c_int(0)
+    inj = None if inject is None else (ctypes.c_int * 6)(*[int(v) for v in inject])
+    check(_lib.load().gf_geodesic_bfs_plan(int(nq), int(scenes), int(fps_n), inj, ctypes.byref(wg), ctypes.byref(cap)),
+          "gf_geodesic_bfs_plan")
+    return wg.value, cap.value
+
+
+def geodesic_bfs(D, I, deg, src, radius, max_step, wg_threads=1024, lds_cap=0, scenes=1, fps_n=0, return_max=False):
     _f32c(D, "D"); _i32c(I, "I"); _i32c(src, "src")
     n, K = D.shape
     nq = src.shape[0]
     dev = D.device
     geo = torch.empty((nq, n), dtype=torch.float32, device=dev)
+    gmax = torch.empty((nq,), dtype=torch.float32, device=dev) if return_max else None
     lib = _lib.load()
     keys = scratch("bfs_keys", nq * n, torch.int64, dev)
     qwords = int(lib.gf_geodesic_bfs_queue_words(n))
     queues = scratch("bfs_queues", nq * qwords, torch.int32, dev)
-    check(lib.gf_geodesic_bfs_cfg(ptr(D), ptr(I), ptr(deg), n, K, ptr(src), nq, float(radius), int(max_step),
-                                          ptr(geo), ptr(keys), ptr(queues), qwords, int(wg_threads), stream_ptr()),
+    check(lib.gf_geodesic_bfs_ex(ptr(D), ptr(I), ptr(deg), n, K, ptr(src), nq, float(radius), int(max_step),
+                                 ptr(geo), ptr(gmax), ptr(keys), ptr(queues), qwords, int(wg_threads), int(lds_cap),
+                                 int(scenes), int(fps_n), None, stream_ptr()),
           "gf_geodesic_bfs")
-    return geo
+    return (geo, gmax) if return_max else geo
 
 
 def _mask_head_split_ws(N, device, split):
diff --git a/include/geoformer_hip.h b/include/geoformer_hip.h
--- a/include/geoformer_hip.h
+++ b/include/geoformer_hip.h
@@ -236,6 +236,10 @@
 int gf_geodesic_bfs_cfg(const float* D, const int32_t* I, const int32_t* deg, int n, int K, const int32_t* src, int nq,
                         float radius, int max_step, float* geo, void* keys_ws, void* queue_ws, size_t queue_words,
                         int wg_threads, void* stream);
+int gf_geodesic_bfs_plan(int nq, int scenes, int fps_n, const int* inject, int* wg_threads, int* lds_cap);
+int gf_geodesic_bfs_ex(const float* D, const int32_t* I, const int32_t* deg, int n, int K, const int32_t* src, int nq,
+                       float radius, int max_step, float* geo, float* geo_max, void* keys_ws, void* queue_ws,
+                       size_t queue_words, int wg_threads, int lds_cap, int scenes, int fps_n, int* chosen, void* stream);
 
 int gf_mask_head(const float* feat, const float* coords, const float* geo, const float* qxyz,
                  const float* sqrt_max_geo, const float* w1, const float* b1, const float* w2, const float* b2, int N,
diff --git a/include/geoformer_hip_dev.h b/include/geoformer_hip_dev.h
--- a/include/geoformer_hip_dev.h
+++ b/include/geoformer_hip_dev.h
@@ -44,6 +44,7 @@
 int gf_dev_cross_attn_bf3(int on);
 
 int gf_dev_bfs_qcap_max(int qcap);
+int gf_dev_bfs_plan_coresident(int on);
 
 #ifdef __cplusplus
 }
```

New measurement: 228.5 (median of 3 runs). No clear change (+1.3%).
